# linkedin/gdmix

Hardware: AMD Instinct MI355X
Metric: random-effect entities converged/sec (higher is better)
Workload: dtype f64; 1 GPU; C2: synthetic 1000000 entities/GPU x avg 64 nnz (n~max(1,Poisson(16)), k=4 distinct uniform columns of D=1024, SURVEY 8(d) generator), per-entity L2 LR, L-BFGS m=10; build_id=003fc741b5b29e59, workload_key=c2, entities_per_gpu=1000000, step=pack+solve, theta on device, parallelism=entity-shard x1

## Files before the change

### gdmix_amd/csrc/re_api.hip

```cpp
#include <stdarg.h>
#include <stdio.h>
#include <stdlib.h>
#include <string.h>
#include <time.h>

#include <errno.h>
#include <fcntl.h>
#include <sys/file.h>
#include <sys/stat.h>
#include <unistd.h>

#include <condition_variable>
#include <map>
#include <new>
#include <string>

#include <mutex>

#include "re_internal.hpp"
#include "re_solve_team.hpp"

namespace gdmix {

static thread_local char g_err[512] = "";
// ... 180 lines not shown
  if ((e && atoi(e) == 0) || hipDeviceGetPCIBusId(bus, sizeof(bus), device) != hipSuccess || !bus[0] ||
      hipStreamCreateWithFlags(&g_rel_stream[device], hipStreamNonBlocking) != hipSuccess) {
    g_dev_lock_off[device] = true;
    return nullptr;
  }
  return g_dev_lock[device] = grid_lock_by_key(bus);
}

void grid_lock_release_cb(void* p) { static_cast<GridLock*>(p)->release(); }

std::mutex g_here_mu;
std::map<std::string, int> g_here_fd;

int presence_fd(int device) {
  char bus[64] = "";
  if (hipDeviceGetPCIBusId(bus, sizeof(bus), device) != hipSuccess || !bus[0]) return -1;
  std::lock_guard<std::mutex> g(g_here_mu);
  auto it = g_here_fd.find(bus);
  if (it != g_here_fd.end()) return it->second;
  const char* dir = getenv("GDMIX_RE_LOCK_DIR");
  std::string path = std::string(dir && *dir ? dir : "/tmp") + "/gdmix_re_grid_";
  for (const char* c = bus; *c; ++c) path += (isalnum((unsigned char)*c) || *c == '.' || *c == '-') ? *c : '_';
  path += ".here";
  const int fd = open(path.c_str(), O_RDWR | O_CREAT | O_CLOEXEC, 0666);
  if (fd >= 0) {
    (void)fchmod(fd, 0666);
    struct flock fl = {};
    fl.l_type = F_RDLCK; fl.l_whence = SEEK_SET; fl.l_start = 0; fl.l_len = 1;
    (void)fcntl(fd, F_SETLK, &fl);
  }
  return g_here_fd[bus] = fd;
}
}

void device_register_process(int device) {
  const char* e = getenv("GDMIX_RE_GRID_LOCK");
  if (!(e && atoi(e) == 0)) (void)presence_fd(device);
}

bool device_has_another_process(int device) {
  const char* e = getenv("GDMIX_RE_GRID_LOCK");
  if (e && atoi(e) == 0) return false;
  const int fd = presence_fd(device);
  if (fd < 0) return false;
  struct flock fl = {};
  fl.l_type = F_WRLCK; fl.l_whence = SEEK_SET; fl.l_start = 0; fl.l_len = 1;
  return fcntl(fd, F_GETLK, &fl) == 0 && fl.l_type != F_UNLCK;
}

ScopedGridGate::ScopedGridGate(int device, hipStream_t s) : device_(device >= 0 && device < GATE_DEVICES ? device : 0), s_(s), err_(hipSuccess), held_(nullptr) {
  g_gate_mu[device_].lock();
  if (!g_gate_ev[device_]) err_ = hipEventCreateWithFlags(&g_gate_ev[device_], hipEventDisableTiming);
  if (err_ == hipSuccess && g_gate_armed[device_]) err_ = hipStreamWaitEvent(s_, g_gate_ev[device_], 0);
  if (err_ == hipSuccess) {
    GridLock* const L = grid_lock_of_device(device_);
    if (L && L->acquire()) held_ = L;
  }
}

ScopedGridGate::~ScopedGridGate() {
  const bool recorded = g_gate_ev[device_] && hipEventRecord(g_gate_ev[device_], s_) == hipSuccess;
  if (recorded) g_gate_armed[device_] = true;
  if (held_) {
    GridLock* const L = static_cast<GridLock*>(held_);
    if (!(recorded && hipStreamWaitEvent(g_rel_stream[device_], g_gate_ev[device_], 0) == hipSuccess &&
          hipLaunchHostFunc(g_rel_stream[device_], grid_lock_release_cb, L) == hipSuccess)) {
      (void)hipStreamSynchronize(s_);
      L->release();
    }
  }
  g_gate_mu[device_].unlock();
}
}

extern "C" {

static int spread_default() {
  const char* e = getenv("GDMIX_RE_SPREAD");
  const int n = e ? atoi(e) : 4;
  return n > 1 ? n : 0;
}
GDMIX_API int gdmix_re_abi_version(void) { return GDMIX_RE_ABI_VERSION; }

GDMIX_API int gdmix_re_grid_lock_acquire(const char* key) {
  if (!key || !*key) { set_error("key is empty"); return GDMIX_RE_EINVAL; }
  return grid_lock_by_key(key)->acquire() ? GDMIX_RE_OK : GDMIX_RE_EINVAL;
}
GDMIX_API int gdmix_re_grid_lock_release(const char* key) {
  if (!key || !*key) { set_error("key is empty"); return GDMIX_RE_EINVAL; }
  grid_lock_by_key(key)->release();
  return GDMIX_RE_OK;
}
GDMIX_API int gdmix_re_grid_lock_stats(const char* key, int64_t* takes, int64_t* rides) {
  if (!key || !*key || !takes || !rides) { set_error("bad argument"); return GDMIX_RE_EINVAL; }
  long t = 0, r = 0;
  grid_lock_by_key(key)->stats(&t, &r);
  *takes = t;
  *rides = r;
  return GDMIX_RE_OK;
}

GDMIX_API const char* gdmix_re_last_error(void) { return g_err; }

GDMIX_API void gdmix_re_default_opts(gdmix_re_opts* o) {
  if (!o) return;
  o->l2 = 1.0; o->regularize_bias = 1; o->has_intercept = 1; o->m = 10; o->max_iter = 100;
  o->maxfun = 15000; o->maxls = 20; o->ftol = 1e-12; o->pgtol = 1e-5;
  o->variance_mode = GDMIX_RE_VAR_NONE; o->threshold = 1e-4;
  o->sum_loss = 0; o->loss = 0;
}

GDMIX_API int gdmix_re_create(int hip_device, gdmix_re_ctx** out) {
  if (!out) { set_error("out is NULL"); return GDMIX_RE_EINVAL; }
  *out = nullptr;
  int count = 0;
  HIP_TRY(hipGetDeviceCount(&count));
  if (hip_device < 0 || hip_device >= count) {
    set_error("HIP device %d not present (%d visible)", hip_device, count);
    return GDMIX_RE_EHIP;
  }
  HIP_TRY(hipSetDevice(hip_device));
  hipDeviceProp_t prop;
  HIP_TRY(hipGetDeviceProperties(&prop, hip_device));
  if (strncmp(prop.gcnArchName, "gfx950", 6) != 0) {
    set_error("device %d is %s; this library only carries gfx950 (MI355X) code", hip_device, prop.gcnArchName);
    return GDMIX_RE_EHIP;
  }
  gdmix_re_ctx* c = new (std::nothrow) gdmix_re_ctx();
  if (!c) { set_error("out of host memory"); return GDMIX_RE_ENOMEM; }
  c->impl.device = hip_device;
  c->impl.num_cus = prop.multiProcessorCount;
  device_register_process(hip_device);
  c->impl.tall_adapt_limit = c->impl.num_cus * 3 / 2;
  if (const char* e = getenv("GDMIX_RE_TALL_ADAPT")) c->impl.tall_adapt_limit = atoi(e) > 0 ? atoi(e) : 0;
  c->impl.scratch = nullptr;
  c->impl.scratch_bytes = 0;
  c->impl.host_pinned = nullptr;
  c->impl.wave_lds_limit = 65536;
  c->impl.kernel_mask = 7;
  c->impl.timing = 0;
  c->impl.giant_nnz = 16777216;
  c->impl.team_nnz = 16384;
  c->impl.tall_min_n = GDMIX_RE_TALL_MIN_N_DEFAULT;
  c->impl.tall_split_n = GDMIX_RE_TALL_SPLIT_N_DEFAULT;
  c->impl.tall_split_set = 0;
  c->impl.tall_team_n = GDMIX_RE_TALL_TEAM_N_DEFAULT;
  c->impl.tall_team_limit = c->impl.num_cus / 4 < TALL_TEAM_MAX ? c->impl.num_cus / 4 : TALL_TEAM_MAX;
  c->impl.tall_mid_n = 0;
  if (const char* e = getenv("GDMIX_RE_TALL_MID")) { if (atoi(e) == 1) c->impl.tall_mid_n = -(c->impl.num_cus * TALL_MID_WGS); else if (atoi(e) > 1) c->impl.tall_mid_n = -atoi(e); }
  if (c->impl.num_cus < 8 * TALL_TEAM_C) c->impl.tall_team_n = 0;
  if (const char* e = getenv("GDMIX_RE_TALL_TEAM")) { if (atoi(e) == 0) c->impl.tall_team_n = 0; }
  if (const char* e = getenv("GDMIX_RE_TALL_TEAM_LIMIT")) { if (atoi(e) > 0 && atoi(e) <= TALL_TEAM_MAX) c->impl.tall_team_limit = atoi(e); }
  c->impl.spread = spread_default();
  c->impl.grid_sync = nullptr;
  c->impl.big_tmp = nullptr;
  c->impl.big_tmp_bytes = 0;
  c->impl.eval_small_set = 0; c->impl.eval_small_max = 64;
  c->impl.eval_tmp = nullptr; c->impl.eval_tmp_bytes = 0;
  c->impl.n_side = 0; c->impl.side_fork = nullptr;
  c->impl.aux_ev[0] = c->impl.aux_ev[1] = nullptr;
  c->impl.defer_unique = 0; c->impl.unique_pending = false; c->impl.unique_ev = nullptr;
  for (int k = 0; k < gdmix_ctx_impl::MAX_SIDE; ++k) { c->impl.side[k] = nullptr; c->impl.side_join[k] = nullptr; }
  for (int k = 0; k < GDMIX_RE_NUM_CLASSES; ++k) { c->impl.ev0[k] = nullptr; c->impl.ev1[k] = nullptr; c->impl.ev_used[k] = false; }
  for (uint32_t& q : c->impl.mail_seq) q = 0;
  hipError_t rc = hipHostMalloc(reinterpret_cast<void**>(&c->impl.host_pinned), HOST_PINNED_BYTES, hipHostMallocMapped | hipHostMallocCoherent);
  if (rc == hipSuccess) memset(c->impl.host_pinned, 0, HOST_PINNED_BYTES);
  if (rc != hipSuccess) {
    set_error("hipHostMalloc failed: %s", hipGetErrorString(rc));
    delete c;
    return GDMIX_RE_EHIP;
  }
  {
    const char* e = getenv("GDMIX_RE_SIDE_STREAM");
    int want = e ? atoi(e) : 3;
    if (want > gdmix_ctx_impl::MAX_SIDE) want = gdmix_ctx_impl::MAX_SIDE;
    if (want > 0) {
      rc = hipEventCreateWithFlags(&c->impl.side_fork, hipEventDisableTiming);
      for (int k = 0; k < 2 && rc == hipSuccess; ++k) rc = hipEventCreateWithFlags(&c->impl.aux_ev[k], hipEventDisableTiming);
      if (rc == hipSuccess) rc = hipEventCreateWithFlags(&c->impl.unique_ev, hipEventDisableTiming);
      for (int k = 0; k < want && rc == hipSuccess; ++k) {
        rc = hipStreamCreateWithFlags(&c->impl.side[k], hipStreamNonBlocking);
        if (rc == hipSuccess) rc = hipEventCreateWithFlags(&c->impl.side_join[k], hipEventDisableTiming);
        if (rc == hipSuccess) c->impl.n_side = k + 1;
      }
      if (rc != hipSuccess) {
        set_error("creating the side streams failed: %s", hipGetErrorString(rc));
        gdmix_re_destroy(c);
        return GDMIX_RE_EHIP;
      }
    }
  }
  rc = hipMalloc(&c->impl.grid_sync, GridSyncLayout::BYTES);
  if (rc != hipSuccess) {
    set_error("hipMalloc failed: %s", hipGetErrorString(rc));
    (void)hipHostFree(c->impl.host_pinned);
    delete c;
    return GDMIX_RE_EHIP;
  }
  *out = c;
  return GDMIX_RE_OK;
}

GDMIX_API void gdmix_re_destroy(gdmix_re_ctx* ctx) {
  if (!ctx) return;
  if (ctx->impl.unique_pending && ctx->impl.unique_ev) (void)hipEventSynchronize(ctx->impl.unique_ev);
  if (ctx->impl.unique_ev) (void)hipEventDestroy(ctx->impl.unique_ev);
  if (ctx->impl.grid_sync) (void)hipFree(ctx->impl.grid_sync);
  if (ctx->impl.big_tmp) (void)hipFree(ctx->impl.big_tmp);
  if (ctx->impl.eval_tmp) (void)hipFree(ctx->impl.eval_tmp);
  if (ctx->impl.host_pinned) (void)hipHostFree(ctx->impl.host_pinned);
  if (ctx->impl.side_fork) (void)hipEventDestroy(ctx->impl.side_fork);
  for (int k = 0; k < 2; ++k) if (ctx->impl.aux_ev[k]) (void)hipEventDestroy(ctx->impl.aux_ev[k]);
  for (int k = 0; k < gdmix_ctx_impl::MAX_SIDE; ++k) {
    if (ctx->impl.side_join[k]) (void)hipEventDestroy(ctx->impl.side_join[k]);
    if (ctx->impl.side[k]) (void)hipStreamDestroy(ctx->impl.side[k]);
  }
  for (int k = 0; k < GDMIX_RE_NUM_CLASSES; ++k) {
    if (ctx->impl.ev0[k]) (void)hipEventDestroy(ctx->impl.ev0[k]);
    if (ctx->impl.ev1[k]) (void)hipEventDestroy(ctx->impl.ev1[k]);
  }
  delete ctx;
}

GDMIX_API size_t gdmix_re_pack_workspace_bytes(int64_t E, int64_t N, int64_t Z) {
  if (E < 0 || N < 0 || Z < 0) return 0;
  return pack_workspace_bytes(E, N, Z);
}

GDMIX_API int gdmix_re_pack(gdmix_re_ctx* ctx, const gdmix_re_raw_batch* raw_dev, int has_intercept, void* workspace,
                  size_t workspace_bytes, gdmix_re_packed* out, void* stream) {
  if (!ctx || !raw_dev || !out || (!workspace && workspace_bytes)) { set_error("NULL argument"); return GDMIX_RE_EINVAL; }
  if (raw_dev->E > 0 && (!raw_dev->ent_row_ptr || !raw_dev->row_nnz_ptr || !raw_dev->y || !raw_dev->offset)) {
    set_error("raw batch has NULL arrays");
    return GDMIX_RE_EINVAL;
  }
  if (raw_dev->Z > 0 && (!raw_dev->col_global || !raw_dev->val)) { set_error("raw batch has NULL arrays"); return GDMIX_RE_EINVAL; }
  HIP_TRY(hipSetDevice(ctx->impl.device));
  HIP_TRY(join_unique(&ctx->impl, static_cast<hipStream_t>(stream)));
  return pack_impl(&ctx->impl, raw_dev, has_intercept, workspace, workspace_bytes, out, static_cast<hipStream_t>(stream));
}

GDMIX_API int gdmix_re_set_defer_unique(gdmix_re_ctx* ctx, int enabled) {
  if (!ctx) { set_error("ctx is NULL"); return GDMIX_RE_EINVAL; }
  ctx->impl.defer_unique = (enabled && ctx->impl.n_side > 0) ? 1 : 0;
  return GDMIX_RE_OK;
}

GDMIX_API int gdmix_re_pack_join(gdmix_re_ctx* ctx, void* stream) {
  if (!ctx) { set_error("ctx is NULL"); return GDMIX_RE_EINVAL; }
  HIP_TRY(hipSetDevice(ctx->impl.device));
  HIP_TRY(join_unique(&ctx->impl, static_cast<hipStream_t>(stream)));
  return GDMIX_RE_OK;
}

static int slots_for(const gdmix_re_packed* b, const gdmix_re_opts* o, size_t* slot_doubles) {
  *slot_doubles = block_slot_doubles(b->max_p, b->max_n, o->m);
  size_t bytes = *slot_doubles * 8;
  size_t by_budget = ((size_t)4 << 30) / (bytes ? bytes : 1);
  size_t slots = 1024;
  if (slots > by_budget) slots = by_budget;
  if (slots < 8) slots = 8;
  if ((int64_t)slots > b->E) slots = (size_t)(b->E > 0 ? b->E : 1);
  return (int)slots;
}

static int64_t var_small_p(const gdmix_re_packed* b) { return b->max_p < VAR_FULL_MAX_P ? b->max_p : VAR_FULL_MAX_P; }

static int var_slots_for(const gdmix_re_packed* b) {
  size_t bytes = var_full_slot_doubles(var_small_p(b)) * 8;
  size_t slots = ((size_t)2 << 30) / (bytes ? bytes : 1);
  if (slots > 2048) slots = 2048;
  if (slots < 4) slots = 4;
  slots &= ~(size_t)3;
  return (int)slots;
}

GDMIX_API size_t gdmix_re_solve_scratch_bytes(const gdmix_re_packed* batch, const gdmix_re_opts* opts) {
  if (!batch || !opts || batch->E == 0) return 0;
  size_t slot_doubles;
  int slots = slots_for(batch, opts, &slot_doubles);
  size_t need = (size_t)slots * slot_doubles * 8;
  if (opts->variance_mode == GDMIX_RE_VAR_FULL && batch->max_p <= VAR_FULL_BIG_MAX_P) {
    size_t v = (size_t)var_slots_for(batch) * var_full_slot_doubles(var_small_p(batch)) * 8;
    if (v > need) need = v;
    if (batch->max_p > VAR_FULL_MAX_P) {
      v = var_full_big_doubles(batch->max_p, batch->max_n) * 8;
      if (v > need) need = v;
    }
  }
  return need;
}

GDMIX_API int gdmix_re_set_wave_lds_limit(gdmix_re_ctx* ctx, int bytes) {
  if (!ctx || bytes < 0) { set_error("bad argument"); return GDMIX_RE_EINVAL; }
  ctx->impl.wave_lds_limit = bytes > 65536 ? 65536 : bytes;
  return GDMIX_RE_OK;
}

GDMIX_API int gdmix_re_set_kernel_mask(gdmix_re_ctx* ctx, int mask) {
  if (!ctx) { set_error("ctx is NULL"); return GDMIX_RE_EINVAL; }
  ctx->impl.kernel_mask = mask & 7;
  return GDMIX_RE_OK;
}

GDMIX_API int gdmix_re_set_giant_nnz(gdmix_re_ctx* ctx, int64_t nnz) {
  if (!ctx || nnz < 0) { set_error("bad argument"); return GDMIX_RE_EINVAL; }
  ctx->impl.giant_nnz = nnz;
  return GDMIX_RE_OK;
}

GDMIX_API int gdmix_re_set_team_nnz(gdmix_re_ctx* ctx, int64_t nnz) {
  if (!ctx || nnz < 0) { set_error("bad argument"); return GDMIX_RE_EINVAL; }
  ctx->impl.team_nnz = nnz;
  return GDMIX_RE_OK;
}

GDMIX_API int gdmix_re_set_tall_min_n(gdmix_re_ctx* ctx, int min_n) {
  if (!ctx || min_n < 0) { set_error("bad argument"); return GDMIX_RE_EINVAL; }
  ctx->impl.tall_min_n = min_n;
  return GDMIX_RE_OK;
}

GDMIX_API int gdmix_re_set_spread(gdmix_re_ctx* ctx, int queues) {
  if (!ctx || queues < 0) { set_error("bad argument"); return GDMIX_RE_EINVAL; }
  ctx->impl.spread = queues > 1 ? queues : 0;
  return GDMIX_RE_OK;
}

GDMIX_API int gdmix_re_set_tall_team_n(gdmix_re_ctx* ctx, int team_n) {
  if (!ctx) { set_error("bad argument"); return GDMIX_RE_EINVAL; }
  ctx->impl.tall_team_n = ctx->impl.num_cus < 8 * TALL_TEAM_C ? 0 : team_n;
  return GDMIX_RE_OK;
}

GDMIX_API int gdmix_re_device_shared(gdmix_re_ctx* ctx) {
  if (!ctx) { set_error("ctx is NULL"); return GDMIX_RE_EINVAL; }
  return device_has_another_process(ctx->impl.device) ? 1 : 0;
}

GDMIX_API int gdmix_re_set_tall_mid_n(gdmix_re_ctx* ctx, int mid_n) {
  if (!ctx) { set_error("bad argument"); return GDMIX_RE_EINVAL; }
  ctx->impl.tall_mid_n = mid_n < 0 ? -(ctx->impl.num_cus * TALL_MID_WGS) : mid_n;
  return GDMIX_RE_OK;
}

GDMIX_API int gdmix_re_set_tall_split_n(gdmix_re_ctx* ctx, int split_n) {
  if (!ctx || split_n < 0) { set_error("bad argument"); return GDMIX_RE_EINVAL; }
  ctx->impl.tall_split_n = split_n > 0 ? split_n : GDMIX_RE_TALL_SPLIT_N_DEFAULT;
  ctx->impl.tall_split_set = split_n > 0 ? 1 : 0;
  return GDMIX_RE_OK;
}

GDMIX_API int gdmix_re_set_timing(gdmix_re_ctx* ctx, int enabled) {
  if (!ctx) { set_error("ctx is NULL"); return GDMIX_RE_EINVAL; }
  if (enabled && !ctx->impl.ev0[0]) {
    HIP_TRY(hipSetDevice(ctx->impl.device));
    for (int k = 0; k < GDMIX_RE_NUM_CLASSES; ++k) {
      HIP_TRY(hipEventCreate(&ctx->impl.ev0[k]));
      HIP_TRY(hipEventCreate(&ctx->impl.ev1[k]));
    }
  }
  ctx->impl.timing = enabled ? 1 : 0;
  return GDMIX_RE_OK;
}

GDMIX_API int gdmix_re_last_solve_ms(gdmix_re_ctx* ctx, float* ms_out) {
  if (!ctx || !ms_out) { set_error("NULL argument"); return GDMIX_RE_EINVAL; }
  for (int k = 0; k < GDMIX_RE_NUM_CLASSES; ++k) {
    ms_out[k] = 0.0f;
    if (ctx->impl.ev_used[k]) {
      HIP_TRY(hipEventSynchronize(ctx->impl.ev1[k]));
      HIP_TRY(hipEventElapsedTime(&ms_out[k], ctx->impl.ev0[k], ctx->impl.ev1[k]));
    }
  }
  return GDMIX_RE_OK;
}

GDMIX_API int gdmix_re_set_scratch(gdmix_re_ctx* ctx, void* scratch, size_t bytes) {
  if (!ctx) { set_error("ctx is NULL"); return GDMIX_RE_EINVAL; }
  ctx->impl.scratch = scratch;
  ctx->impl.scratch_bytes = bytes;
  return GDMIX_RE_OK;
}

static int run_variance_full(gdmix_re_ctx* ctx, const gdmix_re_packed* b, const BatchDev& B, const SolveParams& P, const double* theta,
                             double* variance, hipStream_t s) {
  const size_t vslot = var_full_slot_doubles(var_small_p(b));
  int vslots = var_slots_for(b);
  size_t avail = ctx->impl.scratch ? ctx->impl.scratch_bytes : 0;
  void* base = ctx->impl.scratch;
  if (b->scratch_bytes > avail) { avail = b->scratch_bytes; base = b->scratch; }
  if ((size_t)vslots * vslot * 8 > avail) vslots = (int)(avail / (vslot * 8)) & ~3;
  if (vslots < 4) {
    set_error("variance_mode FULL needs >= %zu bytes of scratch (gdmix_re_set_scratch)", 4 * vslot * 8);
    return GDMIX_RE_ENOMEM;
  }
  HIP_TRY(launch_variance_full(B, b->E, P, theta, variance, static_cast<double*>(base), vslot, vslots, var_small_p(b), s));
  if (b->max_p > VAR_FULL_MAX_P) {
    if (var_full_big_doubles(b->max_p, b->max_n) * 8 > avail) {
      set_error("variance_mode FULL with p = %d needs >= %zu bytes of scratch (gdmix_re_set_scratch)", b->max_p,
                var_full_big_doubles(b->max_p, b->max_n) * 8);
      return GDMIX_RE_ENOMEM;
    }
    HIP_TRY(launch_variance_full_big(&ctx->impl, B, b->E, P, theta, variance, static_cast<double*>(base), b->max_p, b->max_n, s));
  }
  return GDMIX_RE_OK;
}

}

namespace {

struct Slots { double* scratch = nullptr; size_t doubles = 0; int n = 0; };

int size_slots(const gdmix_ctx_impl* ci, const gdmix_re_packed* b, const gdmix_re_opts* opts, int n_slot_users, Slots* out) {
  if (n_slot_users <= 0) return GDMIX_RE_OK;
  out->n = slots_for(b, opts, &out->doubles);
  const size_t need = (size_t)out->n * out->doubles * 8;
  if (ci->scratch && ci->scratch_bytes >= need) out->scratch = static_cast<double*>(ci->scratch);
  else if (b->scratch && b->scratch_bytes >= need) out->scratch = static_cast<double*>(b->scratch);
  else {
    size_t avail = ci->scratch ? ci->scratch_bytes : 0;
    void* base = ci->scratch;
    if (b->scratch_bytes > avail) { avail = b->scratch_bytes; base = b->scratch; }
    out->n = (int)(avail / (out->doubles * 8));
    if (out->n < 1) {
      set_error("%d entities need a scratch slot: provide >= %zu bytes via gdmix_re_set_scratch", n_slot_users, out->doubles * 8);
      return GDMIX_RE_ENOMEM;
    }
    out->scratch = static_cast<double*>(base);
  }
  return GDMIX_RE_OK;
}

template <class F>
int timed(gdmix_ctx_impl* ci, int c, hipStream_t s, F&& launch) {
  if (ci->timing) HIP_TRY(hipEventRecord(ci->ev0[c], s));
  const hipError_t rc = launch();
  if (rc != hipSuccess) { set_error("launch of class %d (%s) failed: %s", c, kClasses[c].name, hipGetErrorString(rc)); return GDMIX_RE_EHIP; }
  if (ci->timing) { HIP_TRY(hipEventRecord(ci->ev1[c], s)); ci->ev_used[c] = true; }
  return GDMIX_RE_OK;
}

hipError_t launch_class(const gdmix_ctx_impl* ci, const gdmix_re_packed* b, const BatchDev& B, const OutDev& O, const SolveParams& P,
                        const double* theta0, const Launch& L, int lean_merged, hipStream_t s) {
  const ClassDesc& d = kClasses[L.c];
  switch (d.kind) {
    case KIND_WLDS:
      return launch_solve_wave(B, O, P, theta0, L.begin, L.count, d.lds, s);
    case KIND_TALL_T: {
      const char* xe = getenv("GDMIX_RE_XCD_BARRIER");
      return launch_solve_tall_team(B, O, P, theta0, L.begin, L.count, ci->num_cus, b->Z, GridSyncLayout::tall_tail(ci, d.tall_variant),
                                    GridSyncLayout::tall_team_buf(ci), (xe && atoi(xe) == 0) ? 0 : 1, s);
    }
    case KIND_TALL_L: case KIND_TALL_S: case KIND_TALL_M: case KIND_TALL:
      return launch_solve_tall(d.tall_variant, B, O, P, theta0, L.begin, L.count, ci->num_cus, b->Z, GridSyncLayout::tall_tail(ci, d.tall_variant),
                               GridSyncLayout::tall_ticket(ci, d.tall_variant), d.kind == KIND_TALL_S ? lean_merged : 0, s);
    default:
      return d.lanes > 0 ? launch_solve_quad(d.lanes, d.epl, B, O, P, theta0, L.begin, L.count, d.ncap, d.zcap, s) : hipErrorInvalidValue;
  }
}

int team_count(int tier_max, unsigned long long total_nnz, unsigned long long largest_nnz, int entities, int slots, int num_cus) {
  const unsigned long long ratio = largest_nnz ? total_nnz / largest_nnz : 1;
  int teams = 1;
  while (teams * 2 <= tier_max && (unsigned long long)(teams * 2) <= ratio) teams *= 2;
  if (entities <= 16) {
    int want = 1;
    while (want * 2 <= entities && want * 2 <= tier_max && want * 2 <= teams * 4) want *= 2;
    if (want > teams) teams = want;
  }
  if (const char* ev = getenv("GDMIX_RE_TEAMS")) teams = atoi(ev);
  if (teams > TEAM_MAX_TEAMS) teams = TEAM_MAX_TEAMS;
  while (teams > 1 && (slots < teams || num_cus % teams)) teams >>= 1;
  return teams < 1 ? 1 : teams;
}

int launch_slot_classes(gdmix_ctx_impl* ci, const gdmix_re_packed* b, const ClassCounts& hc, const BatchDev& B, OutDev O, const SolveParams& P,
                        const double* theta0, const Slots& slots, int n_slot_users, hipStream_t s) {
  const bool follow_var = P.loss != LOSS_LOGISTIC && P.variance_mode == GDMIX_RE_VAR_SIMPLE && P.m <= TEAM_MCAP;
  if (follow_var && P.loss == LOSS_POISSON && !O.theta) {
    set_error("variance_mode SIMPLE with the Poisson loss needs out->theta");
    return GDMIX_RE_EINVAL;
  }
  double* const variance = O.variance;
  if (follow_var) O.variance = nullptr;
  if (hc.count[BLOCK_CLASS] > 0) {
    const int rc = timed(ci, BLOCK_CLASS, s, [&] {
      return launch_solve_block(B, O, P, theta0, hc.base[BLOCK_CLASS], hc.count[BLOCK_CLASS], slots.scratch, slots.doubles, slots.n, b->max_p, s);
    });
    if (rc != GDMIX_RE_OK) return rc;
  }
  for (int c = TEAM128_CLASS; c <= GIANT_CLASS; ++c) {
    if (hc.count[c] <= 0) continue;
    const int tier_max = c == TEAM128_CLASS ? 128 : (c == TEAM32_CLASS ? 32 : 8);
    const int teams = c == GIANT_CLASS ? 1 : team_count(tier_max, hc.team_nnz_total[c], (unsigned long long)hc.largest_nnz(c), hc.count[c], slots.n, ci->num_cus);
    const int rc = timed(ci, c, s, [&] {
      return launch_solve_grid(B, O, P, theta0, hc.base[c], hc.count[c], slots.scratch, slots.doubles, b->max_p, GridSyncLayout::team_sync(ci), ci->num_cus, teams, s);
    });
    if (rc != GDMIX_RE_OK) return rc;
  }
  if (follow_var) HIP_TRY(launch_variance_simple(B, P, O.theta, variance, hc.base[BLOCK_CLASS], n_slot_users, slots.scratch, slots.doubles, slots.n, s));
  return GDMIX_RE_OK;
}

}

extern "C" {

GDMIX_API int gdmix_re_solve(gdmix_re_ctx* ctx, const gdmix_re_packed* b, const gdmix_re_opts* opts, const double* theta0,
                   const gdmix_re_result* out, void* stream) {
  if (!ctx || !b || !opts || !out) { set_error("NULL argument"); return GDMIX_RE_EINVAL; }
  if (opts->m < 1 || opts->max_iter < 0 || opts->maxls < 1) { set_error("bad solver options (m, max_iter, maxls)"); return GDMIX_RE_EINVAL; }
  if (!loss_code_ok(opts->loss, "gdmix_re_solve")) return GDMIX_RE_EINVAL;
  if (opts->variance_mode == GDMIX_RE_VAR_FULL) {
    if (!out->theta) { set_error("variance_mode FULL needs out->theta"); return GDMIX_RE_EINVAL; }
    if (b->max_p > VAR_FULL_BIG_MAX_P) {
      set_error("variance_mode FULL densifies a p x p Hessian per entity; largest entity has p = %d > %lld", b->max_p,
                (long long)VAR_FULL_BIG_MAX_P);
      return GDMIX_RE_ERANGE;
    }
  }
  if (opts->variance_mode != GDMIX_RE_VAR_NONE && !out->variance) { set_error("variance requested but out->variance is NULL"); return GDMIX_RE_EINVAL; }
  if (b->E == 0) return GDMIX_RE_OK;
  gdmix_ctx_impl* const ci = &ctx->impl;
  hipStream_t const s = static_cast<hipStream_t>(stream);
  HIP_TRY(hipSetDevice(ci->device));

  ClassTable tab;
  int rc = make_class_table(ci, opts, &tab);
  if (rc != GDMIX_RE_OK) return rc;
  const ClassCounts* hc = nullptr;
  rc = route(ci, b, tab, opts, s, &hc);
  if (rc != GDMIX_RE_OK) return rc;

  SolveParams P;
  P.l2 = opts->l2; P.ftol = opts->ftol; P.pgtol = opts->pgtol; P.threshold = opts->threshold;
  P.regularize_bias = opts->regularize_bias; P.has_intercept = opts->has_intercept ? 1 : 0; P.m = opts->m; P.max_iter = opts->max_iter;
  P.maxfun = opts->maxfun; P.maxls = opts->maxls; P.variance_mode = opts->variance_mode;
  P.sum_loss = opts->sum_loss ? 1 : 0; P.loss = opts->loss;
  const BatchDev B = batch_dev(b);
  const OutDev O{out->theta, out->theta_thr, out->variance, out->fval, out->gnorm, out->nit, out->nfev, out->status};
  for (int c = 0; c < GDMIX_RE_NUM_CLASSES; ++c) ci->ev_used[c] = false;

  int n_slot_users = 0;
  for (int c = BLOCK_CLASS; c <= GIANT_CLASS; ++c) n_slot_users += hc->count[c];
  Slots slots;
  rc = size_slots(ci, b, opts, n_slot_users, &slots);
  if (rc != GDMIX_RE_OK) return rc;

  int lean_rounds = 4;
  if (const char* ev = getenv("GDMIX_RE_LEAN_MERGE_ROUNDS")) lean_rounds = atoi(ev);
  const LaunchPlan plan = plan_launches(*hc, ci->num_cus, ci->n_side, ci->spread, lean_rounds);
  SideJoin side_join{ci, s};
  if (plan.fork) HIP_TRY(hipEventRecord(ci->side_fork, s));
  for (int k = 0; k < plan.n; ++k) {
    const Launch& L = plan.launch[k];
    hipStream_t q = s;
    if (L.stream >= 0) { HIP_TRY(side_join.use(L.stream)); q = ci->side[L.stream]; }
    rc = timed(ci, L.c, q, [&] { return launch_class(ci, b, B, O, P, theta0, L, plan.lean_merged, q); });
    if (rc != GDMIX_RE_OK) return rc;
  }
  side_join.join();
  if (n_slot_users > 0) {
    rc = launch_slot_classes(ci, b, *hc, B, O, P, theta0, slots, n_slot_users, s);
    if (rc != GDMIX_RE_OK) return rc;
  }
  if (opts->variance_mode == GDMIX_RE_VAR_FULL) {
    rc = run_variance_full(ctx, b, B, P, out->theta, out->variance, s);
    if (rc != GDMIX_RE_OK) return rc;
  }
  HIP_TRY(join_unique(ci, s));
  return GDMIX_RE_OK;
}

GDMIX_API int gdmix_re_variance_full(gdmix_re_ctx* ctx, const gdmix_re_packed* b, const gdmix_re_opts* opts, const double* theta,
                                     double* variance, void* stream) {
  if (!ctx || !b || !opts || !theta || !variance) { set_error("NULL argument"); return GDMIX_RE_EINVAL; }
  if (!loss_code_ok(opts->loss, "gdmix_re_variance_full")) return GDMIX_RE_EINVAL;
  if (b->max_p > VAR_FULL_BIG_MAX_P) {
    set_error("variance_mode FULL densifies a p x p Hessian per entity; largest entity has p = %d > %lld", b->max_p, (long long)VAR_FULL_BIG_MAX_P);
    return GDMIX_RE_ERANGE;
  }
  if (b->E == 0) return GDMIX_RE_OK;
  HIP_TRY(hipSetDevice(ctx->impl.device));
  HIP_TRY(join_unique(&ctx->impl, static_cast<hipStream_t>(stream)));
  SolveParams P;
  P.l2 = opts->l2; P.ftol = opts->ftol; P.pgtol = opts->pgtol; P.threshold = opts->threshold;
  P.regularize_bias = opts->regularize_bias; P.has_intercept = opts->has_intercept ? 1 : 0; P.m = opts->m; P.max_iter = opts->max_iter;
  P.maxfun = opts->maxfun; P.maxls = opts->maxls; P.variance_mode = GDMIX_RE_VAR_FULL;
  P.sum_loss = 0; P.loss = opts->loss;
  return run_variance_full(ctx, b, batch_dev(b), P, theta, variance, static_cast<hipStream_t>(stream));
}

GDMIX_API int gdmix_re_score(gdmix_re_ctx* ctx, const gdmix_re_packed* b, int has_intercept, const double* theta,
                   const uint8_t* has_model, float* logit, float* logit_per_coord, void* stream) {
  if (!ctx || !b || !logit || !logit_per_coord) { set_error("NULL argument"); return GDMIX_RE_EINVAL; }
  if (!theta && !has_model) { set_error("theta is NULL"); return GDMIX_RE_EINVAL; }
  HIP_TRY(hipSetDevice(ctx->impl.device));
  HIP_TRY(join_unique(&ctx->impl, static_cast<hipStream_t>(stream)));
  BatchDev B = batch_dev(b);
  HIP_TRY(launch_score(B, b->E, b->N, has_intercept ? 1 : 0, theta, has_model, logit, logit_per_coord,
                       static_cast<hipStream_t>(stream)));
  return GDMIX_RE_OK;
}

GDMIX_API const char* gdmix_re_class_kernel_name(int c) {
  if (c < 0 || c >= GDMIX_RE_NUM_CLASSES) return nullptr;
  return kClasses[c].name;
}

GDMIX_API int32_t gdmix_java_string_hash(const uint16_t* utf16, int64_t len) {
// ... 22 lines not shown
```

### gdmix_amd/csrc/re_internal.hpp

```cpp
#pragma once
#include <hip/hip_runtime.h>
#include <stdint.h>
#include <stddef.h>

#include <type_traits>

#include "../../include/gdmix_re.h"
#include "re_solve_core.hpp"
#include "re_solve_wreg.hpp"
#include "re_solve_quad.hpp"

namespace gdmix {

enum { KIND_WREG1 = 0, KIND_WREG2 = 1, KIND_WREG4 = 2, KIND_WLDS = 3, KIND_BLOCK = 4, KIND_QUAD2 = 5, KIND_QUAD4 = 6, KIND_PAIR4 = 7, KIND_QUAD3 = 8, KIND_PAIR3 = 9, KIND_WREG8 = 10,
       KIND_G64_3 = 11, KIND_G64_4 = 12, KIND_G128_4 = 13, KIND_G256_4 = 14, KIND_G512_4 = 15, KIND_GRID = 16, KIND_G128_3 = 17, KIND_G256_3 = 18,
       KIND_TALL = 20, KIND_TALL_S = 21, KIND_TALL_L = 22, KIND_TALL_T = 23, KIND_TALL_M = 24 };

__host__ __device__ constexpr int group_lanes(int kind) {
  return (kind == KIND_QUAD2 || kind == KIND_QUAD3 || kind == KIND_QUAD4) ? 16 : ((kind == KIND_PAIR3 || kind == KIND_PAIR4) ? 32 :
         ((kind == KIND_G64_3 || kind == KIND_G64_4) ? 64 : ((kind == KIND_G128_4 || kind == KIND_G128_3) ? 128 : ((kind == KIND_G256_4 || kind == KIND_G256_3) ? 256 : (kind == KIND_G512_4 ? 512 : 0)))));
}
__host__ __device__ constexpr int group_epl(int kind) {
  return kind == KIND_QUAD2 ? 2 : ((kind == KIND_QUAD3 || kind == KIND_PAIR3 || kind == KIND_G64_3 || kind == KIND_G128_3 || kind == KIND_G256_3) ? 3 : (group_lanes(kind) > 0 ? 4 : 0));
}
constexpr int TALL_TEAM_C = 4;
constexpr int TALL_TEAM_MAX = 64;
constexpr int TALL_TEAM_BYTES = 192 * 1024;
constexpr int TALL_TEAM_MIN_N = 64;
#ifndef GDMIX_TALL_NW_SMALL
#define GDMIX_TALL_NW_SMALL 1
#endif
constexpr int TALL_NW = 8;
constexpr int TALL_NW_SMALL = GDMIX_TALL_NW_SMALL;
constexpr int TALL_NW_MID = 4;
constexpr int TALL_MID_WGS = 2;
constexpr int TALL_MAX_P = 64;
constexpr int TALL_LEAN_WAVES = 3;
constexpr int TALL_LEAN_WGS = 4 * TALL_LEAN_WAVES;
__host__ __device__ constexpr int tall_sets(int nw, int p) { return (nw > 1 && p <= 32) ? 32 : 16; }
__host__ __device__ constexpr int tall_lds_bytes(int wg_per_cu) { return 160 * 1024 / wg_per_cu - 512; }
constexpr int TALL_LEAN_ARENA = (tall_lds_bytes(TALL_LEAN_WGS) - 1408) & ~15;
__host__ __device__ inline size_t tall_resident_bytes(int nw, int S, int d, int n, int nnz, bool has_w) {
  return (size_t)nw * (d + 1) * (S + 1) * 8 + (size_t)8 * (nnz + 8) + (size_t)4 * (n + 2) + (size_t)(has_w ? 12 : 8) * n + 16;
}

struct ClassDesc {
  int kind;
  int lanes, epl;
  int ncap, zcap;
  int lds;
  int occ_lanes;
  int tall_variant;
  int tall_rank;
  int small_side;
  const char* name;
};
enum { TALL_VARIANT_LARGE = 0, TALL_VARIANT_SMALL = 1, TALL_VARIANT_LEAN = 2, TALL_VARIANT_TEAM = 3, TALL_VARIANT_MID = 4, TALL_VARIANTS = 5 };
constexpr ClassDesc grp_class(int kind, int lanes, int epl, int ncap, int zcap, const char* name) { return {kind, lanes, epl, ncap, zcap, 1, lanes, -1, -1, -1, name}; }
constexpr ClassDesc wave_class(int lds, const char* name) { return {KIND_WLDS, 0, 0, 0, 0, lds, WAVE, -1, -1, -1, name}; }
constexpr ClassDesc tall_class(int kind, int variant, int rank, int occ_lanes, int side, const char* name) { return {kind, 0, 0, 0, 0, 0, occ_lanes, variant, rank, side, name}; }
constexpr ClassDesc team_class(int kind, const char* name) { return {kind, 0, 0, 0, 0, 0, WAVE, -1, -1, -1, name}; }
inline constexpr ClassDesc kClasses[GDMIX_RE_NUM_CLASSES] = {
    grp_class(KIND_QUAD2, 16, 2, 16, 64, "re_solve_grp_kernel<16,2> n<=16 nnz<=64"),
    grp_class(KIND_QUAD2, 16, 2, 32, 128, "re_solve_grp_kernel<16,2> n<=32 nnz<=128"),
    grp_class(KIND_QUAD2, 16, 2, 128, 512, "re_solve_grp_kernel<16,2> n<=128 nnz<=512"),
    grp_class(KIND_QUAD3, 16, 3, 16, 64, "re_solve_grp_kernel<16,3> n<=16 nnz<=64"),
    grp_class(KIND_QUAD3, 16, 3, 32, 128, "re_solve_grp_kernel<16,3> n<=32 nnz<=128"),
    grp_class(KIND_QUAD3, 16, 3, 128, 512, "re_solve_grp_kernel<16,3> n<=128 nnz<=512"),
    grp_class(KIND_QUAD4, 16, 4, 16, 64, "re_solve_grp_kernel<16,4> n<=16 nnz<=64"),
    grp_class(KIND_QUAD4, 16, 4, 32, 128, "re_solve_grp_kernel<16,4> n<=32 nnz<=128"),
    grp_class(KIND_QUAD4, 16, 4, 128, 512, "re_solve_grp_kernel<16,4> n<=128 nnz<=512"),
    grp_class(KIND_PAIR3, 32, 3, 32, 128, "re_solve_grp_kernel<32,3> n<=32 nnz<=128"),
    grp_class(KIND_PAIR3, 32, 3, 64, 256, "re_solve_grp_kernel<32,3> n<=64 nnz<=256"),
    grp_class(KIND_PAIR3, 32, 3, 256, 1024, "re_solve_grp_kernel<32,3> n<=256 nnz<=1024"),
    grp_class(KIND_PAIR4, 32, 4, 32, 128, "re_solve_grp_kernel<32,4> n<=32 nnz<=128"),
    grp_class(KIND_PAIR4, 32, 4, 64, 256, "re_solve_grp_kernel<32,4> n<=64 nnz<=256"),
    grp_class(KIND_PAIR4, 32, 4, 256, 1024, "re_solve_grp_kernel<32,4> n<=256 nnz<=1024"),
    grp_class(KIND_G64_3, 64, 3, 64, 512, "re_solve_grp_kernel<64,3> n<=64 nnz<=512"),
    grp_class(KIND_G64_3, 64, 3, 512, 2048, "re_solve_grp_kernel<64,3> n<=512 nnz<=2048"),
    grp_class(KIND_G64_4, 64, 4, 64, 512, "re_solve_grp_kernel<64,4> n<=64 nnz<=512"),
    grp_class(KIND_G64_4, 64, 4, 512, 2048, "re_solve_grp_kernel<64,4> n<=512 nnz<=2048"),
    grp_class(KIND_G128_3, 128, 3, 128, 1024, "re_solve_grp_kernel<128,3> n<=128 nnz<=1024"),
    grp_class(KIND_G128_3, 128, 3, 1024, 3072, "re_solve_grp_kernel<128,3> n<=1024 nnz<=3072"),
    grp_class(KIND_G128_4, 128, 4, 128, 1024, "re_solve_grp_kernel<128,4> n<=128 nnz<=1024"),
    grp_class(KIND_G128_4, 128, 4, 1024, 3072, "re_solve_grp_kernel<128,4> n<=1024 nnz<=3072"),
    grp_class(KIND_G256_3, 256, 3, 256, 2048, "re_solve_grp_kernel<256,3> n<=256 nnz<=2048"),
    grp_class(KIND_G256_3, 256, 3, 2048, 4096, "re_solve_grp_kernel<256,3> n<=2048 nnz<=4096"),
    grp_class(KIND_G256_4, 256, 4, 256, 2048, "re_solve_grp_kernel<256,4> n<=256 nnz<=2048"),
    grp_class(KIND_G256_4, 256, 4, 2048, 4096, "re_solve_grp_kernel<256,4> n<=2048 nnz<=4096"),
    grp_class(KIND_G512_4, 512, 4, 512, 4096, "re_solve_grp_kernel<512,4> n<=512 nnz<=4096"),
    wave_class(24576, "re_solve_wave_kernel lds<=24K"),
    wave_class(65536, "re_solve_wave_kernel lds<=64K"),
    tall_class(KIND_TALL_T, TALL_VARIANT_TEAM, 0, 0, 0, "re_solve_tall_team_kernel<8> x4 p<=64"),
    tall_class(KIND_TALL_L, TALL_VARIANT_LEAN, 4, WAVE, 0, "re_solve_tall_kernel<1> lean p<=64"),
    tall_class(KIND_TALL_S, TALL_VARIANT_SMALL, 3, WAVE, 2, "re_solve_tall_kernel<1> p<=64"),
    tall_class(KIND_TALL_M, TALL_VARIANT_MID, 2, 8 / TALL_MID_WGS * WAVE, -1, "re_solve_tall_kernel<4> p<=64"),
    tall_class(KIND_TALL, TALL_VARIANT_LARGE, 1, 4 * TALL_NW / 8 * WAVE, 1, "re_solve_tall_kernel<8> p<=64"),
    team_class(KIND_BLOCK, "re_solve_team_kernel workgroup"),
    team_class(KIND_GRID, "re_solve_team_kernel 128 teams"),
    team_class(KIND_GRID, "re_solve_team_kernel 32 teams"),
    team_class(KIND_GRID, "re_solve_team_kernel 8 teams"),
    team_class(KIND_GRID, "re_solve_team_kernel device-wide")};
constexpr int class_of_kind(int kind) {
  for (int c = 0; c < GDMIX_RE_NUM_CLASSES; ++c)
    if (kClasses[c].kind == kind) return c;
  return -1;
}
constexpr int TALL_T_CLASS = class_of_kind(KIND_TALL_T);
constexpr int TALL_L_CLASS = class_of_kind(KIND_TALL_L);
constexpr int TALL_S_CLASS = class_of_kind(KIND_TALL_S);
constexpr int TALL_M_CLASS = class_of_kind(KIND_TALL_M);
constexpr int TALL_CLASS = class_of_kind(KIND_TALL);
constexpr int BLOCK_CLASS = class_of_kind(KIND_BLOCK);
constexpr int TEAM128_CLASS = BLOCK_CLASS + 1;
constexpr int TEAM32_CLASS = BLOCK_CLASS + 2;
constexpr int TEAM8_CLASS = BLOCK_CLASS + 3;
constexpr int GIANT_CLASS = BLOCK_CLASS + 4;
constexpr int tall_class_of_rank(int rank) {
  for (int c = 0; c < GDMIX_RE_NUM_CLASSES; ++c)
    if (kClasses[c].tall_rank == rank) return c;
  return -1;
}
constexpr bool class_table_consistent() {
  for (int k = 0; k < TALL_VARIANTS; ++k)
    if (tall_class_of_rank(k) < 0) return false;

  for (int c = 0; c < GDMIX_RE_NUM_CLASSES; ++c) {
    const ClassDesc& d = kClasses[c];
    if (d.lanes != group_lanes(d.kind) || d.epl != group_epl(d.kind)) return false;
    if ((d.tall_variant >= 0) != (c >= TALL_T_CLASS && c < BLOCK_CLASS) || (d.tall_variant >= 0) != (d.tall_rank >= 0)) return false;
    if (c > BLOCK_CLASS && d.kind != KIND_GRID) return false;
    if (c < TALL_T_CLASS && d.lds <= 0) return false;
  }
  return true;
}
static_assert(class_table_consistent(), "group_lanes / group_epl and the class constants describe kClasses");
static_assert(GIANT_CLASS == GDMIX_RE_NUM_CLASSES - 1 && BLOCK_CLASS - TALL_T_CLASS == TALL_VARIANTS, "the tall classes, the block class, three tiers and the giant class end the table");
static_assert(TALL_L_CLASS + 1 == TALL_S_CLASS, "a merged lean class sits right in front of the one-wavefront class in `order`");
constexpr int BLOCK_NW = 4;
#ifndef GDMIX_TEAM_BLOCK_NW
#define GDMIX_TEAM_BLOCK_NW 8
#endif
constexpr int TEAM_BLOCK_NW = GDMIX_TEAM_BLOCK_NW;
constexpr int TEAM_GRID_NW = 8;

struct ClassTable {
  int kind[GDMIX_RE_NUM_CLASSES];
  int lds_bytes[GDMIX_RE_NUM_CLASSES];
  int ncap[GDMIX_RE_NUM_CLASSES];
  int zcap[GDMIX_RE_NUM_CLASSES];
  int64_t giant_nnz;
  int64_t team_nnz;
  int tall_min_n;
  int tall_split_n;
  int tall_adapt_limit;
  int tall_team_n;
  int tall_team_limit;
  int tall_mid_n;
};
constexpr int TALL_ADAPT_STEPS = 3;
__host__ __device__ constexpr int tall_adapt_n(int k) { return k == 0 ? 512 : (k == 1 ? 1024 : 2048); }
constexpr int TALL_TEAM_STEPS = 3;
constexpr int TALL_MID_STEPS = 6;
__host__ __device__ constexpr int tall_mid_step(int k) { return k == 0 ? 256 : (k == 1 ? 384 : (k == 2 ? 512 : (k == 3 ? 768 : (k == 4 ? 1024 : 1536)))); }
struct TallRouting {
  int32_t tall_ge[TALL_ADAPT_STEPS];
  int32_t split;
  int32_t team_ge[TALL_TEAM_STEPS];
  int32_t team_from;
  int32_t mid_ge[TALL_MID_STEPS];
  int32_t mid_from;
};
struct ClassCounts {
  int32_t count[GDMIX_RE_NUM_CLASSES];
  int32_t base[GDMIX_RE_NUM_CLASSES];
  int32_t cursor[GDMIX_RE_NUM_CLASSES];
  TallRouting tall;
  int32_t row3_free[TEAM128_CLASS - (int)(sizeof(TallRouting) / sizeof(int32_t))];
  int32_t team_largest_nnz[GDMIX_RE_NUM_CLASSES - TEAM128_CLASS];
  unsigned long long team_nnz_total[GDMIX_RE_NUM_CLASSES];
  __host__ __device__ int32_t& largest_nnz(int c) { return team_largest_nnz[c - TEAM128_CLASS]; }
  __host__ __device__ const int32_t& largest_nnz(int c) const { return team_largest_nnz[c - TEAM128_CLASS]; }
};
static_assert(sizeof(ClassCounts) == 6 * GDMIX_RE_NUM_CLASSES * sizeof(int32_t), "gdmix_re_packed::class_count is documented as [6*NUM_CLASSES]");
static_assert(offsetof(ClassCounts, count) == 0 && offsetof(ClassCounts, base) == 1 * GDMIX_RE_NUM_CLASSES * sizeof(int32_t) &&
              offsetof(ClassCounts, cursor) == 2 * GDMIX_RE_NUM_CLASSES * sizeof(int32_t) && offsetof(ClassCounts, tall) == 3 * GDMIX_RE_NUM_CLASSES * sizeof(int32_t) &&
              offsetof(ClassCounts, team_largest_nnz) == (3 * GDMIX_RE_NUM_CLASSES + TEAM128_CLASS) * sizeof(int32_t) &&
              offsetof(ClassCounts, team_nnz_total) == 4 * GDMIX_RE_NUM_CLASSES * sizeof(int32_t), "the rows of the count record");
static_assert(offsetof(TallRouting, mid_from) / sizeof(int32_t) < (size_t)TEAM128_CLASS, "row 3: the last threshold slot stays below the team tiers' columns");

struct BatchDev {
  const int64_t* ent_row_ptr;
  const int64_t* ent_nnz_ptr;
  const int64_t* ent_feat_ptr;
  const int32_t* row_ptr;
  const int32_t* csr_col;
  const float* csr_val;
  const int32_t* col_ptr;
  const int32_t* csc_row;
  const float* csc_val;
  const float* y;
  const float* offset;
  const float* weight;
  const int32_t* order;
};
inline BatchDev batch_dev(const gdmix_re_packed* b) {
  BatchDev B;
  B.ent_row_ptr = b->ent_row_ptr; B.ent_nnz_ptr = b->ent_nnz_ptr; B.ent_feat_ptr = b->ent_feat_ptr;
  B.row_ptr = b->row_ptr; B.csr_col = b->csr_col; B.csr_val = b->csr_val;
  B.col_ptr = b->col_ptr; B.csc_row = b->csc_row; B.csc_val = b->csc_val;
  B.y = b->y; B.offset = b->offset; B.weight = b->weight; B.order = b->order;
  return B;
}

struct OutDev {
  double* theta;
  double* theta_thr;
  double* variance;
  double* fval;
  double* gnorm;
  int32_t* nit;
  int32_t* nfev;
  int32_t* status;
};

struct gdmix_ctx_impl {
  int device;
  int num_cus;
  void* scratch;
  size_t scratch_bytes;
  int32_t* host_pinned;
  uint32_t mail_seq[4];
  int wave_lds_limit;
  int kernel_mask;
  int timing;
  int64_t giant_nnz;
  int64_t team_nnz;
  int tall_min_n;
  int tall_split_n;
  int tall_adapt_limit;
  int tall_split_set;
  int tall_team_n;
  int tall_team_limit;
  int tall_mid_n;
  int spread;
  void* grid_sync;
  void* big_tmp;
  size_t big_tmp_bytes;
  static constexpr int MAX_SIDE = 4;
  hipStream_t side[MAX_SIDE];
  int n_side;
  hipEvent_t side_fork, side_join[MAX_SIDE];
  hipEvent_t aux_ev[2];
  int defer_unique;
  bool unique_pending;
  hipEvent_t unique_ev;
  hipEvent_t ev0[GDMIX_RE_NUM_CLASSES], ev1[GDMIX_RE_NUM_CLASSES];
  bool ev_used[GDMIX_RE_NUM_CLASSES];
  int eval_small_set, eval_small_max;
  void* eval_tmp;
  size_t eval_tmp_bytes;
};

constexpr size_t HOST_PINNED_BYTES = 8192;
constexpr size_t MAILBOX_OFFSET = 4096, MAILBOX_BYTES = 1024, MAILBOX_DATA = 64;
constexpr int FETCH_SPIN_US = 400;
constexpr size_t COUNTS_READBACK_WORDS = 256;
static_assert(sizeof(ClassCounts) <= MAILBOX_BYTES - MAILBOX_DATA, "a larger count record falls back to copy + synchronise in post_small");
static_assert(COUNTS_READBACK_WORDS * sizeof(int32_t) + sizeof(ClassCounts) <= MAILBOX_OFFSET, "the read-back areas end where the mailboxes begin");
struct SmallFetch { int box; uint32_t seq; size_t bytes; void* host_dst; hipStream_t s; };
hipError_t post_small(gdmix_ctx_impl* ctx, int box, const void* dev_src, size_t bytes, void* host_dst, hipStream_t s, SmallFetch* f);
hipError_t wait_small(gdmix_ctx_impl* ctx, const SmallFetch& f);
inline hipError_t fetch_small(gdmix_ctx_impl* ctx, int box, const void* dev_src, size_t bytes, void* host_dst, hipStream_t s) {
  SmallFetch f;
  hipError_t rc = post_small(ctx, box, dev_src, bytes, host_dst, s, &f);
  return rc != hipSuccess ? rc : wait_small(ctx, f);
}

}

struct gdmix_re_ctx {
  gdmix::gdmix_ctx_impl impl;
};

namespace gdmix {

__host__ __device__ inline size_t wave_lds_bytes(int p, int n, int nnz, int d, int m, bool has_w) {
  size_t dbl = (size_t)(5 + 2 * m) * p + n + 2 * m;
  size_t w32 = (size_t)4 * nnz + (n + 1) + (d + 1) + (has_w ? 3 : 2) * (size_t)n;
  return ((dbl * 8 + w32 * 4) + 15) & ~(size_t)15;
}

inline size_t block_slot_doubles(int64_t max_p, int64_t max_n, int m) {
  return (size_t)5 * max_p + (size_t)2 * m * ((max_p + 63) & ~(int64_t)63) + max_n + 2 * m + 8 + 256 * 64;
}

struct SideJoin {
  gdmix_ctx_impl* ci; hipStream_t main; unsigned used = 0;
  hipError_t use(int k) {
    if (used & (1u << k)) return hipSuccess;
    const hipError_t rc = hipStreamWaitEvent(ci->side[k], ci->side_fork, 0);
    if (rc == hipSuccess) used |= 1u << k;
    return rc;
  }
  void join() {
    for (int k = 0; k < ci->n_side; ++k) {
      if (!(used & (1u << k))) continue;
      if (hipEventRecord(ci->side_join[k], ci->side[k]) != hipSuccess || hipStreamWaitEvent(main, ci->side_join[k], 0) != hipSuccess)
        (void)hipStreamSynchronize(ci->side[k]);
    }
    used = 0;
  }
  ~SideJoin() { join(); }
};

int make_class_table(const gdmix_ctx_impl* ci, const gdmix_re_opts* opts, ClassTable* out);
int route(gdmix_ctx_impl* ci, const gdmix_re_packed* b, const ClassTable& tab, const gdmix_re_opts* opts, hipStream_t s, const ClassCounts** host);
struct Launch { int c, begin, count, stream; };
struct LaunchPlan {
  Launch launch[GDMIX_RE_NUM_CLASSES];
  int n;
  int lean_merged;
  bool fork;
};
LaunchPlan plan_launches(const ClassCounts& counts, int num_cus, int n_side, int spread, int lean_rounds);
hipError_t launch_solve_quad(int g, int epl, const BatchDev& B, const OutDev& O, const SolveParams& o, const double* theta0,
                             int begin, int count, int ncap, int zcap, hipStream_t s);
hipError_t launch_solve_wave(const BatchDev& B, const OutDev& O, const SolveParams& o, const double* theta0,
                             int begin, int count, int lds_bytes, hipStream_t s);
hipError_t launch_solve_block(const BatchDev& B, const OutDev& O, const SolveParams& o, const double* theta0,
                              int begin, int count, double* scratch, size_t slot_doubles, int slots,
                              int64_t max_p, hipStream_t s);
hipError_t launch_solve_grid(const BatchDev& B, const OutDev& O, const SolveParams& o, const double* theta0,
                             int begin, int count, double* scratch, size_t slot_doubles, int64_t max_p,
                             void* sync_buf, int blocks, int teams, hipStream_t s);
constexpr int TALL_TAIL_BYTES = 256;
hipError_t launch_solve_tall(int variant, const BatchDev& B, const OutDev& O, const SolveParams& o, const double* theta0, int begin, int count,
                             int num_cus, int64_t Z, void* tail_buf, unsigned* ticket, int front_small, hipStream_t s);
hipError_t launch_solve_tall_team(const BatchDev& B, const OutDev& O, const SolveParams& o, const double* theta0, int begin, int count,
                                  int num_cus, int64_t Z, void* tail_buf, void* team_buf, int xcd_fast, hipStream_t s);
void launch_sort_class(int32_t* list, int count, const int64_t* ent_nnz_ptr, hipStream_t s);
static_assert(LOSS_LOGISTIC == GDMIX_RE_LOSS_LOGISTIC && LOSS_SQUARED == GDMIX_RE_LOSS_SQUARED && LOSS_POISSON == GDMIX_RE_LOSS_POISSON,
              "the device's loss codes are the header's");
bool loss_code_ok(int code, const char* who);
template <class F>
inline hipError_t with_loss(int code, F&& f) {
  switch (code) {
    case LOSS_LOGISTIC: return f(std::integral_constant<int, LOSS_LOGISTIC>{});
    case LOSS_SQUARED: return f(std::integral_constant<int, LOSS_SQUARED>{});
    case LOSS_POISSON: return f(std::integral_constant<int, LOSS_POISSON>{});
    default: return hipErrorInvalidValue;
  }
}
hipError_t launch_variance_simple(const BatchDev& B, const SolveParams& o, const double* theta, double* variance, int begin, int count,
                                  double* scratch, size_t slot_doubles, int slots, hipStream_t s);
hipError_t launch_variance_full(const BatchDev& B, int64_t E, const SolveParams& o, const double* theta, double* variance,
                                double* scratch, size_t slot_doubles, int slots, int64_t max_p, hipStream_t s);
constexpr int64_t VAR_FULL_MAX_P = 2048;
constexpr int64_t VAR_FULL_BIG_MAX_P = 16384;
constexpr int VAR_BIG_BUILD_GROUPS = 128;
size_t var_full_big_doubles(int64_t max_p, int64_t max_n);
hipError_t launch_variance_full_big(gdmix_ctx_impl* ci, const BatchDev& B, int64_t E, const SolveParams& o, const double* theta,
                                    double* variance, double* scratch, int64_t max_p, int64_t max_n, hipStream_t s);
size_t hessian_dense_scratch_doubles(int64_t n);
hipError_t launch_hessian_dense(gdmix_ctx_impl* ci, const BatchDev& B, int64_t n, int64_t d, int ic, const double* theta, double* H, int64_t ld,
                                double* scratch, hipStream_t s, int loss = LOSS_LOGISTIC);
hipError_t launch_variance_of_hessian(gdmix_ctx_impl* ci, double* H, double* M, int64_t p, int64_t ld, double l2, int64_t unreg, double* variance,
                                      hipStream_t s);
inline size_t var_full_slot_doubles(int64_t max_p) { return (size_t)2 * max_p * max_p + max_p + 8; }
hipError_t launch_score(const BatchDev& B, int64_t E, int64_t N, int ic, const double* theta, const uint8_t* has_model,
                        float* logit, float* per_coord, hipStream_t s);

inline hipError_t join_unique(gdmix_ctx_impl* ci, hipStream_t s) {
  if (!ci->unique_pending) return hipSuccess;
  const hipError_t q = hipEventQuery(ci->unique_ev);
  if (q == hipSuccess) { ci->unique_pending = false; return hipSuccess; }
  if (q != hipErrorNotReady) return q;
  return hipStreamWaitEvent(s, ci->unique_ev, 0);
}

size_t pack_workspace_bytes(int64_t E, int64_t N, int64_t Z);
int pack_impl(gdmix_ctx_impl* ctx, const gdmix_re_raw_batch* raw, int has_intercept, void* ws, size_t ws_bytes,
              gdmix_re_packed* out, hipStream_t s);
struct BigPackArgs {
  const int64_t* ent_row_ptr;
  const int64_t* ent_nnz_ptr;
  const int64_t* row_nnz_ptr;
  const int64_t* col_global;
  const float* val;
  int ic;
  int32_t* row_ptr;
  int32_t* csr_col;
  int32_t* col_ptr;
  int32_t* csc_row;
  float* csc_val;
  int32_t* uniq_sparse;
  int32_t* d_cnt;
  const int32_t* big_list;
  int n_big;
  int64_t big_nnz;
  int* max_p;
  int* err;
};
int pack_big_entities(gdmix_ctx_impl* ctx, const BigPackArgs& a, hipStream_t s, hipStream_t aux);

hipError_t launch_partition_ids(const int64_t* ids, int64_t count, int32_t num_partitions, int32_t* out,
                                hipStream_t s);

void set_error(const char* fmt, ...);

#define HIP_TRY(expr)                                                                        \
  do {                                                                                       \
    hipError_t _rc = (expr);                                                                 \
    if (_rc != hipSuccess) {                                                                 \
      set_error("%s failed: %s (%s:%d)", #expr, hipGetErrorString(_rc), __FILE__, __LINE__); \
      return GDMIX_RE_EHIP;                                                                  \
    }                                                                                        \
  } while (0)

void device_register_process(int device);
bool device_has_another_process(int device);

class ScopedGridGate {
 public:
  ScopedGridGate(int device, hipStream_t s);
  ~ScopedGridGate();
  hipError_t status() const { return err_; }
 private:
  int device_;
  hipStream_t s_;
  hipError_t err_;
  void* held_;
};

struct DynLdsOnce {
  unsigned long long done = 0;
  hipError_t set(const void* fn, int bytes = 160 * 1024) {
    int dev = 0;
    hipError_t rc = hipGetDevice(&dev);
    if (rc != hipSuccess) return rc;
    if (dev >= 0 && dev < 64 && ((done >> dev) & 1ull)) return hipSuccess;
    rc = hipFuncSetAttribute(fn, hipFuncAttributeMaxDynamicSharedMemorySize, bytes);
    if (rc == hipSuccess && dev >= 0 && dev < 64) done |= 1ull << dev;
    return rc;
  }
};

}
```

### gdmix_amd/csrc/re_route.hip

```cpp
#include <stdlib.h>

#include "re_internal.hpp"
#include "re_solve_team.hpp"

namespace gdmix {

int make_class_table(const gdmix_ctx_impl* ci, const gdmix_re_opts* opts, ClassTable* out) {
  ClassTable& tab = *out;
  for (int c = 0; c < GDMIX_RE_NUM_CLASSES; ++c) {
    const ClassDesc& d = kClasses[c];
    tab.kind[c] = d.kind;
    tab.ncap[c] = d.ncap;
    tab.zcap[c] = d.zcap;
    int lds = d.lds;
    const int gl = d.lanes;
    if (lds > 0 && gl > 0)
      lds = (gl >= WAVE ? 1 : WAVE / gl) * quad_layout(gl * d.epl, d.ncap, d.zcap, gl > WAVE ? gl / WAVE : 1).bytes;
    bool on = lds > 0 && (lds <= ci->wave_lds_limit || (gl > WAVE && ci->wave_lds_limit >= 65536 && lds <= 160 * 1024));
    if (gl > 0 && !(ci->kernel_mask & 4)) on = false;
    if (d.kind == KIND_WLDS && !(ci->kernel_mask & 2)) on = false;
    tab.lds_bytes[c] = on ? lds : 0;
  }
  tab.giant_nnz = opts->m <= TEAM_MCAP ? ci->giant_nnz : 0;
  tab.team_nnz = opts->m <= TEAM_MCAP ? ci->team_nnz : 0;
  tab.tall_min_n = ci->tall_min_n;
  tab.tall_split_n = ci->tall_split_n;
  tab.tall_adapt_limit = ci->tall_split_set ? 0 : ci->tall_adapt_limit;
  {
    const int tn = ci->tall_team_n;
    tab.tall_team_n = tn > 0 ? tn : -tn;
    if (tab.tall_team_n > 0 && tab.tall_team_n < TALL_TEAM_MIN_N) tab.tall_team_n = TALL_TEAM_MIN_N;
    tab.tall_team_limit = tn > 0 ? ci->tall_team_limit : 0;
  }
  tab.tall_mid_n = (ci->tall_mid_n < 0 && ci->tall_split_set) ? 0 : ci->tall_mid_n;
  if (opts->sum_loss) {
    if (opts->m > TEAM_MCAP) { set_error("sum_loss needs m <= %d", TEAM_MCAP); return GDMIX_RE_EINVAL; }
    if (opts->variance_mode != GDMIX_RE_VAR_NONE) { set_error("variance is not available with sum_loss"); return GDMIX_RE_EINVAL; }
    tab.giant_nnz = 1;
  }
  return GDMIX_RE_OK;
}

__global__ void re_classify_kernel(const int64_t* __restrict__ ent_row_ptr, const int64_t* __restrict__ ent_nnz_ptr,
                                   const int64_t* __restrict__ ent_feat_ptr, int64_t E, int ic, int m, bool has_w,
                                   ClassTable tab, int32_t* __restrict__ cls_out, ClassCounts* __restrict__ counts) {
  __shared__ int32_t local[GDMIX_RE_NUM_CLASSES];
  __shared__ int32_t tall_ge[TALL_ADAPT_STEPS], team_ge[TALL_TEAM_STEPS], mid_ge[TALL_MID_STEPS];
  if (threadIdx.x < GDMIX_RE_NUM_CLASSES) local[threadIdx.x] = 0;
  if (threadIdx.x < TALL_ADAPT_STEPS) tall_ge[threadIdx.x] = 0;
  if (threadIdx.x < TALL_TEAM_STEPS) team_ge[threadIdx.x] = 0;
  if (threadIdx.x < TALL_MID_STEPS) mid_ge[threadIdx.x] = 0;
  __syncthreads();
  for (int64_t e = (int64_t)blockIdx.x * blockDim.x + threadIdx.x; e < E; e += (int64_t)gridDim.x * blockDim.x) {
    const int n = (int)(ent_row_ptr[e + 1] - ent_row_ptr[e]);
    const int z = (int)(ent_nnz_ptr[e + 1] - ent_nnz_ptr[e]);
    const int d = (int)(ent_feat_ptr[e + 1] - ent_feat_ptr[e]);
    const int p = d + ic;
    int c = BLOCK_CLASS;
    const size_t wlds_bytes = wave_lds_bytes(p, n, z, d, m, has_w);
    for (int k = 0; k < BLOCK_CLASS; ++k) {
      if (tab.lds_bytes[k] <= 0) continue;
      const int kind = tab.kind[k];
      if (group_lanes(kind) > 0) {
        const int cap = group_lanes(kind) * group_epl(kind);
        if (m <= M_REG && p <= cap && n <= tab.ncap[k] && z <= tab.zcap[k]) { c = k; break; }
      } else if (kind == KIND_WLDS) {
        if (wlds_bytes <= (size_t)tab.lds_bytes[k]) { c = k; break; }
      }
    }
    if (tab.tall_min_n > 0 && m <= M_REG && p <= TALL_MAX_P && n >= tab.tall_min_n && !(tab.giant_nnz > 0 && z >= tab.giant_nnz)) c = (n >= tab.tall_split_n) ? TALL_CLASS
        : (tall_resident_bytes(1, tall_sets(1, p), d, n, z, has_w) <= (size_t)TALL_LEAN_ARENA ? TALL_L_CLASS : TALL_S_CLASS);
    else if (tab.giant_nnz > 0 && z >= tab.giant_nnz) c = GIANT_CLASS;
    else if (c == BLOCK_CLASS || (tab.team_nnz > 0 && z >= tab.team_nnz)) {
      if (tab.team_nnz > 0 && z >= tab.team_nnz)
        c = (z >= 128 * tab.team_nnz) ? TEAM8_CLASS : ((z >= 8 * tab.team_nnz) ? TEAM32_CLASS : TEAM128_CLASS);
    }
    cls_out[e] = c;
    atomicAdd(&local[c], 1);
    if (c == TALL_S_CLASS && tab.tall_adapt_limit > 0 && n >= tall_adapt_n(0)) {
#pragma unroll
      for (int k = 0; k < TALL_ADAPT_STEPS; ++k)
        if (n >= tall_adapt_n(k)) atomicAdd(&tall_ge[k], 1);
    }
    if (c == TALL_S_CLASS && tab.tall_mid_n < 0 && n >= tall_mid_step(0)) {
#pragma unroll
      for (int k = 0; k < TALL_MID_STEPS; ++k)
        if (n >= tall_mid_step(k)) atomicAdd(&mid_ge[k], 1);
    }
    if (c == TALL_S_CLASS && tab.tall_mid_n > 0 && n >= tab.tall_mid_n) atomicAdd(&mid_ge[0], 1);
    if (c == TALL_CLASS && tab.tall_team_n > 0 && n >= tab.tall_team_n) {
#pragma unroll
      for (int k = 0; k < TALL_TEAM_STEPS; ++k)
        if ((int64_t)n >= ((int64_t)tab.tall_team_n << k)) atomicAdd(&team_ge[k], 1);
    }
    if (c >= TEAM128_CLASS && c <= TEAM8_CLASS) {
      atomicAdd(&counts->team_nnz_total[c], (unsigned long long)z);
      atomicMax(&counts->largest_nnz(c), z);
    }
  }
  __syncthreads();
  if (threadIdx.x < GDMIX_RE_NUM_CLASSES && local[threadIdx.x]) atomicAdd(&counts->count[threadIdx.x], local[threadIdx.x]);
  if (threadIdx.x < TALL_ADAPT_STEPS && tall_ge[threadIdx.x]) atomicAdd(&counts->tall.tall_ge[threadIdx.x], tall_ge[threadIdx.x]);
  if (threadIdx.x < TALL_TEAM_STEPS && team_ge[threadIdx.x]) atomicAdd(&counts->tall.team_ge[threadIdx.x], team_ge[threadIdx.x]);
  if (threadIdx.x < TALL_MID_STEPS && mid_ge[threadIdx.x]) atomicAdd(&counts->tall.mid_ge[threadIdx.x], mid_ge[threadIdx.x]);
}

__global__ void class_base_kernel(ClassCounts* cc, int tall_adapt_limit, int tall_adapt_small, int tall_team_n, int tall_team_limit, int tall_mid_n) {
  if (threadIdx.x == 0 && blockIdx.x == 0) {
    int32_t* const count = cc->count;
    TallRouting& t = cc->tall;
    int team_from = 0;
    if (tall_team_n > 0) {
      if (tall_team_limit <= 0) { if (t.team_ge[0] > 0) team_from = tall_team_n; }
      else
        for (int k = 0; k < TALL_TEAM_STEPS && team_from == 0; ++k)
          if (t.team_ge[k] > 0 && t.team_ge[k] <= tall_team_limit) team_from = tall_team_n << k;
      if (team_from > 0) {
        const int moved = t.team_ge[team_from == tall_team_n ? 0 : (team_from == 2 * tall_team_n ? 1 : 2)];
        count[TALL_T_CLASS] += moved;
        count[TALL_CLASS] -= moved;
      }
    }
    t.team_from = team_from;
    int split = 0;
    if (tall_adapt_limit > 0 && count[TALL_S_CLASS] <= tall_adapt_small) {
      for (int k = 0; k < TALL_ADAPT_STEPS && split == 0; ++k)
        if (t.tall_ge[k] > 0 && count[TALL_CLASS] + t.tall_ge[k] <= tall_adapt_limit) {
          split = tall_adapt_n(k);
          count[TALL_CLASS] += t.tall_ge[k];
          count[TALL_S_CLASS] -= t.tall_ge[k];
        }
    }
    t.split = split;
    int mid_from = 0;
    const int gone = split > 0 ? t.tall_ge[split == tall_adapt_n(0) ? 0 : (split == tall_adapt_n(1) ? 1 : 2)] : 0;
    if (tall_mid_n > 0) {
      const int cnt = (split > 0 && split <= tall_mid_n) ? 0 : t.mid_ge[0] - gone;
      if (cnt > 0) { mid_from = tall_mid_n; count[TALL_M_CLASS] += cnt; count[TALL_S_CLASS] -= cnt; }
    } else if (tall_mid_n < 0 && count[TALL_S_CLASS] <= tall_adapt_small) {
      for (int k = 0; k < TALL_MID_STEPS && mid_from == 0; ++k) {
        if (split > 0 && tall_mid_step(k) >= split) break;
        const int cnt = t.mid_ge[k] - gone;
        if (cnt > 0 && cnt <= -tall_mid_n) { mid_from = tall_mid_step(k); count[TALL_M_CLASS] += cnt; count[TALL_S_CLASS] -= cnt; }
      }
    }
    t.mid_from = mid_from;
    int run = 0;
#pragma unroll
    for (int c = 0; c < GDMIX_RE_NUM_CLASSES; ++c) { cc->base[c] = run; run += count[c]; cc->cursor[c] = 0; }
  }
}

__global__ __launch_bounds__(256) void re_order_kernel(int32_t* __restrict__ cls, int64_t E, ClassCounts* __restrict__ cc,
                                                       int32_t* __restrict__ order, const int64_t* __restrict__ ent_row_ptr) {
  __shared__ int32_t cnt[GDMIX_RE_NUM_CLASSES], base[GDMIX_RE_NUM_CLASSES];
  const int split = cc->tall.split;
  const int team_from = cc->tall.team_from;
  const int mid_from = cc->tall.mid_from;
  const int64_t chunk = (int64_t)blockDim.x * 8;
  for (int64_t start = (int64_t)blockIdx.x * chunk; start < E; start += (int64_t)gridDim.x * chunk) {
    if (threadIdx.x < GDMIX_RE_NUM_CLASSES) cnt[threadIdx.x] = 0;
    __syncthreads();
    int c[8], pos[8];
#pragma unroll
    for (int k = 0; k < 8; ++k) {
      const int64_t e = start + (int64_t)k * blockDim.x + threadIdx.x;
      c[k] = (e < E) ? cls[e] : -1;
      if (split > 0 && c[k] == TALL_S_CLASS && ent_row_ptr[e + 1] - ent_row_ptr[e] >= split) { c[k] = TALL_CLASS; cls[e] = TALL_CLASS; }
      else if (team_from > 0 && c[k] == TALL_CLASS && ent_row_ptr[e + 1] - ent_row_ptr[e] >= team_from) { c[k] = TALL_T_CLASS; cls[e] = TALL_T_CLASS; }
      else if (mid_from > 0 && c[k] == TALL_S_CLASS && ent_row_ptr[e + 1] - ent_row_ptr[e] >= mid_from) { c[k] = TALL_M_CLASS; cls[e] = TALL_M_CLASS; }
      pos[k] = (c[k] >= 0) ? atomicAdd(&cnt[c[k]], 1) : 0;
    }
    __syncthreads();
    if (threadIdx.x < GDMIX_RE_NUM_CLASSES)
      base[threadIdx.x] = cnt[threadIdx.x] ? atomicAdd(&cc->cursor[threadIdx.x], cnt[threadIdx.x]) : 0;
    __syncthreads();
#pragma unroll
    for (int k = 0; k < 8; ++k) {
      const int64_t e = start + (int64_t)k * blockDim.x + threadIdx.x;
      if (c[k] >= 0) order[cc->base[c[k]] + base[c[k]] + pos[k]] = (int32_t)e;
    }
    __syncthreads();
  }
}

static hipError_t launch_classify(const gdmix_re_packed* b, int ic, int m, const ClassTable& tab, ClassCounts* counts, hipStream_t s) {
  int grid = (int)((b->E + 255) / 256);
  if (grid > 2048) grid = 2048;
  hipLaunchKernelGGL(re_classify_kernel, dim3(grid), dim3(256), 0, s, b->ent_row_ptr, b->ent_nnz_ptr,
                     b->ent_feat_ptr, b->E, ic, m, b->weight != nullptr, tab, b->cls_tmp, counts);
  return hipGetLastError();
}

static hipError_t launch_order(const gdmix_re_packed* b, ClassCounts* counts, hipStream_t s) {
  int grid = (int)((b->E + 2047) / 2048);
  if (grid > 2048) grid = 2048;
  hipLaunchKernelGGL(re_order_kernel, dim3(grid), dim3(256), 0, s, b->cls_tmp, b->E, counts, b->order, b->ent_row_ptr);
  return hipGetLastError();
}

int route(gdmix_ctx_impl* ci, const gdmix_re_packed* b, const ClassTable& tab, const gdmix_re_opts* opts, hipStream_t s,
          const ClassCounts** host) {
  ClassCounts* const cc = reinterpret_cast<ClassCounts*>(b->class_count);
  HIP_TRY(hipMemsetAsync(cc, 0, sizeof(ClassCounts), s));
  HIP_TRY(launch_classify(b, opts->has_intercept ? 1 : 0, opts->m, tab, cc, s));
  hipLaunchKernelGGL(class_base_kernel, dim3(1), dim3(1), 0, s, cc, tab.tall_adapt_limit, 16 * ci->num_cus, tab.tall_team_n, tab.tall_team_limit, tab.tall_mid_n);
  HIP_TRY(hipGetLastError());
  HIP_TRY(launch_order(b, cc, s));
  ClassCounts* const hc = reinterpret_cast<ClassCounts*>(ci->host_pinned + COUNTS_READBACK_WORDS);
  HIP_TRY(fetch_small(ci, 0, cc, sizeof(ClassCounts), hc, s));
  *host = hc;
  return GDMIX_RE_OK;
}

static bool class_is_small(const ClassDesc& d, int count, int num_cus) {
  const long waves = ((long)count * d.occ_lanes + WAVE - 1) / WAVE;
  return waves < (long)num_cus * 6;
}

LaunchPlan plan_launches(const ClassCounts& counts, int num_cus, int n_side, int spread, int lean_rounds) {
  LaunchPlan plan;
  plan.n = 0;
  const int lean = counts.count[TALL_L_CLASS];
  plan.lean_merged = (lean > 0 && lean < lean_rounds * num_cus * TALL_LEAN_WGS) ? lean : 0;
  int begin[GDMIX_RE_NUM_CLASSES], count[GDMIX_RE_NUM_CLASSES], n_launch_classes = 0;
  for (int c = 0; c < GDMIX_RE_NUM_CLASSES; ++c) { begin[c] = counts.base[c]; count[c] = counts.count[c]; }
  if (plan.lean_merged) { count[TALL_L_CLASS] = 0; begin[TALL_S_CLASS] -= plan.lean_merged; count[TALL_S_CLASS] += plan.lean_merged; }
  for (int c = 0; c < GDMIX_RE_NUM_CLASSES; ++c) n_launch_classes += (counts.count[c] > 0 && !(c == TALL_L_CLASS && plan.lean_merged)) ? 1 : 0;
  plan.fork = false;
  if (n_side > 0 && n_launch_classes > 1) {
    for (int c = 0; c < BLOCK_CLASS && !plan.fork; ++c) plan.fork = count[c] > 0 && class_is_small(kClasses[c], count[c], num_cus);
    if (spread > 1) plan.fork = true;
  }
  bool small[GDMIX_RE_NUM_CLASSES], any_large = false;
  for (int k = 0; k < TALL_VARIANTS + BLOCK_CLASS; ++k) {
    const int c = k < TALL_VARIANTS ? tall_class_of_rank(k) : k - TALL_VARIANTS;
    if (k >= TALL_VARIANTS && kClasses[c].tall_rank >= 0) continue;
    if (count[c] <= 0) continue;
    small[plan.n] = plan.fork && class_is_small(kClasses[c], count[c], num_cus);
    any_large = any_large || !small[plan.n];
    plan.launch[plan.n++] = Launch{c, begin[c], count[c], -1};
  }
  int spread_rr = 0;
  for (int k = 0; k < plan.n; ++k) {
    Launch& L = plan.launch[k];
    if (small[k]) {
      const int side = kClasses[L.c].small_side;
      L.stream = side >= 0 ? side % n_side : (any_large ? 0 : -1);
    } else if (plan.fork && spread > 1) {
      const int nq = spread < n_side + 1 ? spread : n_side + 1;
      L.stream = spread_rr++ % nq - 1;
    }
  }
  return plan;
}

}
```

### gdmix_amd/csrc/re_solve.hip

```cpp
#include "re_internal.hpp"
#include "re_search.hpp"
#include "re_solve_team.hpp"

namespace gdmix {

template <class G>
__device__ __forceinline__ void write_results(G& grp, const OutDev& O, const SolveParams& o, int64_t e, int64_t c0,
                                              int p, const double* x, const SolveStats& st) {
  for (int j = grp.tid; j < p; j += grp.NT) {
    const double v = x[j];
    if (O.theta) O.theta[c0 + j] = v;
    if (O.theta_thr) O.theta_thr[c0 + j] = (fabs(v) <= o.threshold) ? 0.0 : v;
  }
  if (grp.tid == 0) {
    if (O.fval) O.fval[e] = st.f;
    if (O.gnorm) O.gnorm[e] = st.gnorm;
    if (O.nit) O.nit[e] = st.nit;
    if (O.nfev) O.nfev[e] = st.nfev;
    if (O.status) O.status[e] = st.status;
  }
}

#ifndef GDMIX_QUAD_WAVES_EPL4
#define GDMIX_QUAD_WAVES_EPL4 2
#endif
#ifndef GDMIX_QUAD_WAVES_EPL2
#define GDMIX_QUAD_WAVES_EPL2 2
#endif
template <int G, int EPL, int NCAP, int ZCAP, int LOSS>
__global__ __launch_bounds__(G > WAVE ? G : WAVE)
__attribute__((amdgpu_waves_per_eu(EPL == 2 ? GDMIX_QUAD_WAVES_EPL2 : (EPL >= 3 ? GDMIX_QUAD_WAVES_EPL4 : 1)))) void re_solve_grp_kernel(
    BatchDev B, OutDev O, SolveParams o, const double* __restrict__ theta0, int begin, int count) {
  extern __shared__ __align__(16) unsigned char smem[];
  constexpr int NG = G >= WAVE ? 1 : WAVE / G;
  constexpr int NWG = G > WAVE ? G / WAVE : 1;
  const int tid = threadIdx.x;
  const int row = (G >= WAVE) ? 0 : (tid / G);
  const int gl = (G >= WAVE) ? tid : (tid & (G - 1));
  const int slot = blockIdx.x * NG + row;
  const bool valid = slot < count;
  const int64_t e = valid ? (int64_t)B.order[begin + slot] : 0;
  const int ic = o.has_intercept ? 1 : 0;
  const int64_t r0 = B.ent_row_ptr[e], z0 = B.ent_nnz_ptr[e], f0 = B.ent_feat_ptr[e];
  const int n = valid ? (int)(B.ent_row_ptr[e + 1] - r0) : 0;
  const int nnz = valid ? (int)(B.ent_nnz_ptr[e + 1] - z0) : 0;
  const int d = valid ? (int)(B.ent_feat_ptr[e + 1] - f0) : 0;
  const int p = valid ? d + ic : 0;
  const int64_t c0 = f0 + e * ic;

  QuadLds L;
  L.q = quad_layout(G * EPL, NCAP, ZCAP, NWG);
  L.base = smem + (size_t)row * L.q.bytes;
  L.hdr = L.base + (NWG > 1 ? (tid >> 6) * QUAD_HDR_BYTES : 0);
  L.has_w = B.weight != nullptr;
  XWave X;
  X.buf = reinterpret_cast<double*>(L.base + QUAD_HDR_BYTES * NWG);
  X.phase = 0;

  if (valid) {
    for (int k = gl; k < nnz; k += G) {
      L.csr()[k] = make_int2(B.csr_col[z0 + k], __float_as_int(B.csr_val[z0 + k]));
      L.csc()[k] = make_int2(B.csc_row[z0 + k], __float_as_int(B.csc_val[z0 + k]));
    }
    for (int i = gl; i < n; i += G) {
      L.y()[i] = B.y[r0 + i];
      L.o()[i] = B.offset[r0 + i];
      if (L.has_w) L.w()[i] = B.weight[r0 + i];
    }
    for (int i = gl; i <= n; i += G) L.row_ptr()[i] = B.row_ptr[r0 + e + i];
    for (int i = gl; i <= d; i += G) L.col_ptr()[i] = B.col_ptr[z0 + e + i];
  }
  unsigned rowc = 0, colc[EPL];
  if (gl < n) {
    const int k0 = B.row_ptr[r0 + e + gl], k1 = B.row_ptr[r0 + e + gl + 1];
    rowc = (unsigned)k0 | ((unsigned)(k1 - k0) << 16);
  }
  QuadState<EPL> V;
#pragma unroll
  for (int s = 0; s < EPL; ++s) {
    const int j = gl + G * s;
    colc[s] = 0;
    if (j < p && j >= ic) {
      const int k0 = B.col_ptr[z0 + e + (j - ic)], k1 = B.col_ptr[z0 + e + (j - ic) + 1];
      colc[s] = (unsigned)k0 | ((unsigned)(k1 - k0) << 16);
    }
    V.x[s] = (theta0 && j < p) ? theta0[c0 + j] : 0.0;
    V.g[s] = 0.0; V.d[s] = 0.0;
  }
  grp_fence<G>();
  SolveStats st;
  quad_solve<G, EPL, (NCAP > G), LOSS>(L, o, gl, n, p, ic, valid, rowc, colc, V, X, st);
  if (!valid) return;

#pragma unroll
  for (int s = 0; s < EPL; ++s) {
    const int j = gl + G * s;
    if (j < p) {
      const double v = V.x[s];
      if (O.theta) O.theta[c0 + j] = v;
      if (O.theta_thr) O.theta_thr[c0 + j] = (fabs(v) <= o.threshold) ? 0.0 : v;
    }
  }
  if (gl == 0) {
    if (O.fval) O.fval[e] = st.f;
    if (O.gnorm) O.gnorm[e] = st.gnorm;
    if (O.nit) O.nit[e] = st.nit;
    if (O.nfev) O.nfev[e] = st.nfev;
    if (O.status) O.status[e] = st.status;
  }
  if (o.variance_mode == GDMIX_RE_VAR_SIMPLE && O.variance) {
    double* const xs = L.xs();
    double* const rs = L.rs();
    grp_fence<G>();
#pragma unroll
    for (int s = 0; s < EPL; ++s) {
      const int j = gl + G * s;
      if (j < p) xs[j] = V.x[s];
    }
    grp_fence<G>();
    const double x0 = ic ? xs[0] : 0.0;
    double dpart = 0.0;
    for (int i = gl; i < n; i += G) {
      double di;
      if constexpr (LOSS == LOSS_SQUARED) {
        di = 2.0 * (L.has_w ? (double)L.w()[i] : 1.0);
      } else if constexpr (LOSS == LOSS_POISSON) {
        const int k0 = L.row_ptr()[i], k1 = L.row_ptr()[i + 1];
        const double z = gather_dot(L.csr() + k0, k1 - k0, xs + ic, x0) + (double)L.o()[i];
        di = exp_any(z) * (L.has_w ? (double)L.w()[i] : 1.0);
      } else {
        const int k0 = L.row_ptr()[i], k1 = L.row_ptr()[i + 1];
        const double z = gather_dot(L.csr() + k0, k1 - k0, xs + ic, x0) + (double)L.o()[i];
        const double rho = sigmoid_full(z);
        di = rho * (1.0 - rho) * (L.has_w ? (double)L.w()[i] : 1.0);
      }
      rs[i] = di;
      dpart += di;
    }
    const double dsum = grp_sum<G>(dpart, X);
    grp_fence<G>();
    const int first_reg = (ic && !o.regularize_bias) ? 1 : 0;
#pragma unroll
    for (int s = 0; s < EPL; ++s) {
      const int j = gl + G * s;
      if (j < p) {
        double h;
        if (ic && j == 0) {
          h = dsum;
        } else {
          h = 0.0;
          const int2* csc = L.csc();
          int k = (int)(colc[s] & 0xffffu);
          const int k1 = k + (int)(colc[s] >> 16);
          while (k < k1) {
            const int rw = csc[k].x;
            double v = (double)__int_as_float(csc[k].y);
            ++k;
            while (k < k1 && csc[k].x == rw) { v += (double)__int_as_float(csc[k].y); ++k; }
            h += v * v * rs[rw];
          }
        }
        h += (j < first_reg) ? 0.0 : o.l2;
        O.variance[c0 + j] = 1.0 / (h + 1.0e-12);
      }
    }
  }
}

template <int G, int EPL, int NCAP, int ZCAP, int LOSS>
static hipError_t launch_quad_t(const BatchDev& B, const OutDev& O, const SolveParams& o, const double* theta0,
                                int begin, int count, hipStream_t s) {
  constexpr int NG = G >= WAVE ? 1 : WAVE / G;
  constexpr int NWG = G > WAVE ? G / WAVE : 1;
  const int row_lds_bytes = quad_layout(G * EPL, NCAP, ZCAP, NWG).bytes;
  static DynLdsOnce lds_attr;
  if (hipError_t rc = lds_attr.set(reinterpret_cast<const void*>(re_solve_grp_kernel<G, EPL, NCAP, ZCAP, LOSS>)); rc != hipSuccess) return rc;
  hipLaunchKernelGGL((re_solve_grp_kernel<G, EPL, NCAP, ZCAP, LOSS>), dim3((count + NG - 1) / NG), dim3(G > WAVE ? G : WAVE),
                     (size_t)row_lds_bytes * NG, s, B, O, o, theta0, begin, count);
  return hipGetLastError();
}

hipError_t launch_solve_quad(int g, int epl, const BatchDev& B, const OutDev& O, const SolveParams& o, const double* theta0,
                             int begin, int count, int ncap, int zcap, hipStream_t s) {
  if (count <= 0) return hipSuccess;
#define GDMIX_GRP_CASE(GG, EE, NN, ZZ) \
  if (g == GG && epl == EE && ncap == NN && zcap == ZZ)                                                            \
    return with_loss(o.loss, [&](auto L) { return launch_quad_t<GG, EE, NN, ZZ, decltype(L)::value>(B, O, o, theta0, begin, count, s); });
  GDMIX_GRP_CASE(16, 2, 16, 64) GDMIX_GRP_CASE(16, 2, 32, 128) GDMIX_GRP_CASE(16, 2, 128, 512)
  GDMIX_GRP_CASE(16, 3, 16, 64) GDMIX_GRP_CASE(16, 3, 32, 128) GDMIX_GRP_CASE(16, 3, 128, 512)
  GDMIX_GRP_CASE(16, 4, 16, 64) GDMIX_GRP_CASE(16, 4, 32, 128) GDMIX_GRP_CASE(16, 4, 128, 512)
  GDMIX_GRP_CASE(32, 3, 32, 128) GDMIX_GRP_CASE(32, 3, 64, 256) GDMIX_GRP_CASE(32, 3, 256, 1024)
  GDMIX_GRP_CASE(32, 4, 32, 128) GDMIX_GRP_CASE(32, 4, 64, 256) GDMIX_GRP_CASE(32, 4, 256, 1024)
  GDMIX_GRP_CASE(64, 3, 64, 512) GDMIX_GRP_CASE(64, 3, 512, 2048) GDMIX_GRP_CASE(64, 4, 64, 512) GDMIX_GRP_CASE(64, 4, 512, 2048)
  GDMIX_GRP_CASE(128, 3, 128, 1024) GDMIX_GRP_CASE(128, 3, 1024, 3072) GDMIX_GRP_CASE(128, 4, 128, 1024) GDMIX_GRP_CASE(128, 4, 1024, 3072)
  GDMIX_GRP_CASE(256, 3, 256, 2048) GDMIX_GRP_CASE(256, 3, 2048, 4096) GDMIX_GRP_CASE(256, 4, 256, 2048) GDMIX_GRP_CASE(256, 4, 2048, 4096)
  GDMIX_GRP_CASE(512, 4, 512, 4096)
#undef GDMIX_GRP_CASE
  return hipErrorInvalidValue;
}

template <int LOSS>
__global__ __launch_bounds__(WAVE) void re_solve_wave_kernel(BatchDev B, OutDev O, SolveParams o,
                                                             const double* __restrict__ theta0, int begin) {
  extern __shared__ __align__(16) unsigned char smem[];
  const int lane = threadIdx.x;
  const int64_t e = B.order[begin + blockIdx.x];
  const int ic = o.has_intercept ? 1 : 0;
  const int64_t r0 = B.ent_row_ptr[e], z0 = B.ent_nnz_ptr[e], f0 = B.ent_feat_ptr[e];
  const int n = (int)(B.ent_row_ptr[e + 1] - r0);
  const int nnz = (int)(B.ent_nnz_ptr[e + 1] - z0);
  const int d = (int)(B.ent_feat_ptr[e + 1] - f0);
  const int p = d + ic;
  const int m = o.m;
  const int64_t c0 = f0 + e * ic;

  double* dp = reinterpret_cast<double*>(smem);
  Work W;
  W.x = dp; dp += p;
  W.g = dp; dp += p;
  W.d = dp; dp += p;
  W.t = dp; dp += p;
  W.r = dp; dp += p;
  W.ws = dp; dp += (size_t)m * p;
  W.wy = dp; dp += (size_t)m * p;
  W.rs = dp; dp += n;
  W.alpha = dp; dp += m;
  W.rho = dp; dp += m;
  float* fp = reinterpret_cast<float*>(dp);
  float* s_csr_val = fp; fp += nnz;
  float* s_csc_val = fp; fp += nnz;
  float* s_y = fp; fp += n;
  float* s_o = fp; fp += n;
  float* s_w = nullptr;
  if (B.weight) { s_w = fp; fp += n; }
  int32_t* ip = reinterpret_cast<int32_t*>(fp);
  int32_t* s_csr_col = ip; ip += nnz;
  int32_t* s_csc_row = ip; ip += nnz;
  int32_t* s_row_ptr = ip; ip += n + 1;
  int32_t* s_col_ptr = ip; ip += d + 1;

  for (int k = lane; k < nnz; k += WAVE) {
    s_csr_val[k] = B.csr_val[z0 + k];
    s_csr_col[k] = B.csr_col[z0 + k];
    s_csc_val[k] = B.csc_val[z0 + k];
    s_csc_row[k] = B.csc_row[z0 + k];
  }
  for (int i = lane; i < n; i += WAVE) {
    s_y[i] = B.y[r0 + i];
    s_o[i] = B.offset[r0 + i];
    if (s_w) s_w[i] = B.weight[r0 + i];
  }
  for (int i = lane; i <= n; i += WAVE) s_row_ptr[i] = B.row_ptr[r0 + e + i];
  for (int i = lane; i <= d; i += WAVE) s_col_ptr[i] = B.col_ptr[z0 + e + i];
  for (int j = lane; j < p; j += WAVE) W.x[j] = theta0 ? theta0[c0 + j] : 0.0;

  WaveGroup grp{lane};
  grp.sync();
  EntityView P{n, d, p, ic, s_row_ptr, s_csr_col, s_csr_val, s_col_ptr, s_csc_row, s_csc_val, s_y, s_o, s_w};
  SolveStats st;
  lbfgs_solve<LOSS>(grp, P, o, W, st);
  write_results(grp, O, o, e, c0, p, W.x, st);
  if (o.variance_mode == GDMIX_RE_VAR_SIMPLE && O.variance) variance_simple<false, LOSS>(grp, P, o, W, O.variance + c0);
}

hipError_t launch_solve_wave(const BatchDev& B, const OutDev& O, const SolveParams& o, const double* theta0,
                             int begin, int count, int lds_bytes, hipStream_t s) {
  if (count <= 0) return hipSuccess;
  return with_loss(o.loss, [&](auto L) {
    constexpr int LOSS = decltype(L)::value;
    static DynLdsOnce lds_attr;
    if (hipError_t rc = lds_attr.set(reinterpret_cast<const void*>(re_solve_wave_kernel<LOSS>)); rc != hipSuccess) return rc;
    hipLaunchKernelGGL(re_solve_wave_kernel<LOSS>, dim3(count), dim3(WAVE), (size_t)lds_bytes, s, B, O, o, theta0, begin);
    return hipGetLastError();
  });
}

template <int LOSS>
__global__ __launch_bounds__(WAVE* BLOCK_NW) void re_solve_block_kernel(BatchDev B, OutDev O, SolveParams o,
                                                                        const double* __restrict__ theta0,
                                                                        int begin, int count, double* scratch,
                                                                        size_t slot_doubles, int64_t max_p) {
  __shared__ double red[2 * BLOCK_NW];
  const int ic = o.has_intercept ? 1 : 0;
  const int m = o.m;
  double* slot = scratch + (size_t)blockIdx.x * slot_doubles;
  for (int idx = blockIdx.x; idx < count; idx += gridDim.x) {
    const int64_t e = B.order[begin + idx];
    const int64_t r0 = B.ent_row_ptr[e], z0 = B.ent_nnz_ptr[e], f0 = B.ent_feat_ptr[e];
    const int n = (int)(B.ent_row_ptr[e + 1] - r0);
    const int d = (int)(B.ent_feat_ptr[e + 1] - f0);
    const int p = d + ic;
    const int64_t c0 = f0 + e * ic;
    double* dp = slot;
    Work W;
    W.x = dp; dp += max_p;
    W.g = dp; dp += max_p;
    W.d = dp; dp += max_p;
    W.t = dp; dp += max_p;
    W.r = dp; dp += max_p;
    W.ws = dp; dp += (size_t)m * max_p;
    W.wy = dp; dp += (size_t)m * max_p;
    W.alpha = dp; dp += m;
    W.rho = dp; dp += m;
    W.rs = dp;
    BlockGroup<BLOCK_NW> grp{(int)threadIdx.x, red, 0};
    for (int j = grp.tid; j < p; j += grp.NT) W.x[j] = theta0 ? theta0[c0 + j] : 0.0;
    grp.sync();
    EntityView P{n, d, p, ic, B.row_ptr + r0 + e, B.csr_col + z0, B.csr_val + z0, B.col_ptr + z0 + e,
                 B.csc_row + z0, B.csc_val + z0, B.y + r0, B.offset + r0, B.weight ? B.weight + r0 : nullptr};
    SolveStats st;
    lbfgs_solve<LOSS>(grp, P, o, W, st);
    write_results(grp, O, o, e, c0, p, W.x, st);
    if (o.variance_mode == GDMIX_RE_VAR_SIMPLE && O.variance) variance_simple<false, LOSS>(grp, P, o, W, O.variance + c0);
    grp.sync();
  }
}

constexpr int SORT_CAP = 16384;
constexpr int SORT_RANK_CAP = 4096;
__global__ __launch_bounds__(1024) void re_sort_class_kernel(int32_t* __restrict__ list, int count,
                                                             const int64_t* __restrict__ ent_nnz_ptr) {
  extern __shared__ __align__(16) unsigned char sort_smem[];
  unsigned long long* const key = reinterpret_cast<unsigned long long*>(sort_smem);
  int np2 = 1;
  while (np2 < count) np2 <<= 1;
  for (int i = threadIdx.x; i < np2; i += blockDim.x) {
    unsigned long long k = ~0ull;
    if (i < count) {
      const int64_t e = list[i];
      const unsigned long long z = (unsigned long long)(ent_nnz_ptr[e + 1] - ent_nnz_ptr[e]);
      k = ((0xffffffffull - (z & 0xffffffffull)) << 32) | (unsigned long long)(uint32_t)e;
    }
    key[i] = k;
  }
  __syncthreads();
  if (count <= SORT_RANK_CAP) {
    unsigned long long mine[SORT_RANK_CAP / 1024];
    int rank[SORT_RANK_CAP / 1024];
#pragma unroll
    for (int q = 0; q < SORT_RANK_CAP / 1024; ++q) {
      const int i = threadIdx.x + q * 1024;
      mine[q] = i < count ? key[i] : ~0ull;
      rank[q] = 0;
// ... 403 lines not shown
```

### gdmix_amd/csrc/re_solve_quad.hpp

```cpp
#pragma once
#include "re_solve_wreg.hpp"

namespace gdmix {

constexpr int ROW = 16;

template <int CTRL>
__device__ __forceinline__ double dpp_row(double v) {
  int lo = __builtin_amdgcn_mov_dpp(__double2loint(v), CTRL, 0xf, 0xf, true);
  int hi = __builtin_amdgcn_mov_dpp(__double2hiint(v), CTRL, 0xf, 0xf, true);
  return __hiloint2double(hi, lo);
}


__device__ __forceinline__ double row_sum(double v) {
  v += dpp_row<0xB1>(v);
  v += dpp_row<0x4E>(v);
  v += dpp_row<0x141>(v);
  v += dpp_row<0x140>(v);
  return v;
}

__device__ __forceinline__ void row_sum2(double& a, double& b) {
#define GDMIX_RSTEP2(CTRL)              \
// ... 257 lines not shown
    acc += (r > 3 ? (double)__int_as_float(p3.y) : 0.0) * v3;
  }
  return acc;
}

template <int EPL>
__device__ __forceinline__ void gather_dot2_cols(const int2* csc, const unsigned (&colc)[EPL], const double* vec, double (&acc)[EPL]) {
  int len[EPL], mx = 0;
  const int2* pairs[EPL];
#pragma unroll
  for (int s = 0; s < EPL; ++s) {
    len[s] = (int)(colc[s] >> 16);
    pairs[s] = csc + (colc[s] & 0xffffu);
    mx = max(mx, len[s]);
  }
  for (int c = 0; c < mx; c += 2) {
    int2 p0[EPL], p1[EPL];
#pragma unroll
    for (int s = 0; s < EPL; ++s) {
      const int r = len[s] - c;
      p0[s] = pairs[s][r > 0 ? c : 0];
      p1[s] = pairs[s][r > 1 ? c + 1 : 0];
      if (r <= 0) p0[s] = make_int2(0, 0);
      if (r <= 1) p1[s] = make_int2(0, 0);
    }
    double v0[EPL], v1[EPL];
#pragma unroll
    for (int s = 0; s < EPL; ++s) { v0[s] = vec[p0[s].x]; v1[s] = vec[p1[s].x]; }
#pragma unroll
    for (int s = 0; s < EPL; ++s) {
      acc[s] += (double)__int_as_float(p0[s].y) * v0[s];
      acc[s] += (double)__int_as_float(p1[s].y) * v1[s];
    }
  }
}

template <int EPL>
__device__ __forceinline__ void gather_dot1_cols(const int2* csc, const unsigned (&colc)[EPL], const double* vec, double (&acc)[EPL]) {
  int len[EPL], mx = 0;
  const int2* pairs[EPL];
#pragma unroll
  for (int s = 0; s < EPL; ++s) {
    len[s] = (int)(colc[s] >> 16);
    pairs[s] = csc + (colc[s] & 0xffffu);
    mx = max(mx, len[s]);
  }
  for (int c = 0; c < mx; ++c) {
    int2 p0[EPL];
#pragma unroll
    for (int s = 0; s < EPL; ++s) {
      p0[s] = pairs[s][c < len[s] ? c : 0];
      if (c >= len[s]) p0[s] = make_int2(0, 0);
    }
    double v0[EPL];
#pragma unroll
    for (int s = 0; s < EPL; ++s) v0[s] = vec[p0[s].x];
#pragma unroll
    for (int s = 0; s < EPL; ++s) acc[s] += (double)__int_as_float(p0[s].y) * v0[s];
  }
}

template <int G, int EPL, bool LONG_COLS = true, int LOSS = LOSS_LOGISTIC>
__device__ __forceinline__ double quad_eval(const QuadLds& L, const SolveParams& o, int gl, int n, int p, int ic,
                                            unsigned rowc, const unsigned (&colc)[EPL], const double (&xt)[EPL],
                                            double (&g)[EPL], XWave& X, bool first, bool& counted) {
  double* const xs = L.xs();
  double* const rs = L.rs();
  bool mv = first;
#pragma unroll
  for (int s = 0; s < EPL; ++s) {
    const int j = gl + G * s;
    if (j < p) {
      mv = mv || (xs[j] != xt[s]);
      xs[j] = xt[s];
    }
  }
  counted = grp_any<G>(mv);
  if (G > WAVE) L.scal()[SC_MOVED] = counted ? 1.0 : 0.0;
  grp_fence<G>();
  if (G > WAVE) {
    constexpr int NWG = G / WAVE;
    bool any = false;
#pragma unroll
    for (int w = 0; w < NWG; ++w) any = any || reinterpret_cast<const double*>(L.base + w * QUAD_HDR_BYTES + 16 * M_REG + 128)[SC_MOVED] != 0.0;
    counted = any;
  }
  double part = 0.0, rpart = 0.0;
  const double x0 = ic ? xs[0] : 0.0;
  if (gl < n) {
    const double z = gather_dot(L.csr() + (rowc & 0xffffu), (int)(rowc >> 16), xs + ic, x0) + (double)L.o()[gl];
    double ri;
    part = loss_terms<LOSS>(z, (double)L.y()[gl], L.has_w ? (double)L.w()[gl] : 1.0, ri);
    rs[gl] = ri;
    rpart = ri;
  }
  for (int i = gl + G; i < n; i += G) {
    const int k0 = L.row_ptr()[i], k1 = L.row_ptr()[i + 1];
    const double z = gather_dot(L.csr() + k0, k1 - k0, xs + ic, x0) + (double)L.o()[i];
    double ri;
    part += loss_terms<LOSS>(z, (double)L.y()[i], L.has_w ? (double)L.w()[i] : 1.0, ri);
    rs[i] = ri;
    rpart += ri;
  }
  const int first_reg = (ic && !o.regularize_bias) ? 1 : 0;
  double sq = 0.0;
#pragma unroll
  for (int s = 0; s < EPL; ++s) {
    const int j = gl + G * s;
    if (j >= first_reg && j < p) sq += xt[s] * xt[s];
  }
  grp_sum3<G>(part, rpart, sq, X);
  part += 0.5 * o.l2 * sq;
  grp_fence<G>();
  const double inv_n = 1.0 / (double)n;
  if (EPL <= 3 || LONG_COLS) {
    double acc[EPL];
    unsigned cc[EPL];
#pragma unroll
    for (int s = 0; s < EPL; ++s) {
      const int j = gl + G * s;
      acc[s] = (ic && j == 0) ? rpart : 0.0;
      cc[s] = (j < p) ? colc[s] : 0u;
    }
    if (EPL <= 3) gather_dot2_cols<EPL>(L.csc(), cc, rs, acc);
    else gather_dot1_cols<EPL>(L.csc(), cc, rs, acc);
#pragma unroll
    for (int s = 0; s < EPL; ++s) {
      const int j = gl + G * s;
      const double reg = (j < first_reg) ? 0.0 : o.l2 * xt[s];
      g[s] = (j < p) ? inv_n * (acc[s] + reg) : 0.0;
    }
    return inv_n * part;
  }
#pragma unroll
  for (int s = 0; s < EPL; ++s) {
    const int j = gl + G * s;
    double gj = 0.0;
    if (j < p) {
      double acc = (ic && j == 0) ? rpart : 0.0;
      acc = gather_dot(L.csc() + (colc[s] & 0xffffu), (int)(colc[s] >> 16), rs, acc);
      const double reg = (j < first_reg) ? 0.0 : o.l2 * xt[s];
      gj = inv_n * (acc + reg);
    }
    g[s] = gj;
  }
  return inv_n * part;
}

template <int EPL>
struct QuadState {
  double x[EPL], g[EPL], d[EPL];
};

template <int G, int EPL, bool LONG_COLS = true, int LOSS = LOSS_LOGISTIC>
__device__ __forceinline__ void quad_solve(const QuadLds& L, const SolveParams& o, int gl, int n, int p, int ic,
                                           bool valid, unsigned rowc, const unsigned (&colc)[EPL], QuadState<EPL>& V,
                                           XWave& X, SolveStats& out) {
  constexpr int KR = M_REG;
  double S[KR][EPL], Y[KR][EPL];
#pragma unroll
  for (int a = 0; a < KR; ++a) {
#pragma unroll
    for (int s = 0; s < EPL; ++s) { S[a][s] = 0.0; Y[a][s] = 0.0; }
  }
  double* const rho = L.rho();
  double* const alpha = L.alpha();
  double* const scal = L.scal();
  double* const xo = L.xo();
  double* const go = L.go();
  const int m = o.m;
  int cnt = 0;
  int nit = 0, nfev = 0, ifun = 0;
  int status = valid ? -1 : 0;
  bool iter0 = true, first = true;
  double f = 0.0, gd = 0.0, rr = 0.0, stp = 0.0, sbgnrm = 0.0;
  if (valid) {
    scal[SC_FOLD] = 0.0; scal[SC_GDOLD] = 0.0; scal[SC_THETA] = 1.0;
#pragma unroll
    for (int s = 0; s < EPL; ++s) {
      const int j = gl + G * s;
      if (j < p) { xo[j] = 0.0; go[j] = 0.0; }
    }
  }
  while (__any(status < 0)) {
    bool need_dir = false, restart = false;
    if (status < 0) {
      bool counted;
      f = quad_eval<G, EPL, LONG_COLS, LOSS>(L, o, gl, n, p, ic, rowc, colc, V.x, V.g, X, first, counted);
      nfev += counted ? 1 : 0;
      {
        double a = 0.0, b = 0.0, c = 0.0;
#pragma unroll
        for (int s = 0; s < EPL; ++s) {
          const int j = gl + G * s;
          const double gold = (j < p) ? go[j] : 0.0;
          a += V.g[s] * V.d[s];
          const double yj = V.g[s] - gold;
          b += yj * yj;
          c = max_nn(c, fabs(V.g[s]));
        }
        grp_sum2_max<G>(a, b, c, X);
        gd = a; rr = b; sbgnrm = c;
      }
      if (first) {
        first = false;
        if (sbgnrm <= o.pgtol) status = 0;
        else need_dir = true;
      } else {
        int task = LS_CONV;
        {
          const LineSearch* const lsp = L.ls();
          const bool conv = dcsrch_converged(lsp->finit, lsp->gtest, lsp->ginit, f, gd, stp);
          if (__any(!conv)) {
            if (!conv) {
              LineSearch LS = *L.ls();
              task = dcsrch_step(LS, f, gd, stp);
              if (task == LS_FG) *L.ls() = LS;
            }
          }
        }
        if (task == LS_FG) {
          ++ifun;
          if (ifun - 1 < o.maxls) {
#pragma unroll
            for (int s = 0; s < EPL; ++s) {
              const int j = gl + G * s;
              if (j < p) V.x[s] = stp * V.d[s] + xo[j];
            }
          } else {
            restart = true;
            need_dir = true;
          }
        } else {
          ++nit;
          iter0 = false;
          const double fold = scal[SC_FOLD];
          const double dmx = fmax(fabs(fold), fmax(fabs(f), 1.0));
          if (nit >= o.max_iter) status = 2;
          else if (nfev > o.maxfun) status = 3;
          else if (sbgnrm <= o.pgtol) status = 0;
          else if (fold - f <= o.ftol * dmx) status = 1;
          else {
            need_dir = true;
            const double gdold = scal[SC_GDOLD];
            double dr, ddum;
            if (stp == 1.0) { dr = gd - gdold; ddum = -gdold; }
            else { dr = (gd - gdold) * stp; ddum = -gdold * stp; }
            if (dr > EPSMCH * ddum) {
#pragma unroll
              for (int a = 0; a < M_REG - 1; ++a) rho[a] = rho[a + 1];
#pragma unroll
              for (int a = 0; a < KR - 1; ++a) {
#pragma unroll
                for (int s = 0; s < EPL; ++s) { S[a][s] = S[a + 1][s]; Y[a][s] = Y[a + 1][s]; }
              }
#pragma unroll
              for (int s = 0; s < EPL; ++s) {
                const int j = gl + G * s;
                S[KR - 1][s] = stp * V.d[s];
                Y[KR - 1][s] = V.g[s] - ((j < p) ? go[j] : 0.0);
              }
              rho[M_REG - 1] = 1.0 / dr;
              scal[SC_THETA] = rr / dr;
              if (cnt < m) ++cnt;
            }
          }
        }
      }
    }
    while (__any(need_dir)) {
      if (need_dir && restart) {
#pragma unroll
        for (int s = 0; s < EPL; ++s) {
          const int j = gl + G * s;
          if (j < p) { V.x[s] = xo[j]; V.g[s] = go[j]; }
        }
        f = scal[SC_FOLD];
        restart = false;
        if (cnt == 0) { status = 4; need_dir = false; }
        else {
          cnt = 0;
          scal[SC_THETA] = 1.0;
        }
      }
      if (need_dir) {
#pragma unroll
        for (int s = 0; s < EPL; ++s) V.d[s] = -V.g[s];
      }
      const int cmax = wave_max_nonneg_i32(need_dir ? cnt : 0);
      const int a0 = M_REG - cmax;
#define QUAD_FIRST_LOOP_STEP(a)                                                   \
      {                                                                           \
        if ((a) < a0) goto first_loop_done;                                       \
        const bool use = need_dir && ((a) >= M_REG - cnt);                        \
        if (use) {                                                                \
          double t = 0.0;                                                         \
          _Pragma("unroll") for (int s = 0; s < EPL; ++s) t += S[a][s] * V.d[s];  \
          const double al = rho[a] * grp_sum<G>(t, X);                            \
          alpha[a] = al;                                                          \
          _Pragma("unroll") for (int s = 0; s < EPL; ++s) V.d[s] -= al * Y[a][s]; \
        }                                                                         \
      }
      static_assert(M_REG == 10, "the steps below are written out for ten pairs");
      QUAD_FIRST_LOOP_STEP(9) QUAD_FIRST_LOOP_STEP(8) QUAD_FIRST_LOOP_STEP(7) QUAD_FIRST_LOOP_STEP(6) QUAD_FIRST_LOOP_STEP(5)
      QUAD_FIRST_LOOP_STEP(4) QUAD_FIRST_LOOP_STEP(3) QUAD_FIRST_LOOP_STEP(2) QUAD_FIRST_LOOP_STEP(1) QUAD_FIRST_LOOP_STEP(0)
#undef QUAD_FIRST_LOOP_STEP
    first_loop_done:;
      if (need_dir && cnt > 0) {
        const double h0 = 1.0 / scal[SC_THETA];
#pragma unroll
        for (int s = 0; s < EPL; ++s) V.d[s] *= h0;
      }
#define QUAD_SECOND_LOOP_STEP(a)                                                  \
      {                                                                           \
        const bool use = need_dir && ((a) >= M_REG - cnt);                        \
        if (use) {                                                                \
          double t = 0.0;                                                         \
          _Pragma("unroll") for (int s = 0; s < EPL; ++s) t += Y[a][s] * V.d[s];  \
          const double c = alpha[a] - rho[a] * grp_sum<G>(t, X);                  \
          _Pragma("unroll") for (int s = 0; s < EPL; ++s) V.d[s] += c * S[a][s];  \
        }                                                                         \
      }
      switch (a0) {
        case 0: QUAD_SECOND_LOOP_STEP(0) [[fallthrough]];
        case 1: QUAD_SECOND_LOOP_STEP(1) [[fallthrough]];
        case 2: QUAD_SECOND_LOOP_STEP(2) [[fallthrough]];
        case 3: QUAD_SECOND_LOOP_STEP(3) [[fallthrough]];
        case 4: QUAD_SECOND_LOOP_STEP(4) [[fallthrough]];
        case 5: QUAD_SECOND_LOOP_STEP(5) [[fallthrough]];
        case 6: QUAD_SECOND_LOOP_STEP(6) [[fallthrough]];
        case 7: QUAD_SECOND_LOOP_STEP(7) [[fallthrough]];
        case 8: QUAD_SECOND_LOOP_STEP(8) [[fallthrough]];
        case 9: QUAD_SECOND_LOOP_STEP(9) [[fallthrough]];
        default: break;
      }
#undef QUAD_SECOND_LOOP_STEP
      if (need_dir) {
        double dd = 0.0, gdp = 0.0;
#pragma unroll
        for (int s = 0; s < EPL; ++s) {
          const int j = gl + G * s;
          const double xj = V.x[s];
          const double z = xj + V.d[s];
          const double dj = z - xj;
          V.d[s] = dj;
          if (j < p) { xo[j] = xj; go[j] = V.g[s]; }
          dd += dj * dj;
          gdp += V.g[s] * dj;
        }
        grp_sum2<G>(dd, gdp, X);
        gd = gdp;
        scal[SC_GDOLD] = gd;
        scal[SC_FOLD] = f;
        if (gd >= 0.0) {
          restart = true;
        } else {
          stp = iter0 ? fmin(1.0 / sqrt(dd), LS_STPMAX) : 1.0;
          LineSearch LS;
          dcsrch_start(LS, f, gd, stp);
          *L.ls() = LS;
          ifun = 1;
#pragma unroll
          for (int s = 0; s < EPL; ++s) V.x[s] = stp * V.d[s] + V.x[s];
          need_dir = false;
        }
      }
    }
  }
  if (status == 4) {
    double mx = 0.0;
#pragma unroll
    for (int s = 0; s < EPL; ++s) mx = max_nn(mx, fabs(V.g[s]));
    double d0 = 0.0, d1 = 0.0;
    grp_sum2_max<G>(d0, d1, mx, X);
    sbgnrm = mx;
  }
  out.f = f;
  out.gnorm = sbgnrm;
  out.nit = nit;
  out.nfev = nfev;
  out.status = status;
}

}
```

### gdmix_amd/solver.py

```python
import ctypes as C
import functools
import os
from dataclasses import dataclass
from typing import Optional

import numpy as np

from .batch import RawBatch, WireRawBatch

_HERE = os.path.dirname(os.path.abspath(__file__))
LIB_PATH = os.path.join(_HERE, "libgdmix_re.so")

NUM_CLASSES = 40
STATUS_NAMES = ("PGTOL", "FACTR", "MAXITER", "MAXFUN", "ABNORMAL")
VAR_NONE, VAR_SIMPLE, VAR_FULL = 0, 1, 2
VARIANCE_MODES = {None: VAR_NONE, "simple": VAR_SIMPLE, "SIMPLE": VAR_SIMPLE, "full": VAR_FULL, "FULL": VAR_FULL,
                  0: VAR_NONE, 1: VAR_SIMPLE, 2: VAR_FULL}


class GdmixReError(RuntimeError):
    pass


class _RawBatch(C.Structure):
    _fields_ = [("E", C.c_int64), ("N", C.c_int64), ("Z", C.c_int64),
                ("ent_row_ptr", C.c_void_p), ("row_nnz_ptr", C.c_void_p), ("col_global", C.c_void_p),
                ("val", C.c_void_p), ("y", C.c_void_p), ("offset", C.c_void_p), ("weight", C.c_void_p)]


class _WireBatch(C.Structure):
    _fields_ = [("E", C.c_int64), ("N", C.c_int64), ("Z", C.c_int64), ("ent_n", C.c_void_p), ("row_nnz", C.c_void_p),
                ("row_nnz_width", C.c_int32), ("y_width", C.c_int32), ("col_width", C.c_int32), ("reserved", C.c_int32),
                ("col_global", C.c_void_p), ("val", C.c_void_p),
                ("y", C.c_void_p), ("offset", C.c_void_p), ("weight", C.c_void_p)]


class _Packed(C.Structure):
    _fields_ = [("E", C.c_int64), ("N", C.c_int64), ("Z", C.c_int64), ("D", C.c_int64),
                ("ent_row_ptr", C.c_void_p), ("ent_nnz_ptr", C.c_void_p), ("ent_feat_ptr", C.c_void_p),
                ("row_ptr", C.c_void_p), ("csr_col", C.c_void_p), ("csr_val", C.c_void_p),
                ("col_ptr", C.c_void_p), ("csc_row", C.c_void_p), ("csc_val", C.c_void_p),
                ("unique_global", C.c_void_p), ("y", C.c_void_p), ("offset", C.c_void_p), ("weight", C.c_void_p),
                ("order", C.c_void_p), ("cls_tmp", C.c_void_p), ("class_count", C.c_void_p),
                ("scratch", C.c_void_p), ("scratch_bytes", C.c_size_t),
                ("max_p", C.c_int32), ("max_n", C.c_int32), ("max_nnz", C.c_int32)]


class _Opts(C.Structure):
    _fields_ = [("l2", C.c_double), ("regularize_bias", C.c_int32), ("has_intercept", C.c_int32),
                ("m", C.c_int32), ("max_iter", C.c_int32), ("maxfun", C.c_int32), ("maxls", C.c_int32),
                ("ftol", C.c_double), ("pgtol", C.c_double), ("variance_mode", C.c_int32),
                ("threshold", C.c_double), ("sum_loss", C.c_int32), ("loss", C.c_int32)]


class _Result(C.Structure):
    _fields_ = [("theta", C.c_void_p), ("theta_thr", C.c_void_p), ("variance", C.c_void_p),
                ("fval", C.c_void_p), ("gnorm", C.c_void_p), ("nit", C.c_void_p), ("nfev", C.c_void_p),
                ("status", C.c_void_p)]


class _EvalOut(C.Structure):
    _fields_ = [("two_u", C.c_void_p), ("n_pos", C.c_void_p), ("n_neg", C.c_void_p), ("n_nan", C.c_void_p), ("sse", C.c_void_p), ("auc", C.c_void_p)]


class _EvalAcc(C.Structure):
    _fields_ = [("keys", C.c_void_p), ("capacity", C.c_int64), ("count", C.c_int64), ("state", C.c_void_p)]


EVAL_ACC_STATE_BYTES = 33024


class _EvalPlOut(C.Structure):
    _fields_ = [("pl", C.c_void_p), ("n", C.c_void_p), ("n_nan", C.c_void_p)]


class _EvalPlAcc(C.Structure):
    _fields_ = [("state", C.c_void_p), ("count", C.c_int64)]


class _EvalPlTotals(C.Structure):
    _fields_ = [("pl", C.c_double), ("n", C.c_int64), ("n_nan", C.c_int64)]


EVAL_PL_STATE_BYTES = 33024


class _EvalTotals(C.Structure):
    _fields_ = [("two_u", C.c_uint64), ("n", C.c_int64), ("n_pos", C.c_int64), ("n_neg", C.c_int64), ("n_nan", C.c_int64), ("sse", C.c_double)]


EXPORTED_SYMBOLS = (
    "gdmix_re_abi_version", "gdmix_re_build_id", "gdmix_re_device_shared", "gdmix_re_grid_lock_acquire", "gdmix_re_grid_lock_release", "gdmix_re_grid_lock_stats", "gdmix_re_last_error", "gdmix_re_default_opts", "gdmix_re_create",
    "gdmix_re_destroy", "gdmix_re_pack_workspace_bytes", "gdmix_re_pack", "gdmix_re_set_defer_unique", "gdmix_re_pack_join", "gdmix_re_solve",
    "gdmix_re_solve_scratch_bytes", "gdmix_re_set_scratch", "gdmix_re_variance_full", "gdmix_re_set_wave_lds_limit", "gdmix_re_score",
    "gdmix_re_widen_workspace_bytes", "gdmix_re_widen", "gdmix_re_set_timing", "gdmix_re_last_solve_ms", "gdmix_re_set_kernel_mask", "gdmix_re_set_giant_nnz", "gdmix_re_set_team_nnz", "gdmix_re_set_tall_min_n", "gdmix_re_set_tall_split_n", "gdmix_re_set_tall_team_n", "gdmix_re_set_tall_mid_n", "gdmix_re_set_spread",
    "gdmix_fe_create", "gdmix_fe_destroy", "gdmix_fe_eval", "gdmix_fe_reduce_buffer", "gdmix_fe_step", "gdmix_fe_step_async", "gdmix_fe_step_status", "gdmix_fe_solve", "gdmix_fe_result",
    "gdmix_fe_last_eval_ms", "gdmix_fe_stream_bytes", "gdmix_fe_score", "gdmix_fe_hessian_diag", "gdmix_fe_hessian_dense_scratch_bytes", "gdmix_fe_hessian_dense", "gdmix_fe_hessian_dense_loss",
    "gdmix_fe_variance_of_hessian", "gdmix_fe_restart", "gdmix_fe_set_prior", "gdmix_fe_score_models_workspace_bytes", "gdmix_fe_score_models",
    "gdmix_re_eval_workspace_bytes", "gdmix_re_eval_entities", "gdmix_re_set_eval_small_max", "gdmix_re_eval_acc_reset", "gdmix_re_eval_acc_add",
    "gdmix_re_eval_acc_workspace_bytes", "gdmix_re_eval_acc_finish",
    "gdmix_re_eval_pl_entities", "gdmix_re_eval_pl_acc_reset", "gdmix_re_eval_pl_acc_add", "gdmix_re_eval_pl_acc_finish",
    "gdmix_re_join_features", "gdmix_re_score_models_workspace_bytes", "gdmix_re_score_models",
    "gdmix_re_prior_workspace_bytes", "gdmix_re_prior_apply", "gdmix_re_prior_restore",
    "gdmix_re_feature_extent", "gdmix_re_feature_moments", "gdmix_re_feature_scale_expand",
    "gdmix_re_class_kernel_name", "gdmix_java_string_hash", "gdmix_java_partition_id",
    "gdmix_java_partition_ids_i64")

_lib = None


def load_library():
    global _lib
    if _lib is not None:
        return _lib
    if not os.path.exists(LIB_PATH):
        raise GdmixReError(
            f"{LIB_PATH} is missing: build it with `python -m gdmix_amd.build` "
            "(there is no CPU fallback for the random-effect solve)")
    try:
        import torch
    except Exception:
        pass
    from . import build as _build
    stale = _build.check_library(LIB_PATH, _build.source_id, "csrc/*.hip, *.hpp")
    if stale:
        raise GdmixReError(stale)
    lib = C.CDLL(LIB_PATH)
    lib.gdmix_re_abi_version.restype = C.c_int
    lib.gdmix_re_build_id.restype = C.c_char_p
    lib.gdmix_re_device_shared.argtypes = [C.c_void_p]
    lib.gdmix_re_grid_lock_acquire.argtypes = [C.c_char_p]
    lib.gdmix_re_grid_lock_release.argtypes = [C.c_char_p]
    lib.gdmix_re_grid_lock_stats.argtypes = [C.c_char_p, C.POINTER(C.c_int64), C.POINTER(C.c_int64)]
    lib.gdmix_re_last_error.restype = C.c_char_p
    lib.gdmix_re_default_opts.argtypes = [C.POINTER(_Opts)]
    lib.gdmix_re_default_opts.restype = None
    lib.gdmix_re_create.argtypes = [C.c_int, C.POINTER(C.c_void_p)]
    lib.gdmix_re_destroy.argtypes = [C.c_void_p]
    lib.gdmix_re_destroy.restype = None
    lib.gdmix_re_pack_workspace_bytes.argtypes = [C.c_int64, C.c_int64, C.c_int64]
    lib.gdmix_re_pack_workspace_bytes.restype = C.c_size_t
    lib.gdmix_re_pack.argtypes = [C.c_void_p, C.POINTER(_RawBatch), C.c_int, C.c_void_p, C.c_size_t,
                                  C.POINTER(_Packed), C.c_void_p]
    lib.gdmix_re_set_defer_unique.argtypes = [C.c_void_p, C.c_int]
    lib.gdmix_re_pack_join.argtypes = [C.c_void_p, C.c_void_p]
    lib.gdmix_re_widen_workspace_bytes.argtypes = [C.c_int64, C.c_int64, C.c_int64]
    lib.gdmix_re_widen_workspace_bytes.restype = C.c_size_t
    lib.gdmix_re_widen.argtypes = [C.c_void_p, C.POINTER(_WireBatch), C.c_void_p, C.c_size_t, C.POINTER(_RawBatch), C.c_void_p]
    lib.gdmix_re_solve.argtypes = [C.c_void_p, C.POINTER(_Packed), C.POINTER(_Opts), C.c_void_p,
                                   C.POINTER(_Result), C.c_void_p]
    lib.gdmix_re_variance_full.argtypes = [C.c_void_p, C.POINTER(_Packed), C.POINTER(_Opts), C.c_void_p, C.c_void_p, C.c_void_p]
    lib.gdmix_re_solve_scratch_bytes.argtypes = [C.POINTER(_Packed), C.POINTER(_Opts)]
    lib.gdmix_re_solve_scratch_bytes.restype = C.c_size_t
    lib.gdmix_re_set_scratch.argtypes = [C.c_void_p, C.c_void_p, C.c_size_t]
    lib.gdmix_re_set_wave_lds_limit.argtypes = [C.c_void_p, C.c_int]
    lib.gdmix_re_set_kernel_mask.argtypes = [C.c_void_p, C.c_int]
    lib.gdmix_re_set_giant_nnz.argtypes = [C.c_void_p, C.c_int64]
    lib.gdmix_fe_create.argtypes = [C.c_void_p, C.POINTER(_Packed), C.c_int64, C.POINTER(_Opts), C.c_void_p,
                                    C.POINTER(C.c_void_p), C.c_void_p]
    lib.gdmix_fe_destroy.argtypes = [C.c_void_p]
    lib.gdmix_fe_destroy.restype = None
    lib.gdmix_fe_eval.argtypes = [C.c_void_p, C.c_void_p]
    lib.gdmix_fe_reduce_buffer.argtypes = [C.c_void_p, C.POINTER(C.c_int64)]
    lib.gdmix_fe_reduce_buffer.restype = C.c_void_p
    lib.gdmix_fe_step.argtypes = [C.c_void_p, C.c_void_p, C.POINTER(C.c_int32)]
    lib.gdmix_fe_step_async.argtypes = [C.c_void_p, C.c_void_p, C.POINTER(C.c_int64)]
    lib.gdmix_fe_step_status.argtypes = [C.c_void_p, C.c_int64, C.POINTER(C.c_int32)]
    lib.gdmix_fe_solve.argtypes = [C.c_void_p, C.c_void_p, C.c_int32, C.c_int64, C.POINTER(C.c_int32), C.POINTER(C.c_int64)]
    lib.gdmix_fe_hessian_diag.argtypes = [C.c_void_p, C.c_void_p, C.c_void_p]
    lib.gdmix_fe_stream_bytes.argtypes = [C.c_void_p, C.POINTER(C.c_int64), C.POINTER(C.c_int64)]
    lib.gdmix_fe_result.argtypes = [C.c_void_p, C.c_void_p, C.POINTER(C.c_double), C.POINTER(C.c_double),
                                    C.POINTER(C.c_int32), C.POINTER(C.c_int32), C.c_void_p]
    lib.gdmix_fe_score.argtypes = [C.c_void_p, C.c_int64, C.c_void_p, C.c_void_p, C.c_void_p, C.c_void_p, C.c_void_p, C.c_int64, C.c_int,
                                   C.c_void_p, C.c_void_p, C.c_void_p]
    lib.gdmix_fe_hessian_dense_scratch_bytes.argtypes = [C.POINTER(_Packed)]
    lib.gdmix_fe_hessian_dense_scratch_bytes.restype = C.c_size_t
    lib.gdmix_fe_hessian_dense.argtypes = [C.c_void_p, C.POINTER(_Packed), C.c_int, C.c_void_p, C.c_void_p, C.c_int64, C.c_void_p, C.c_size_t, C.c_void_p]
    lib.gdmix_fe_hessian_dense_loss.argtypes = [C.c_void_p, C.POINTER(_Packed), C.c_int, C.c_int, C.c_void_p, C.c_void_p, C.c_int64, C.c_void_p, C.c_size_t,
                                                C.c_void_p]
    lib.gdmix_fe_variance_of_hessian.argtypes = [C.c_void_p, C.c_void_p, C.c_int64, C.c_int64, C.c_double, C.c_int64, C.c_void_p, C.c_void_p, C.c_void_p]
    lib.gdmix_fe_last_eval_ms.argtypes = [C.c_void_p, C.POINTER(C.c_float), C.POINTER(C.c_float)]
    lib.gdmix_fe_restart.argtypes = [C.c_void_p, C.POINTER(_Opts), C.c_void_p, C.c_void_p]
    lib.gdmix_fe_set_prior.argtypes = [C.c_void_p, C.c_void_p, C.c_void_p, C.c_void_p]
    lib.gdmix_fe_score_models_workspace_bytes.argtypes = [C.c_int64, C.c_int]
    lib.gdmix_fe_score_models_workspace_bytes.restype = C.c_size_t
    lib.gdmix_fe_score_models.argtypes = [C.c_void_p, C.c_int64, C.c_void_p, C.c_void_p, C.c_void_p, C.c_void_p, C.POINTER(C.c_void_p), C.c_int, C.c_int64,
                                          C.c_int, C.c_void_p, C.c_void_p, C.c_void_p, C.c_size_t, C.c_void_p]
    lib.gdmix_re_set_team_nnz.argtypes = [C.c_void_p, C.c_int64]
    lib.gdmix_re_set_tall_min_n.argtypes = [C.c_void_p, C.c_int]
    lib.gdmix_re_set_tall_split_n.argtypes = [C.c_void_p, C.c_int]
    lib.gdmix_re_set_tall_team_n.argtypes = [C.c_void_p, C.c_int]
    lib.gdmix_re_set_tall_mid_n.argtypes = [C.c_void_p, C.c_int]
    lib.gdmix_re_set_spread.argtypes = [C.c_void_p, C.c_int]
    lib.gdmix_re_set_timing.argtypes = [C.c_void_p, C.c_int]
    lib.gdmix_re_last_solve_ms.argtypes = [C.c_void_p, C.POINTER(C.c_float)]
    lib.gdmix_re_score.argtypes = [C.c_void_p, C.POINTER(_Packed), C.c_int, C.c_void_p, C.c_void_p,
                                   C.c_void_p, C.c_void_p, C.c_void_p]
    lib.gdmix_re_class_kernel_name.argtypes = [C.c_int]
    lib.gdmix_re_class_kernel_name.restype = C.c_char_p
    lib.gdmix_java_string_hash.argtypes = [C.c_void_p, C.c_int64]
    lib.gdmix_java_string_hash.restype = C.c_int32
    lib.gdmix_java_partition_id.argtypes = [C.c_void_p, C.c_int64, C.c_int32]
    lib.gdmix_java_partition_id.restype = C.c_int32
    lib.gdmix_java_partition_ids_i64.argtypes = [C.c_void_p, C.c_void_p, C.c_int64, C.c_int32, C.c_void_p, C.c_void_p]
    lib.gdmix_re_eval_workspace_bytes.argtypes = [C.c_int64, C.c_int64]
    lib.gdmix_re_eval_workspace_bytes.restype = C.c_size_t
    lib.gdmix_re_eval_entities.argtypes = [C.c_void_p, C.c_void_p, C.c_int64, C.c_int64, C.c_void_p, C.c_void_p, C.POINTER(_EvalOut), C.c_void_p,
                                           C.c_size_t, C.c_void_p]
    lib.gdmix_re_set_eval_small_max.argtypes = [C.c_void_p, C.c_int]
    lib.gdmix_re_eval_acc_reset.argtypes = [C.c_void_p, C.POINTER(_EvalAcc), C.c_void_p]
    lib.gdmix_re_eval_acc_add.argtypes = [C.c_void_p, C.POINTER(_EvalAcc), C.c_void_p, C.c_void_p, C.c_int64, C.c_void_p]
    lib.gdmix_re_eval_acc_workspace_bytes.argtypes = [C.c_int64]
    lib.gdmix_re_eval_acc_workspace_bytes.restype = C.c_size_t
    lib.gdmix_re_eval_acc_finish.argtypes = [C.c_void_p, C.POINTER(_EvalAcc), C.c_void_p, C.c_size_t, C.POINTER(_EvalTotals), C.c_void_p]
    lib.gdmix_re_eval_pl_entities.argtypes = [C.c_void_p, C.c_void_p, C.c_int64, C.c_int64, C.c_void_p, C.c_void_p, C.POINTER(_EvalPlOut), C.c_void_p]
    lib.gdmix_re_eval_pl_acc_reset.argtypes = [C.c_void_p, C.POINTER(_EvalPlAcc), C.c_void_p]
    lib.gdmix_re_eval_pl_acc_add.argtypes = [C.c_void_p, C.POINTER(_EvalPlAcc), C.c_void_p, C.c_void_p, C.c_int64, C.c_void_p]
    lib.gdmix_re_eval_pl_acc_finish.argtypes = [C.c_void_p, C.POINTER(_EvalPlAcc), C.POINTER(_EvalPlTotals), C.c_void_p]
    lib.gdmix_re_join_features.argtypes = [C.c_void_p, C.POINTER(_Packed), C.POINTER(_Packed), C.c_int, C.c_void_p, C.c_void_p, C.c_void_p, C.c_void_p]
    lib.gdmix_re_score_models_workspace_bytes.argtypes = [C.c_int64, C.c_int]
    lib.gdmix_re_score_models_workspace_bytes.restype = C.c_size_t
    lib.gdmix_re_score_models.argtypes = [C.c_void_p, C.POINTER(_Packed), C.c_int, C.POINTER(C.c_void_p), C.c_int, C.c_int64, C.c_void_p, C.c_void_p,
                                          C.c_void_p, C.c_void_p, C.c_void_p, C.c_size_t, C.c_void_p]
    lib.gdmix_re_prior_workspace_bytes.argtypes = [C.POINTER(_Packed)]
    lib.gdmix_re_prior_workspace_bytes.restype = C.c_size_t
    lib.gdmix_re_prior_apply.argtypes = [C.c_void_p, C.POINTER(_Packed), C.c_int, C.c_void_p, C.c_void_p, C.c_void_p, C.c_size_t, C.POINTER(_Packed), C.c_void_p]
    lib.gdmix_re_prior_restore.argtypes = [C.c_void_p, C.POINTER(_Packed), C.c_int, C.c_void_p, C.c_void_p, C.c_double, C.c_void_p, C.c_void_p, C.c_void_p,
                                           C.c_void_p, C.c_void_p, C.c_void_p]
    lib.gdmix_re_feature_extent.argtypes = [C.c_void_p, C.c_void_p, C.c_int, C.c_void_p, C.c_int64, C.c_int64, C.c_void_p, C.c_void_p, C.c_void_p, C.c_void_p]
    lib.gdmix_re_feature_moments.argtypes = [C.c_void_p, C.c_void_p, C.c_int, C.c_void_p, C.c_int64, C.c_int64, C.c_void_p, C.c_void_p, C.c_void_p, C.c_void_p,
                                             C.c_void_p, C.c_void_p]
    lib.gdmix_re_feature_scale_expand.argtypes = [C.c_void_p, C.POINTER(_Packed), C.c_int, C.c_void_p, C.c_int64, C.c_void_p, C.c_void_p]
    if lib.gdmix_re_abi_version() != 19:
        raise GdmixReError("libgdmix_re.so ABI version mismatch")
    _lib = lib
    return lib


def _check(rc, what):
    if rc != 0:
        msg = load_library().gdmix_re_last_error().decode("utf-8", "replace")
        raise GdmixReError(f"{what} failed ({rc}): {msg}")


LOSS_CODES = {"logistic": 0, "squared": 1, "poisson": 2}


@dataclass
class SolverOptions:
    l2: float = 1.0
    regularize_bias: bool = True
    has_intercept: bool = True
    m: int = 10
    max_iter: int = 100
    maxfun: int = 15000
    maxls: int = 20
    ftol: float = 1e-12
    pgtol: float = 1e-5
    variance_mode: int = VAR_NONE
    threshold: float = 1e-4
    sum_loss: bool = False
    linear: bool = False
    loss: str = None

    def loss_name(self):
        if self.loss is None:
            return "squared" if self.linear else "logistic"
        if self.linear:
            raise ValueError("SolverOptions: give either linear=True or loss=..., not both")
        if self.loss not in LOSS_CODES:
            raise ValueError(f"SolverOptions.loss must be one of {sorted(LOSS_CODES)}, not {self.loss!r}")
        return self.loss

    def loss_code(self):
        return LOSS_CODES[self.loss_name()]

    def to_c(self):
        return _Opts(float(self.l2), int(bool(self.regularize_bias)), int(bool(self.has_intercept)),
                     int(self.m), int(self.max_iter), int(self.maxfun), int(self.maxls), float(self.ftol),
                     float(self.pgtol), int(VARIANCE_MODES[self.variance_mode]), float(self.threshold),
                     int(bool(self.sum_loss)), self.loss_code())


def java_string_hash(s: str) -> int:
    cu = np.frombuffer(s.encode("utf-16-le"), dtype=np.uint16).copy()
    return int(load_library().gdmix_java_string_hash(cu.ctypes.data_as(C.c_void_p), cu.size))


def java_partition_id(s: str, num_partitions: int) -> int:
    cu = np.frombuffer(s.encode("utf-16-le"), dtype=np.uint16).copy()
    return int(load_library().gdmix_java_partition_id(cu.ctypes.data_as(C.c_void_p), cu.size, num_partitions))


class PackedBatch:

    def __init__(self, c_struct, tensors, raw_dev, has_intercept, join=None, parent=None):
        self.c = c_struct
        self._join = join
        self._parent = parent
        self._tensors = tensors
        self._raw_dev = raw_dev
        self.has_intercept = bool(has_intercept)
        self.E, self.N, self.Z, self.D = int(c_struct.E), int(c_struct.N), int(c_struct.Z), int(c_struct.D)
        self.P = self.D + (self.E if has_intercept else 0)
        self.max_p, self.max_n, self.max_nnz = int(c_struct.max_p), int(c_struct.max_n), int(c_struct.max_nnz)

    def _view(self, ptr, count, dtype):
        import torch
        ws = self._tensors["workspace"]
        own = self._tensors.get("prior_workspace")
        if own is not None and own.data_ptr() <= ptr < own.data_ptr() + own.numel():
            ws = own
        off = ptr - ws.data_ptr()
        nbytes = count * torch.empty(0, dtype=dtype).element_size()
        return ws[off:off + nbytes].view(dtype)

    def ent_feat_ptr(self):
        import torch
        return self._view(self.c.ent_feat_ptr, self.E + 1, torch.int64)

    def ent_nnz_ptr(self):
        import torch
        return self._view(self.c.ent_nnz_ptr, self.E + 1, torch.int64)

    def unique_global(self):
        import torch
        if self._parent is not None:
            return self._parent.unique_global()
        if self._join is not None:
            self._join()
        return self._view(self.c.unique_global, self.D, torch.int32)

    def __del__(self):
        try:
            if self._join is not None:
                self._join(dropping=True)
        except Exception:
            pass

    def csr_col(self):
        import torch
        return self._view(self.c.csr_col, self.Z, torch.int32)

    def row_ptr(self):
        import torch
        return self._view(self.c.row_ptr, self.N + self.E, torch.int32)

    def col_ptr(self):
        import torch
        return self._view(self.c.col_ptr, self.Z + self.E, torch.int32)

    def csc_row(self):
        import torch
        return self._view(self.c.csc_row, self.Z, torch.int32)

    def csc_val(self):
        import torch
        return self._view(self.c.csc_val, self.Z, torch.float32)

    def csr_val(self):
        import torch
        return self._view(self.c.csr_val, self.Z, torch.float32)

    def offset(self):
        import torch
        if self._parent is not None:
            return self._view(self.c.offset, self.N, torch.float32)
        return self._raw_dev["offset"]

    def coef_ptr_host(self):
        fp = self.ent_feat_ptr().cpu().numpy()
        return fp + (np.arange(self.E + 1, dtype=np.int64) if self.has_intercept else 0)


def host_array(t):
    if not getattr(t, "is_cuda", False):
        return t.cpu().numpy()
    if t.numel() * t.element_size() < (1 << 20):
        return t.cpu().numpy()
    import torch
    h = torch.empty(t.shape, dtype=t.dtype, pin_memory=True)
    h.copy_(t, non_blocking=True)
    torch.cuda.current_stream().synchronize()
    return h.numpy()


class SolveResult:
    def __init__(self, tensors, E, P):
        self._t = tensors
        self.E, self.P = E, P

    def __getattr__(self, k):
        t = self.__dict__.get("_t", {})
        if k in t:
            return t[k]
        raise AttributeError(k)

    def to_host(self, keys=None):
        out, staged = {}, []
        for k, v in self._t.items():
            if keys is not None and k not in keys:
                continue
            if v is None:
                out[k] = None
            elif v.is_cuda and v.numel() * v.element_size() >= (1 << 20):
                import torch
                h = torch.empty(v.shape, dtype=v.dtype, pin_memory=True)
                h.copy_(v, non_blocking=True)
                staged.append((k, h))
            else:
                out[k] = v.cpu().numpy()
        if staged:
            import torch
            torch.cuda.current_stream().synchronize()
            for k, h in staged:
                out[k] = h.numpy()
        return out


def _serialised(fn):
    import functools

    @functools.wraps(fn)
    def wrapper(self, *a, **k):
        with self._ctx_lock:
            return fn(self, *a, **k)
    return wrapper


class REDeviceSolver:

    def __init__(self, device: int = 0):
        import torch
        if not torch.cuda.is_available():
            raise GdmixReError("no HIP device visible: the random-effect solve runs on MI355X only "
                               "(there is no CPU fallback)")
        self.torch = torch
        self.lib = load_library()
        self.tall_team_n = self.TALL_TEAM_N_DEFAULT
        self.device_index = int(device)
        self.device = torch.device("cuda", self.device_index)
        torch.cuda.set_device(self.device)
        torch.zeros(1, device=self.device)
        h = C.c_void_p()
        import threading
        self._ctx_lock = threading.RLock()
        _check(self.lib.gdmix_re_create(self.device_index, C.byref(h)), "gdmix_re_create")
        self._h = h
        self._scratch = None
        self._pack_gen = 0
        self.set_defer_unique(os.environ.get("GDMIX_RE_DEFER_UNIQUE", "1") != "0")

    @_serialised
    def set_defer_unique(self, enabled: bool):
        _check(self.lib.gdmix_re_set_defer_unique(self._h, int(bool(enabled))), "gdmix_re_set_defer_unique")

    @_serialised
    def pack_join(self, stream=None):
        if getattr(self, "_h", None):
            _check(self.lib.gdmix_re_pack_join(self._h, self._stream() if stream is None else stream), "gdmix_re_pack_join")

    @_serialised
    def _pack_join_of(self, gen, pack_stream, dropping=False):
        if gen == self._pack_gen:
            self.pack_join(pack_stream if dropping else None)

    @_serialised
    def close(self):
        if getattr(self, "_h", None):
            self.lib.gdmix_re_destroy(self._h)
            self._h = None

    def __del__(self):
        try:
            self.close()
        except Exception:
            pass

    def set_wave_lds_limit(self, nbytes: int):
        _check(self.lib.gdmix_re_set_wave_lds_limit(self._h, int(nbytes)), "set_wave_lds_limit")

    def set_kernel_mask(self, mask: int):
        _check(self.lib.gdmix_re_set_kernel_mask(self._h, int(mask)), "set_kernel_mask")

    def set_giant_nnz(self, nnz: int):
        _check(self.lib.gdmix_re_set_giant_nnz(self._h, int(nnz)), "set_giant_nnz")

    def set_team_nnz(self, nnz: int):
        _check(self.lib.gdmix_re_set_team_nnz(self._h, int(nnz)), "set_team_nnz")

    TALL_MIN_N_DEFAULT = 32

    def set_tall_min_n(self, min_n: int):
        _check(self.lib.gdmix_re_set_tall_min_n(self._h, int(min_n)), "set_tall_min_n")

    def set_tall_split_n(self, split_n: int):
        _check(self.lib.gdmix_re_set_tall_split_n(self._h, int(split_n)), "set_tall_split_n")

    TALL_TEAM_N_DEFAULT = 8192
    TALL_SPLIT_N_DEFAULT = 4096

    def pin_routing(self):
        self.set_tall_split_n(self.TALL_SPLIT_N_DEFAULT)
        self.set_tall_team_n(-self.TALL_TEAM_N_DEFAULT)

    def set_tall_team_n(self, team_n: int):
        _check(self.lib.gdmix_re_set_tall_team_n(self._h, int(team_n)), "set_tall_team_n")
        self.tall_team_n = int(team_n)

    def device_shared(self) -> bool:
        rc = self.lib.gdmix_re_device_shared(self._h)
        if rc < 0:
            _check(rc, "gdmix_re_device_shared")
        return bool(rc)

    def set_tall_mid_n(self, mid_n: int):
        _check(self.lib.gdmix_re_set_tall_mid_n(self._h, int(mid_n)), "set_tall_mid_n")

    def set_spread(self, queues: int):
        _check(self.lib.gdmix_re_set_spread(self._h, int(queues)), "set_spread")

    def set_timing(self, enabled: bool):
        _check(self.lib.gdmix_re_set_timing(self._h, int(bool(enabled))), "set_timing")

    def last_solve_ms(self):
        ms = (C.c_float * NUM_CLASSES)()
        _check(self.lib.gdmix_re_last_solve_ms(self._h, ms), "last_solve_ms")
        return [float(x) for x in ms]

    def _stream(self):
        return C.c_void_p(self.torch.cuda.current_stream(self.device).cuda_stream)

    def upload(self, raw: RawBatch):
        t = self.torch
        dev = self.device
        d = dict(ent_row_ptr=t.from_numpy(raw.ent_row_ptr).to(dev), row_nnz_ptr=t.from_numpy(raw.row_nnz_ptr).to(dev),
                 col_global=t.from_numpy(raw.col_global).to(dev), val=t.from_numpy(raw.val).to(dev),
                 y=t.from_numpy(raw.y).to(dev), offset=t.from_numpy(raw.offset).to(dev),
                 weight=None if raw.weight is None else t.from_numpy(raw.weight).to(dev))
        d["E"], d["N"], d["Z"] = raw.E, raw.N, raw.Z
        return d

    WIRE_ARRAYS = ("ent_n", "row_nnz", "col_global", "val", "y", "offset", "weight")

    def upload_wire(self, wire, pinned=None):
        t = self.torch
        d = {k: wire[k] for k in ("E", "N", "Z", "row_nnz_width", "y_width", "col_width")}
        for k in self.WIRE_ARRAYS:
            a = wire[k]
            if a is None:
                d[k] = None
                continue
            if isinstance(a, t.Tensor):
                d[k] = a.to(self.device, non_blocking=True)
                continue
            if pinned is not None:
                h = pinned[k][:a.size]
                h.numpy()[...] = a
                d[k] = h.to(self.device, non_blocking=True)
            else:
                d[k] = t.from_numpy(a).to(self.device)
        return d

    def wire_stage(self, wire):
        t = self.torch
        st = self.__dict__.setdefault("_wire_stage", {})
        for k in self.WIRE_ARRAYS:
            a = wire[k]
            if a is None or isinstance(a, t.Tensor):
                continue
            tdt = t.from_numpy(a[:0]).dtype
            cur = st.get(k)
            if cur is None or cur.dtype != tdt or cur.numel() < a.size:
                st[k] = t.empty(int(a.size * 1.25) + 1024, dtype=tdt, pin_memory=True)
        return st

    @_serialised
    def widen(self, wd):
        t = self.torch
        E, N, Z = wd["E"], wd["N"], wd["Z"]
        ptr = lambda x: None if x is None or x.numel() == 0 else x.data_ptr()
        c_wire = _WireBatch(E, N, Z, ptr(wd["ent_n"]), ptr(wd["row_nnz"]), wd["row_nnz_width"], wd["y_width"], wd["col_width"], 0, ptr(wd["col_global"]),
                            ptr(wd["val"]), ptr(wd["y"]), ptr(wd["offset"]), ptr(wd["weight"]))
        nbytes = self.lib.gdmix_re_widen_workspace_bytes(E, N, Z)
        ws = t.empty(nbytes, dtype=t.uint8, device=self.device)
        c_raw = _RawBatch()
        _check(self.lib.gdmix_re_widen(self._h, C.byref(c_wire), ws.data_ptr(), nbytes, C.byref(c_raw), self._stream()), "gdmix_re_widen")

        def view(p, count, dtype):
            if not p or count == 0:
                return t.empty(0, dtype=dtype, device=self.device)
            off = p - ws.data_ptr()
            return ws[off:off + count * t.empty(0, dtype=dtype).element_size()].view(dtype)
        y = wd["y"] if wd["y_width"] == 4 else view(c_raw.y, N, t.float32)
        rd = dict(E=E, N=N, Z=Z, ent_row_ptr=view(c_raw.ent_row_ptr, E + 1, t.int64), row_nnz_ptr=view(c_raw.row_nnz_ptr, N + 1, t.int64),
                  col_global=view(c_raw.col_global, Z, t.int64), val=wd["val"], y=y, offset=wd["offset"], weight=wd["weight"],
                  _keep=(ws, wd))
        return rd

    @_serialised
    def pack(self, raw, has_intercept=True) -> PackedBatch:
        t = self.torch
        if isinstance(raw, WireRawBatch):
            rd = self.widen(self.upload_wire(raw.to_wire()))
        else:
            rd = self.upload(raw) if isinstance(raw, RawBatch) else raw
        E, N, Z = rd["E"], rd["N"], rd["Z"]
        ptr = lambda x: None if x is None or x.numel() == 0 else x.data_ptr()
        c_raw = _RawBatch(E, N, Z, rd["ent_row_ptr"].data_ptr(), rd["row_nnz_ptr"].data_ptr(), ptr(rd["col_global"]),
                          ptr(rd["val"]), ptr(rd["y"]), ptr(rd["offset"]), ptr(rd["weight"]))
        nbytes = self.lib.gdmix_re_pack_workspace_bytes(E, N, Z)
        ws = t.empty(nbytes, dtype=t.uint8, device=self.device)
        c_packed = _Packed()
        st = self._stream()
        _check(self.lib.gdmix_re_pack(self._h, C.byref(c_raw), int(bool(has_intercept)), ws.data_ptr(), nbytes,
                                      C.byref(c_packed), st), "gdmix_re_pack")
        self._pack_gen += 1
        return PackedBatch(c_packed, {"workspace": ws}, rd, has_intercept, join=functools.partial(self._pack_join_of, self._pack_gen, st))

    def alloc_result(self, packed: PackedBatch, variance=False):
        t, dev = self.torch, self.device
        E, P = packed.E, packed.P
        return dict(theta=t.empty(P, dtype=t.float64, device=dev), theta_thr=t.empty(P, dtype=t.float64, device=dev),
                    variance=t.empty(P, dtype=t.float64, device=dev) if variance else None,
                    fval=t.empty(E, dtype=t.float64, device=dev), gnorm=t.empty(E, dtype=t.float64, device=dev),
                    nit=t.empty(E, dtype=t.int32, device=dev), nfev=t.empty(E, dtype=t.int32, device=dev),
                    status=t.full((E,), -1, dtype=t.int32, device=dev))

    @_serialised
    def solve(self, packed: PackedBatch, opts: Optional[SolverOptions] = None, theta0=None, out=None) -> SolveResult:
        t = self.torch
        opts = opts or SolverOptions()
        if bool(opts.has_intercept) != packed.has_intercept:
            raise GdmixReError("has_intercept of the options differs from the packed batch")
        c_opts = opts.to_c()
        need = self.lib.gdmix_re_solve_scratch_bytes(C.byref(packed.c), C.byref(c_opts))
        if need > packed.c.scratch_bytes and (self._scratch is None or self._scratch.numel() < need):
            self._scratch = t.empty(need, dtype=t.uint8, device=self.device)
        if self._scratch is not None:
            _check(self.lib.gdmix_re_set_scratch(self._h, self._scratch.data_ptr(), self._scratch.numel()), "set_scratch")
        if theta0 is not None:
            if isinstance(theta0, np.ndarray):
                theta0 = t.from_numpy(np.ascontiguousarray(theta0, np.float64)).to(self.device)
            elif not theta0.is_cuda:
                theta0 = theta0.to(self.device, non_blocking=theta0.is_pinned())
            if theta0.numel() != packed.P or theta0.dtype != t.float64:
                raise GdmixReError("theta0 must be float64 with one entry per coefficient")
        tensors = out or self.alloc_result(packed, variance=c_opts.variance_mode != VAR_NONE)
        p = lambda x: None if x is None else x.data_ptr()
        c_res = _Result(p(tensors["theta"]), p(tensors["theta_thr"]), p(tensors.get("variance")), p(tensors["fval"]),
                        p(tensors["gnorm"]), p(tensors["nit"]), p(tensors["nfev"]), p(tensors["status"]))
        _check(self.lib.gdmix_re_solve(self._h, C.byref(packed.c), C.byref(c_opts), p(theta0), C.byref(c_res),
                                       self._stream()), "gdmix_re_solve")
        return SolveResult(tensors, packed.E, packed.P)

    @_serialised
    def variance_full(self, packed: PackedBatch, opts: SolverOptions, theta):
        t = self.torch
        if isinstance(theta, np.ndarray):
            theta = t.from_numpy(np.ascontiguousarray(theta, np.float64)).to(self.device)
        if theta.numel() != packed.P or theta.dtype != t.float64:
            raise GdmixReError("theta must be float64 with one entry per coefficient")
        c_opts = opts.to_c()
        c_opts.variance_mode = VAR_FULL
        need = self.lib.gdmix_re_solve_scratch_bytes(C.byref(packed.c), C.byref(c_opts))
        if need > packed.c.scratch_bytes and (self._scratch is None or self._scratch.numel() < need):
            self._scratch = t.empty(need, dtype=t.uint8, device=self.device)
        if self._scratch is not None:
            _check(self.lib.gdmix_re_set_scratch(self._h, self._scratch.data_ptr(), self._scratch.numel()), "set_scratch")
        out = t.empty(packed.P, dtype=t.float64, device=self.device)
        _check(self.lib.gdmix_re_variance_full(self._h, C.byref(packed.c), C.byref(c_opts), theta.data_ptr(), out.data_ptr(), self._stream()),
               "gdmix_re_variance_full")
        return out
# ... 166 lines not shown
```

### include/gdmix_re.h

```cpp
#ifndef GDMIX_RE_H_
#define GDMIX_RE_H_

#include <stdint.h>
#include <stddef.h>

#ifdef __cplusplus
extern "C" {
#endif

#define GDMIX_RE_ABI_VERSION 19

#if defined(__GNUC__)
#define GDMIX_API __attribute__((visibility("default")))
#else
#define GDMIX_API
#endif

#define GDMIX_RE_OK          0
#define GDMIX_RE_EINVAL    (-1)
#define GDMIX_RE_EHIP      (-2)
#define GDMIX_RE_ENOMEM    (-3)
#define GDMIX_RE_ERANGE    (-4)

#define GDMIX_RE_ST_PGTOL     0
#define GDMIX_RE_ST_FACTR     1
#define GDMIX_RE_ST_MAXITER   2
#define GDMIX_RE_ST_MAXFUN    3
#define GDMIX_RE_ST_ABNORMAL  4
#define GDMIX_RE_ST_ABORTED   9
#define GDMIX_RE_ST_ABORTED_PEER 10

#define GDMIX_RE_VAR_NONE    0
#define GDMIX_RE_VAR_SIMPLE  1
#define GDMIX_RE_VAR_FULL    2

typedef struct gdmix_re_ctx gdmix_re_ctx;

typedef struct {
  int64_t E, N, Z;
  const int64_t* ent_row_ptr;
  const int64_t* row_nnz_ptr;
  const int64_t* col_global;
  const float*   val;
  const float*   y;
  const float*   offset;
  const float*   weight;
} gdmix_re_raw_batch;

typedef struct {
  int64_t E, N, Z;
  const int32_t* ent_n;
  const void*    row_nnz;
  int32_t        row_nnz_width;
  int32_t        y_width;
  int32_t        col_width;
  int32_t        reserved;
  const void*    col_global;
  const float*   val;
  const void*    y;
  const float*   offset;
  const float*   weight;
} gdmix_re_wire_batch;

typedef struct {
  int64_t E, N, Z, D;
  const int64_t* ent_row_ptr;
  int64_t*       ent_nnz_ptr;
  int64_t*       ent_feat_ptr;
  int32_t*       row_ptr;
  int32_t*       csr_col;
  float*         csr_val;
  int32_t*       col_ptr;
  int32_t*       csc_row;
  float*         csc_val;
  int32_t*       unique_global;
  const float*   y;
  const float*   offset;
  const float*   weight;
  int32_t*       order;
  int32_t*       cls_tmp;
  int32_t*       class_count;
  void*          scratch;
  size_t         scratch_bytes;
  int32_t        max_p, max_n, max_nnz;
} gdmix_re_packed;

#define GDMIX_RE_NUM_CLASSES 40

typedef struct {
  double  l2;
  int32_t regularize_bias;
  int32_t has_intercept;
  int32_t m;
  int32_t max_iter;
  int32_t maxfun;
  int32_t maxls;
  double  ftol;
  double  pgtol;
  int32_t variance_mode;
  double  threshold;
  int32_t sum_loss;
  int32_t loss;
} gdmix_re_opts;

#define GDMIX_RE_LOSS_LOGISTIC 0
#define GDMIX_RE_LOSS_SQUARED  1
#define GDMIX_RE_LOSS_POISSON  2

GDMIX_API void gdmix_re_default_opts(gdmix_re_opts* o);

typedef struct {
  double*  theta;
  double*  theta_thr;
  double*  variance;
  double*  fval;
  double*  gnorm;
  int32_t* nit;
  int32_t* nfev;
  int32_t* status;
} gdmix_re_result;

GDMIX_API int  gdmix_re_abi_version(void);
GDMIX_API const char* gdmix_re_build_id(void);
GDMIX_API const char* gdmix_re_last_error(void);

GDMIX_API int gdmix_re_device_shared(gdmix_re_ctx* ctx);
GDMIX_API int gdmix_re_grid_lock_acquire(const char* key);
GDMIX_API int gdmix_re_grid_lock_release(const char* key);
GDMIX_API int gdmix_re_grid_lock_stats(const char* key, int64_t* takes, int64_t* rides);

GDMIX_API int  gdmix_re_create(int hip_device, gdmix_re_ctx** out);
GDMIX_API void gdmix_re_destroy(gdmix_re_ctx* ctx);

GDMIX_API size_t gdmix_re_pack_workspace_bytes(int64_t E, int64_t N, int64_t Z);

GDMIX_API int gdmix_re_pack(gdmix_re_ctx* ctx, const gdmix_re_raw_batch* raw_dev, int has_intercept,
                  void* workspace, size_t workspace_bytes, gdmix_re_packed* out, void* stream);

GDMIX_API int gdmix_re_set_defer_unique(gdmix_re_ctx* ctx, int enabled);
GDMIX_API int gdmix_re_pack_join(gdmix_re_ctx* ctx, void* stream);

GDMIX_API size_t gdmix_re_widen_workspace_bytes(int64_t E, int64_t N, int64_t Z);
GDMIX_API int gdmix_re_widen(gdmix_re_ctx* ctx, const gdmix_re_wire_batch* wire_dev, void* workspace, size_t workspace_bytes,
                   gdmix_re_raw_batch* out, void* stream);

GDMIX_API int gdmix_re_solve(gdmix_re_ctx* ctx, const gdmix_re_packed* batch, const gdmix_re_opts* opts,
                   const double* theta0, const gdmix_re_result* out, void* stream);

GDMIX_API size_t gdmix_re_solve_scratch_bytes(const gdmix_re_packed* batch, const gdmix_re_opts* opts);
GDMIX_API int    gdmix_re_set_scratch(gdmix_re_ctx* ctx, void* scratch, size_t bytes);

GDMIX_API int gdmix_re_variance_full(gdmix_re_ctx* ctx, const gdmix_re_packed* batch, const gdmix_re_opts* opts, const double* theta,
                                     double* variance, void* stream);

GDMIX_API int gdmix_re_score(gdmix_re_ctx* ctx, const gdmix_re_packed* batch, int has_intercept,
                   const double* theta, const uint8_t* has_model,
                   float* logit, float* logit_per_coord, void* stream);

GDMIX_API int gdmix_re_set_wave_lds_limit(gdmix_re_ctx* ctx, int bytes);

GDMIX_API int gdmix_re_set_kernel_mask(gdmix_re_ctx* ctx, int mask);

GDMIX_API int gdmix_re_set_giant_nnz(gdmix_re_ctx* ctx, int64_t giant_nnz);
GDMIX_API int gdmix_re_set_team_nnz(gdmix_re_ctx* ctx, int64_t team_nnz);

#define GDMIX_RE_TALL_MIN_N_DEFAULT 32
GDMIX_API int gdmix_re_set_tall_min_n(gdmix_re_ctx* ctx, int min_n);
#define GDMIX_RE_TALL_SPLIT_N_DEFAULT 4096
GDMIX_API int gdmix_re_set_tall_split_n(gdmix_re_ctx* ctx, int split_n);
#define GDMIX_RE_TALL_TEAM_N_DEFAULT 8192
GDMIX_API int gdmix_re_set_tall_team_n(gdmix_re_ctx* ctx, int team_n);
GDMIX_API int gdmix_re_set_tall_mid_n(gdmix_re_ctx* ctx, int mid_n);

GDMIX_API int gdmix_re_set_spread(gdmix_re_ctx* ctx, int queues);

GDMIX_API int gdmix_re_set_timing(gdmix_re_ctx* ctx, int enabled);
GDMIX_API int gdmix_re_last_solve_ms(gdmix_re_ctx* ctx, float* ms_out);

GDMIX_API const char* gdmix_re_class_kernel_name(int c);

typedef struct {
  uint64_t* two_u;
  int32_t*  n_pos;
  int32_t*  n_neg;
  int32_t*  n_nan;
  double*   sse;
  double*   auc;
} gdmix_re_eval_out;

typedef struct {
  uint64_t two_u;
  int64_t  n;
  int64_t  n_pos, n_neg, n_nan;
  double   sse;
} gdmix_re_eval_totals;

GDMIX_API size_t gdmix_re_eval_workspace_bytes(int64_t E, int64_t N);
GDMIX_API int gdmix_re_eval_entities(gdmix_re_ctx* ctx, const int64_t* ent_row_ptr, int64_t E, int64_t N, const float* score, const float* label,
                                     const gdmix_re_eval_out* out, void* workspace, size_t workspace_bytes, void* stream);
GDMIX_API int gdmix_re_set_eval_small_max(gdmix_re_ctx* ctx, int small_max);

#define GDMIX_RE_EVAL_ACC_STATE_BYTES 33024
typedef struct {
  uint64_t* keys;
  int64_t   capacity;
  int64_t   count;
  void*     state;
} gdmix_re_eval_acc;
GDMIX_API int gdmix_re_eval_acc_reset(gdmix_re_ctx* ctx, gdmix_re_eval_acc* acc, void* stream);
GDMIX_API int gdmix_re_eval_acc_add(gdmix_re_ctx* ctx, gdmix_re_eval_acc* acc, const float* score, const float* label, int64_t N, void* stream);
GDMIX_API size_t gdmix_re_eval_acc_workspace_bytes(int64_t N);
GDMIX_API int gdmix_re_eval_acc_finish(gdmix_re_ctx* ctx, const gdmix_re_eval_acc* acc, void* workspace, size_t workspace_bytes,
                                       gdmix_re_eval_totals* host_out, void* stream);

typedef struct {
  double*  pl;
  int32_t* n;
  int32_t* n_nan;
} gdmix_re_eval_pl_out;
typedef struct {
  double  pl;
  int64_t n;
  int64_t n_nan;
} gdmix_re_eval_pl_totals;
GDMIX_API int gdmix_re_eval_pl_entities(gdmix_re_ctx* ctx, const int64_t* ent_row_ptr, int64_t E, int64_t N, const float* score, const float* label,
                                        const gdmix_re_eval_pl_out* out, void* stream);
#define GDMIX_RE_EVAL_PL_STATE_BYTES 33024
typedef struct {
  void*   state;
  int64_t count;
} gdmix_re_eval_pl_acc;
GDMIX_API int gdmix_re_eval_pl_acc_reset(gdmix_re_ctx* ctx, gdmix_re_eval_pl_acc* acc, void* stream);
GDMIX_API int gdmix_re_eval_pl_acc_add(gdmix_re_ctx* ctx, gdmix_re_eval_pl_acc* acc, const float* score, const float* label, int64_t N, void* stream);
GDMIX_API int gdmix_re_eval_pl_acc_finish(gdmix_re_ctx* ctx, const gdmix_re_eval_pl_acc* acc, gdmix_re_eval_pl_totals* host_out, void* stream);

#define GDMIX_RE_SWEEP_MODELS_PER_PASS 8
GDMIX_API int gdmix_re_join_features(gdmix_re_ctx* ctx, const gdmix_re_packed* eval, const gdmix_re_packed* train, int has_intercept,
                                     const int32_t* train_entity, int64_t* coef_pos, uint8_t* has_model, void* stream);
GDMIX_API size_t gdmix_re_score_models_workspace_bytes(int64_t P_train, int K);
GDMIX_API int gdmix_re_score_models(gdmix_re_ctx* ctx, const gdmix_re_packed* eval, int has_intercept, const double* const* thetas, int K,
                                    int64_t P_train, const int64_t* coef_pos, const uint8_t* has_model, float* logit, float* logit_per_coord,
                                    void* workspace, size_t workspace_bytes, void* stream);

GDMIX_API size_t gdmix_re_prior_workspace_bytes(const gdmix_re_packed* packed);
GDMIX_API int gdmix_re_prior_apply(gdmix_re_ctx* ctx, const gdmix_re_packed* packed, int has_intercept, const double* mean, const double* scale,
                                   void* workspace, size_t workspace_bytes, gdmix_re_packed* out, void* stream);
GDMIX_API int gdmix_re_prior_restore(gdmix_re_ctx* ctx, const gdmix_re_packed* packed, int has_intercept, const double* mean, const double* scale,
                                     double threshold, const double* phi, const double* var_phi, double* theta, double* theta_thr,
                                     double* variance, void* stream);

GDMIX_API int gdmix_re_feature_extent(gdmix_re_ctx* ctx, const void* col, int col_width, const float* val, int64_t Z, int64_t num_features,
                                      uint64_t* count, uint32_t* max_abs_bits, int64_t* bad, void* stream);
GDMIX_API int gdmix_re_feature_moments(gdmix_re_ctx* ctx, const void* col, int col_width, const float* val, int64_t Z, int64_t num_features,
                                       const int32_t* limb_bits, const int32_t* shift1, const int32_t* shift2, int64_t* limbs, int64_t* bad,
                                       void* stream);
GDMIX_API int gdmix_re_feature_scale_expand(gdmix_re_ctx* ctx, const gdmix_re_packed* packed, int has_intercept, const double* factor,
                                            int64_t num_features, double* scale, void* stream);

GDMIX_API int32_t gdmix_java_string_hash(const uint16_t* utf16, int64_t len);
GDMIX_API int32_t gdmix_java_partition_id(const uint16_t* utf16, int64_t len, int32_t num_partitions);
GDMIX_API int gdmix_java_partition_ids_i64(gdmix_re_ctx* ctx, const int64_t* ids_dev, int64_t count,
                                 int32_t num_partitions, int32_t* out_dev, void* stream);

#ifdef __cplusplus
}
#endif
#endif
```

Baseline: 111.8 million entities/s.

## Route small PAIR3 entities to a narrow 16-lane EPL=5 kernel with partial register history

Measured after the change: 122.8 million entities/s (median of 6 runs). 9.8% higher.

```diff
diff --git a/gdmix_amd/csrc/re_api.hip b/gdmix_amd/csrc/re_api.hip
--- a/gdmix_amd/csrc/re_api.hip
+++ b/gdmix_amd/csrc/re_api.hip
@@ -356,6 +356,8 @@
   if (const char* e = getenv("GDMIX_RE_TALL_TEAM")) { if (atoi(e) == 0) c->impl.tall_team_n = 0; }
   if (const char* e = getenv("GDMIX_RE_TALL_TEAM_LIMIT")) { if (atoi(e) > 0 && atoi(e) <= TALL_TEAM_MAX) c->impl.tall_team_limit = atoi(e); }
   c->impl.spread = spread_default();
+  c->impl.narrow = 1;
+  if (const char* e = getenv("GDMIX_RE_NARROW")) c->impl.narrow = atoi(e) != 0 ? 1 : 0;
   c->impl.grid_sync = nullptr;
   c->impl.big_tmp = nullptr;
   c->impl.big_tmp_bytes = 0;
@@ -531,6 +533,12 @@
   return GDMIX_RE_OK;
 }
 
+GDMIX_API int gdmix_re_set_narrow(gdmix_re_ctx* ctx, int on) {
+  if (!ctx) { set_error("ctx is NULL"); return GDMIX_RE_EINVAL; }
+  ctx->impl.narrow = on ? 1 : 0;
+  return GDMIX_RE_OK;
+}
+
 GDMIX_API int gdmix_re_set_tall_team_n(gdmix_re_ctx* ctx, int team_n) {
   if (!ctx) { set_error("bad argument"); return GDMIX_RE_EINVAL; }
   ctx->impl.tall_team_n = ctx->impl.num_cus < 8 * TALL_TEAM_C ? 0 : team_n;
@@ -660,8 +668,12 @@
     case KIND_TALL_L: case KIND_TALL_S: case KIND_TALL_M: case KIND_TALL:
       return launch_solve_tall(d.tall_variant, B, O, P, theta0, L.begin, L.count, ci->num_cus, b->Z, GridSyncLayout::tall_tail(ci, d.tall_variant),
                                GridSyncLayout::tall_ticket(ci, d.tall_variant), d.kind == KIND_TALL_S ? lean_merged : 0, s);
-    default:
-      return d.lanes > 0 ? launch_solve_quad(d.lanes, d.epl, B, O, P, theta0, L.begin, L.count, d.ncap, d.zcap, s) : hipErrorInvalidValue;
+    default: {
+      if (d.lanes <= 0) return hipErrorInvalidValue;
+      const int nn = (L.c == NARROW_HOST_CLASS && L.narrow > 0) ? (L.narrow < L.count ? L.narrow : L.count) : 0;
+      if (hipError_t rc = launch_solve_quad(NARROW_LANES, NARROW_EPL, B, O, P, theta0, L.begin, nn, NARROW_NCAP, NARROW_ZCAP, s); rc != hipSuccess) return rc;
+      return launch_solve_quad(d.lanes, d.epl, B, O, P, theta0, L.begin + nn, L.count - nn, d.ncap, d.zcap, s);
+    }
   }
 }
 
diff --git a/gdmix_amd/csrc/re_internal.hpp b/gdmix_amd/csrc/re_internal.hpp
--- a/gdmix_amd/csrc/re_internal.hpp
+++ b/gdmix_amd/csrc/re_internal.hpp
@@ -137,6 +137,13 @@
 static_assert(class_table_consistent(), "group_lanes / group_epl and the class constants describe kClasses");
 static_assert(GIANT_CLASS == GDMIX_RE_NUM_CLASSES - 1 && BLOCK_CLASS - TALL_T_CLASS == TALL_VARIANTS, "the tall classes, the block class, three tiers and the giant class end the table");
 static_assert(TALL_L_CLASS + 1 == TALL_S_CLASS, "a merged lean class sits right in front of the one-wavefront class in `order`");
+constexpr int NARROW_HOST_CLASS = 9;
+static_assert(kClasses[NARROW_HOST_CLASS].kind == KIND_PAIR3 && kClasses[NARROW_HOST_CLASS].ncap == 32 && kClasses[NARROW_HOST_CLASS].zcap == 128 &&
+              class_of_kind(KIND_PAIR3) == NARROW_HOST_CLASS, "the narrow kernel takes its entities from <32,3> n<=32 nnz<=128");
+constexpr int NARROW_LANES = 16, NARROW_EPL = 5, NARROW_NCAP = 24, NARROW_ZCAP = 96;
+constexpr int NARROW_FLAG = 0x100;
+static_assert(NARROW_FLAG > GDMIX_RE_NUM_CLASSES, "the mark is no class index");
+__host__ __device__ constexpr bool narrow_fits(int p, int n, int z) { return p <= NARROW_LANES * NARROW_EPL && n <= NARROW_NCAP && z <= NARROW_ZCAP; }
 constexpr int BLOCK_NW = 4;
 #ifndef GDMIX_TEAM_BLOCK_NW
 #define GDMIX_TEAM_BLOCK_NW 8
@@ -156,6 +163,7 @@
   int tall_adapt_limit;
   int tall_team_n;
   int tall_team_limit;
+  int narrow;
   int tall_mid_n;
 };
 constexpr int TALL_ADAPT_STEPS = 3;
@@ -176,7 +184,8 @@
   int32_t base[GDMIX_RE_NUM_CLASSES];
   int32_t cursor[GDMIX_RE_NUM_CLASSES];
   TallRouting tall;
-  int32_t row3_free[TEAM128_CLASS - (int)(sizeof(TallRouting) / sizeof(int32_t))];
+  int32_t narrow_count;
+  int32_t row3_free[TEAM128_CLASS - 1 - (int)(sizeof(TallRouting) / sizeof(int32_t))];
   int32_t team_largest_nnz[GDMIX_RE_NUM_CLASSES - TEAM128_CLASS];
   unsigned long long team_nnz_total[GDMIX_RE_NUM_CLASSES];
   __host__ __device__ int32_t& largest_nnz(int c) { return team_largest_nnz[c - TEAM128_CLASS]; }
@@ -188,6 +197,8 @@
               offsetof(ClassCounts, team_largest_nnz) == (3 * GDMIX_RE_NUM_CLASSES + TEAM128_CLASS) * sizeof(int32_t) &&
               offsetof(ClassCounts, team_nnz_total) == 4 * GDMIX_RE_NUM_CLASSES * sizeof(int32_t), "the rows of the count record");
 static_assert(offsetof(TallRouting, mid_from) / sizeof(int32_t) < (size_t)TEAM128_CLASS, "row 3: the last threshold slot stays below the team tiers' columns");
+static_assert(offsetof(ClassCounts, narrow_count) == (3 * GDMIX_RE_NUM_CLASSES + GDMIX_RE_NARROW_COUNT_WORD) * sizeof(int32_t) && GDMIX_RE_NARROW_COUNT_WORD < TEAM128_CLASS,
+              "row 3: the narrow count sits where include/gdmix_re.h says, below the team tiers' columns");
 
 struct BatchDev {
   const int64_t* ent_row_ptr;
@@ -243,6 +254,7 @@
   int tall_team_n;
   int tall_team_limit;
   int tall_mid_n;
+  int narrow;
   int spread;
   void* grid_sync;
   void* big_tmp;
@@ -316,7 +328,7 @@
 
 int make_class_table(const gdmix_ctx_impl* ci, const gdmix_re_opts* opts, ClassTable* out);
 int route(gdmix_ctx_impl* ci, const gdmix_re_packed* b, const ClassTable& tab, const gdmix_re_opts* opts, hipStream_t s, const ClassCounts** host);
-struct Launch { int c, begin, count, stream; };
+struct Launch { int c, begin, count, stream, narrow; };
 struct LaunchPlan {
   Launch launch[GDMIX_RE_NUM_CLASSES];
   int n;
diff --git a/gdmix_amd/csrc/re_route.hip b/gdmix_amd/csrc/re_route.hip
--- a/gdmix_amd/csrc/re_route.hip
+++ b/gdmix_amd/csrc/re_route.hip
@@ -33,6 +33,8 @@
     tab.tall_team_limit = tn > 0 ? ci->tall_team_limit : 0;
   }
   tab.tall_mid_n = (ci->tall_mid_n < 0 && ci->tall_split_set) ? 0 : ci->tall_mid_n;
+  tab.narrow = (ci->narrow && tab.lds_bytes[NARROW_HOST_CLASS] > 0 &&
+                (WAVE / NARROW_LANES) * quad_layout(NARROW_LANES * NARROW_EPL, NARROW_NCAP, NARROW_ZCAP).bytes <= ci->wave_lds_limit) ? 1 : 0;
   if (opts->sum_loss) {
     if (opts->m > TEAM_MCAP) { set_error("sum_loss needs m <= %d", TEAM_MCAP); return GDMIX_RE_EINVAL; }
     if (opts->variance_mode != GDMIX_RE_VAR_NONE) { set_error("variance is not available with sum_loss"); return GDMIX_RE_EINVAL; }
@@ -75,7 +77,7 @@
       if (tab.team_nnz > 0 && z >= tab.team_nnz)
         c = (z >= 128 * tab.team_nnz) ? TEAM8_CLASS : ((z >= 8 * tab.team_nnz) ? TEAM32_CLASS : TEAM128_CLASS);
     }
-    cls_out[e] = c;
+    cls_out[e] = (c == NARROW_HOST_CLASS && tab.narrow && narrow_fits(p, n, z)) ? (c | NARROW_FLAG) : c;
     atomicAdd(&local[c], 1);
     if (c == TALL_S_CLASS && tab.tall_adapt_limit > 0 && n >= tall_adapt_n(0)) {
 #pragma unroll
@@ -154,31 +156,40 @@
 __global__ __launch_bounds__(256) void re_order_kernel(int32_t* __restrict__ cls, int64_t E, ClassCounts* __restrict__ cc,
                                                        int32_t* __restrict__ order, const int64_t* __restrict__ ent_row_ptr) {
   __shared__ int32_t cnt[GDMIX_RE_NUM_CLASSES], base[GDMIX_RE_NUM_CLASSES];
+  __shared__ int32_t nar_cnt, nar_base;
   const int split = cc->tall.split;
   const int team_from = cc->tall.team_from;
   const int mid_from = cc->tall.mid_from;
   const int64_t chunk = (int64_t)blockDim.x * 8;
   for (int64_t start = (int64_t)blockIdx.x * chunk; start < E; start += (int64_t)gridDim.x * chunk) {
     if (threadIdx.x < GDMIX_RE_NUM_CLASSES) cnt[threadIdx.x] = 0;
+    if (threadIdx.x == 0) nar_cnt = 0;
     __syncthreads();
     int c[8], pos[8];
+    unsigned nar = 0;
 #pragma unroll
     for (int k = 0; k < 8; ++k) {
       const int64_t e = start + (int64_t)k * blockDim.x + threadIdx.x;
       c[k] = (e < E) ? cls[e] : -1;
+      if (c[k] >= NARROW_FLAG) { c[k] -= NARROW_FLAG; cls[e] = c[k]; nar |= 1u << k; }
       if (split > 0 && c[k] == TALL_S_CLASS && ent_row_ptr[e + 1] - ent_row_ptr[e] >= split) { c[k] = TALL_CLASS; cls[e] = TALL_CLASS; }
       else if (team_from > 0 && c[k] == TALL_CLASS && ent_row_ptr[e + 1] - ent_row_ptr[e] >= team_from) { c[k] = TALL_T_CLASS; cls[e] = TALL_T_CLASS; }
       else if (mid_from > 0 && c[k] == TALL_S_CLASS && ent_row_ptr[e + 1] - ent_row_ptr[e] >= mid_from) { c[k] = TALL_M_CLASS; cls[e] = TALL_M_CLASS; }
-      pos[k] = (c[k] >= 0) ? atomicAdd(&cnt[c[k]], 1) : 0;
+      pos[k] = (c[k] >= 0) ? atomicAdd((nar >> k) & 1u ? &nar_cnt : &cnt[c[k]], 1) : 0;
     }
     __syncthreads();
     if (threadIdx.x < GDMIX_RE_NUM_CLASSES)
       base[threadIdx.x] = cnt[threadIdx.x] ? atomicAdd(&cc->cursor[threadIdx.x], cnt[threadIdx.x]) : 0;
+    if (threadIdx.x == GDMIX_RE_NUM_CLASSES) nar_base = nar_cnt ? atomicAdd(&cc->narrow_count, nar_cnt) : 0;
     __syncthreads();
 #pragma unroll
     for (int k = 0; k < 8; ++k) {
       const int64_t e = start + (int64_t)k * blockDim.x + threadIdx.x;
-      if (c[k] >= 0) order[cc->base[c[k]] + base[c[k]] + pos[k]] = (int32_t)e;
+      if (c[k] < 0) continue;
+      const int seg = cc->base[c[k]];
+      if ((nar >> k) & 1u) order[seg + nar_base + pos[k]] = (int32_t)e;
+      else if (c[k] == NARROW_HOST_CLASS) order[seg + cc->count[c[k]] - 1 - (base[c[k]] + pos[k])] = (int32_t)e;
+      else order[seg + base[c[k]] + pos[k]] = (int32_t)e;
     }
     __syncthreads();
   }
@@ -239,7 +250,7 @@
     if (count[c] <= 0) continue;
     small[plan.n] = plan.fork && class_is_small(kClasses[c], count[c], num_cus);
     any_large = any_large || !small[plan.n];
-    plan.launch[plan.n++] = Launch{c, begin[c], count[c], -1};
+    plan.launch[plan.n++] = Launch{c, begin[c], count[c], -1, c == NARROW_HOST_CLASS ? counts.narrow_count : 0};
   }
   int spread_rr = 0;
   for (int k = 0; k < plan.n; ++k) {
diff --git a/gdmix_amd/csrc/re_solve.hip b/gdmix_amd/csrc/re_solve.hip
--- a/gdmix_amd/csrc/re_solve.hip
+++ b/gdmix_amd/csrc/re_solve.hip
@@ -27,6 +27,10 @@
 #ifndef GDMIX_QUAD_WAVES_EPL2
 #define GDMIX_QUAD_WAVES_EPL2 2
 #endif
+#ifndef GDMIX_NARROW_KR
+#define GDMIX_NARROW_KR 5
+#endif
+constexpr int grp_reg_pairs(int epl) { return epl >= 5 ? GDMIX_NARROW_KR : M_REG; }
 template <int G, int EPL, int NCAP, int ZCAP, int LOSS>
 __global__ __launch_bounds__(G > WAVE ? G : WAVE)
 __attribute__((amdgpu_waves_per_eu(EPL == 2 ? GDMIX_QUAD_WAVES_EPL2 : (EPL >= 3 ? GDMIX_QUAD_WAVES_EPL4 : 1)))) void re_solve_grp_kernel(
@@ -89,7 +93,7 @@
   }
   grp_fence<G>();
   SolveStats st;
-  quad_solve<G, EPL, (NCAP > G), LOSS>(L, o, gl, n, p, ic, valid, rowc, colc, V, X, st);
+  quad_solve<G, EPL, (NCAP > G), LOSS, grp_reg_pairs(EPL)>(L, o, gl, n, p, ic, valid, rowc, colc, V, X, st);
   if (!valid) return;
 
 #pragma unroll
@@ -189,6 +193,7 @@
   GDMIX_GRP_CASE(16, 2, 16, 64) GDMIX_GRP_CASE(16, 2, 32, 128) GDMIX_GRP_CASE(16, 2, 128, 512)
   GDMIX_GRP_CASE(16, 3, 16, 64) GDMIX_GRP_CASE(16, 3, 32, 128) GDMIX_GRP_CASE(16, 3, 128, 512)
   GDMIX_GRP_CASE(16, 4, 16, 64) GDMIX_GRP_CASE(16, 4, 32, 128) GDMIX_GRP_CASE(16, 4, 128, 512)
+  GDMIX_GRP_CASE(NARROW_LANES, NARROW_EPL, NARROW_NCAP, NARROW_ZCAP)
   GDMIX_GRP_CASE(32, 3, 32, 128) GDMIX_GRP_CASE(32, 3, 64, 256) GDMIX_GRP_CASE(32, 3, 256, 1024)
   GDMIX_GRP_CASE(32, 4, 32, 128) GDMIX_GRP_CASE(32, 4, 64, 256) GDMIX_GRP_CASE(32, 4, 256, 1024)
   GDMIX_GRP_CASE(64, 3, 64, 512) GDMIX_GRP_CASE(64, 3, 512, 2048) GDMIX_GRP_CASE(64, 4, 64, 512) GDMIX_GRP_CASE(64, 4, 512, 2048)
diff --git a/gdmix_amd/csrc/re_solve_quad.hpp b/gdmix_amd/csrc/re_solve_quad.hpp
--- a/gdmix_amd/csrc/re_solve_quad.hpp
+++ b/gdmix_amd/csrc/re_solve_quad.hpp
@@ -433,12 +433,15 @@
   double x[EPL], g[EPL], d[EPL];
 };
 
-template <int G, int EPL, bool LONG_COLS = true, int LOSS = LOSS_LOGISTIC>
+template <int G, int EPL, bool LONG_COLS = true, int LOSS = LOSS_LOGISTIC, int KR = M_REG>
 __device__ __forceinline__ void quad_solve(const QuadLds& L, const SolveParams& o, int gl, int n, int p, int ic,
                                            bool valid, unsigned rowc, const unsigned (&colc)[EPL], QuadState<EPL>& V,
                                            XWave& X, SolveStats& out) {
-  constexpr int KR = M_REG;
+  static_assert(KR >= 1 && KR <= M_REG, "register-resident pairs");
+  constexpr int RN = M_REG - KR;
   double S[KR][EPL], Y[KR][EPL];
+  double RS[RN > 0 ? RN : 1][EPL], RY[RN > 0 ? RN : 1][EPL];
+  int head = 0;
 #pragma unroll
   for (int a = 0; a < KR; ++a) {
 #pragma unroll
@@ -530,6 +533,13 @@
             if (dr > EPSMCH * ddum) {
 #pragma unroll
               for (int a = 0; a < M_REG - 1; ++a) rho[a] = rho[a + 1];
+              if constexpr (RN > 0) {
+                if (cnt >= KR && m > KR) {
+#pragma unroll
+                  for (int s = 0; s < EPL; ++s) { RS[head][s] = S[0][s]; RY[head][s] = Y[0][s]; }
+                }
+                head = (head + 1 == RN) ? 0 : head + 1;
+              }
 #pragma unroll
               for (int a = 0; a < KR - 1; ++a) {
 #pragma unroll
@@ -570,16 +580,27 @@
       }
       const int cmax = wave_max_nonneg_i32(need_dir ? cnt : 0);
       const int a0 = M_REG - cmax;
+      const auto ring_slot = [&](int a) { const int sl = head - (RN - a); return sl < 0 ? sl + RN : sl; };
+      (void)ring_slot;
 #define QUAD_FIRST_LOOP_STEP(a)                                                   \
       {                                                                           \
         if ((a) < a0) goto first_loop_done;                                       \
         const bool use = need_dir && ((a) >= M_REG - cnt);                        \
         if (use) {                                                                \
-          double t = 0.0;                                                         \
-          _Pragma("unroll") for (int s = 0; s < EPL; ++s) t += S[a][s] * V.d[s];  \
-          const double al = rho[a] * grp_sum<G>(t, X);                            \
-          alpha[a] = al;                                                          \
-          _Pragma("unroll") for (int s = 0; s < EPL; ++s) V.d[s] -= al * Y[a][s]; \
+          if constexpr ((a) >= RN) {                                              \
+            double t = 0.0;                                                       \
+            _Pragma("unroll") for (int s = 0; s < EPL; ++s) t += S[(a) - RN][s] * V.d[s];  \
+            const double al = rho[a] * grp_sum<G>(t, X);                          \
+            alpha[a] = al;                                                        \
+            _Pragma("unroll") for (int s = 0; s < EPL; ++s) V.d[s] -= al * Y[(a) - RN][s]; \
+          } else {                                                                \
+            const int sl = ring_slot(a);                                          \
+            double t = 0.0;                                                       \
+            _Pragma("unroll") for (int s = 0; s < EPL; ++s) t += RS[sl][s] * V.d[s];       \
+            const double al = rho[a] * grp_sum<G>(t, X);                          \
+            alpha[a] = al;                                                        \
+            _Pragma("unroll") for (int s = 0; s < EPL; ++s) V.d[s] -= al * RY[sl][s];      \
+          }                                                                       \
         }                                                                         \
       }
       static_assert(M_REG == 10, "the steps below are written out for ten pairs");
@@ -596,10 +617,18 @@
       {                                                                           \
         const bool use = need_dir && ((a) >= M_REG - cnt);                        \
         if (use) {                                                                \
-          double t = 0.0;                                                         \
-          _Pragma("unroll") for (int s = 0; s < EPL; ++s) t += Y[a][s] * V.d[s];  \
-          const double c = alpha[a] - rho[a] * grp_sum<G>(t, X);                  \
-          _Pragma("unroll") for (int s = 0; s < EPL; ++s) V.d[s] += c * S[a][s];  \
+          if constexpr ((a) >= RN) {                                              \
+            double t = 0.0;                                                       \
+            _Pragma("unroll") for (int s = 0; s < EPL; ++s) t += Y[(a) - RN][s] * V.d[s];  \
+            const double c = alpha[a] - rho[a] * grp_sum<G>(t, X);                \
+            _Pragma("unroll") for (int s = 0; s < EPL; ++s) V.d[s] += c * S[(a) - RN][s];  \
+          } else {                                                                \
+            const int sl = ring_slot(a);                                          \
+            double t = 0.0;                                                       \
+            _Pragma("unroll") for (int s = 0; s < EPL; ++s) t += RY[sl][s] * V.d[s];       \
+            const double c = alpha[a] - rho[a] * grp_sum<G>(t, X);                \
+            _Pragma("unroll") for (int s = 0; s < EPL; ++s) V.d[s] += c * RS[sl][s];       \
+          }                                                                       \
         }                                                                         \
       }
       switch (a0) {
diff --git a/gdmix_amd/solver.py b/gdmix_amd/solver.py
--- a/gdmix_amd/solver.py
+++ b/gdmix_amd/solver.py
@@ -93,7 +93,7 @@
     "gdmix_re_abi_version", "gdmix_re_build_id", "gdmix_re_device_shared", "gdmix_re_grid_lock_acquire", "gdmix_re_grid_lock_release", "gdmix_re_grid_lock_stats", "gdmix_re_last_error", "gdmix_re_default_opts", "gdmix_re_create",
     "gdmix_re_destroy", "gdmix_re_pack_workspace_bytes", "gdmix_re_pack", "gdmix_re_set_defer_unique", "gdmix_re_pack_join", "gdmix_re_solve",
     "gdmix_re_solve_scratch_bytes", "gdmix_re_set_scratch", "gdmix_re_variance_full", "gdmix_re_set_wave_lds_limit", "gdmix_re_score",
-    "gdmix_re_widen_workspace_bytes", "gdmix_re_widen", "gdmix_re_set_timing", "gdmix_re_last_solve_ms", "gdmix_re_set_kernel_mask", "gdmix_re_set_giant_nnz", "gdmix_re_set_team_nnz", "gdmix_re_set_tall_min_n", "gdmix_re_set_tall_split_n", "gdmix_re_set_tall_team_n", "gdmix_re_set_tall_mid_n", "gdmix_re_set_spread",
+    "gdmix_re_widen_workspace_bytes", "gdmix_re_widen", "gdmix_re_set_timing", "gdmix_re_last_solve_ms", "gdmix_re_set_kernel_mask", "gdmix_re_set_giant_nnz", "gdmix_re_set_team_nnz", "gdmix_re_set_tall_min_n", "gdmix_re_set_tall_split_n", "gdmix_re_set_tall_team_n", "gdmix_re_set_tall_mid_n", "gdmix_re_set_spread", "gdmix_re_set_narrow",
     "gdmix_fe_create", "gdmix_fe_destroy", "gdmix_fe_eval", "gdmix_fe_reduce_buffer", "gdmix_fe_step", "gdmix_fe_step_async", "gdmix_fe_step_status", "gdmix_fe_solve", "gdmix_fe_result",
     "gdmix_fe_last_eval_ms", "gdmix_fe_stream_bytes", "gdmix_fe_score", "gdmix_fe_hessian_diag", "gdmix_fe_hessian_dense_scratch_bytes", "gdmix_fe_hessian_dense", "gdmix_fe_hessian_dense_loss",
     "gdmix_fe_variance_of_hessian", "gdmix_fe_restart", "gdmix_fe_set_prior", "gdmix_fe_score_models_workspace_bytes", "gdmix_fe_score_models",
@@ -192,6 +192,7 @@
     lib.gdmix_re_set_tall_team_n.argtypes = [C.c_void_p, C.c_int]
     lib.gdmix_re_set_tall_mid_n.argtypes = [C.c_void_p, C.c_int]
     lib.gdmix_re_set_spread.argtypes = [C.c_void_p, C.c_int]
+    lib.gdmix_re_set_narrow.argtypes = [C.c_void_p, C.c_int]
     lib.gdmix_re_set_timing.argtypes = [C.c_void_p, C.c_int]
     lib.gdmix_re_last_solve_ms.argtypes = [C.c_void_p, C.POINTER(C.c_float)]
     lib.gdmix_re_score.argtypes = [C.c_void_p, C.POINTER(_Packed), C.c_int, C.c_void_p, C.c_void_p,
@@ -231,7 +232,7 @@
     lib.gdmix_re_feature_moments.argtypes = [C.c_void_p, C.c_void_p, C.c_int, C.c_void_p, C.c_int64, C.c_int64, C.c_void_p, C.c_void_p, C.c_void_p, C.c_void_p,
                                              C.c_void_p, C.c_void_p]
     lib.gdmix_re_feature_scale_expand.argtypes = [C.c_void_p, C.POINTER(_Packed), C.c_int, C.c_void_p, C.c_int64, C.c_void_p, C.c_void_p]
-    if lib.gdmix_re_abi_version() != 19:
+    if lib.gdmix_re_abi_version() != 20:
         raise GdmixReError("libgdmix_re.so ABI version mismatch")
     _lib = lib
     return lib
@@ -519,6 +520,15 @@
 
     def set_spread(self, queues: int):
         _check(self.lib.gdmix_re_set_spread(self._h, int(queues)), "set_spread")
+
+    def set_narrow(self, on: bool):
+        _check(self.lib.gdmix_re_set_narrow(self._h, int(bool(on))), "set_narrow")
+
+    NARROW_COUNT_WORD = 15
+
+    def narrow_count(self, packed: PackedBatch) -> int:
+        row3 = packed._view(packed.c.class_count, 4 * NUM_CLASSES, self.torch.int32)[3 * NUM_CLASSES:].cpu().numpy()
+        return int(row3[self.NARROW_COUNT_WORD])
 
     def set_timing(self, enabled: bool):
         _check(self.lib.gdmix_re_set_timing(self._h, int(bool(enabled))), "set_timing")
diff --git a/include/gdmix_re.h b/include/gdmix_re.h
--- a/include/gdmix_re.h
+++ b/include/gdmix_re.h
@@ -8,7 +8,7 @@
 extern "C" {
 #endif
 
-#define GDMIX_RE_ABI_VERSION 19
+#define GDMIX_RE_ABI_VERSION 20
 
 #if defined(__GNUC__)
 #define GDMIX_API __attribute__((visibility("default")))
@@ -172,6 +172,9 @@
 GDMIX_API int gdmix_re_set_tall_team_n(gdmix_re_ctx* ctx, int team_n);
 GDMIX_API int gdmix_re_set_tall_mid_n(gdmix_re_ctx* ctx, int mid_n);
 
+#define GDMIX_RE_NARROW_COUNT_WORD 15
+GDMIX_API int gdmix_re_set_narrow(gdmix_re_ctx* ctx, int on);
+
 GDMIX_API int gdmix_re_set_spread(gdmix_re_ctx* ctx, int queues);
 
 GDMIX_API int gdmix_re_set_timing(gdmix_re_ctx* ctx, int enabled);
```
